# kmurf1999/RustSolver

Measured on NVIDIA B200. Metric: cfr_iterations_per_sec, higher is better.
Workload: dtype f32

## Files before the change

### include/b200cfr.h

```cpp
#ifndef B200CFR_H
#define B200CFR_H

#include <stddef.h>
#include <stdint.h>

#ifdef __cplusplus
extern "C" {
#endif

#define RS_OK 0
#define RS_ERR_INVALID -1
#define RS_ERR_CUDA -2
#define RS_ERR_NCCL -3
#define RS_ERR_CAPACITY -4
#define RS_ERR_UNSUPPORTED -5

#define RS_NODE_ACTION 0
#define RS_NODE_TERMINAL 1
#define RS_NODE_PUBLIC_CHANCE 2
#define RS_NODE_PRIVATE_CHANCE 3
#define RS_TERM_ALLIN 0
#define RS_TERM_SHOWDOWN 1
#define RS_TERM_UNCONTESTED 2
#define RS_ROUND_FLOP 0
#define RS_ROUND_TURN 1
#define RS_ROUND_RIVER 2

typedef struct rs_tree {
    uint32_t n_nodes;
    const uint8_t* type;
    const int32_t* parent;
    const uint32_t* child_offset;
    const uint32_t* children;
    const uint8_t* player;
    const uint32_t* an_index;
    const uint8_t* round_idx;
    const uint32_t* value;
    const uint8_t* ttype;
    const uint8_t* last_to_act;
} rs_tree;

typedef struct rs_ranges {
    uint32_t n_hands[2];
    const uint8_t* hands[2];
} rs_ranges;

#define RS_ABS_NONE 0
#define RS_ABS_ISOMORPHIC 1
#define RS_ABS_CLUSTER_ARR 2
#define RS_ABS_BUCKET_TABLE 3
typedef struct rs_round_abstraction {
    uint32_t kind;
    const uint32_t* cluster_arr;
    uint64_t cluster_arr_len;
    const uint32_t* bucket_table[2];
} rs_round_abstraction;
typedef struct rs_abstraction {
    uint32_t n_rounds;
    rs_round_abstraction rounds[3];
} rs_abstraction;

#define RS_NCCL_ID_BYTES 128
typedef struct rs_config {
    uint64_t board_mask;
    int32_t device;
    int32_t rank;
    int32_t world_size;
    uint8_t nccl_id[RS_NCCL_ID_BYTES];
    uint32_t flags;
    uint32_t threads_per_block;
    uint64_t discount_interval;
    uint64_t discount_cap;
} rs_config;
#define RS_FLAG_NO_GRAPH 1u
#define RS_FLAG_NO_CHAIN_SPLIT 2u
#define RS_FLAG_STREET_KERNEL 4u
#define RS_FLAG_SHARD_ISOLATED 8u
#define RS_FLAG_ALL (RS_FLAG_NO_GRAPH | RS_FLAG_NO_CHAIN_SPLIT | RS_FLAG_STREET_KERNEL | RS_FLAG_SHARD_ISOLATED)

typedef struct rs_engine rs_engine;

typedef struct rs_stats {
    uint64_t iterations;
    uint64_t updates_per_iteration;
    uint64_t updates_per_iteration_global;
    double device_ms;
    uint64_t kernel_launches;
    uint64_t table_bytes;
    uint32_t n_rounds;
    uint32_t n_boards[3];
    uint32_t n_boards_local[3];
    uint32_t n_hands[2];
    uint64_t n_combos;
} rs_stats;

const char* rs_last_error(void);
int rs_version(void);
int rs_device_count(void);
int rs_nccl_unique_id(uint8_t* out);

int rs_gpu_index_hands(uint32_t n_board_cards, const uint8_t* cards, size_t n, uint64_t* out, float* kernel_ms);

#define RS_DIST_EMD_1D 0u
#define RS_DIST_L2 1u
int rs_kmeans_assign(const float* points, size_t n, uint32_t dim, const float* centers, uint32_t k, uint32_t dist_kind,
                     uint32_t* cluster, float* min_dist, double* inertia, float* kernel_ms);
int rs_histogram_distances(const float* p, const float* q, size_t n, uint32_t dim, uint32_t dist_kind, float* out);
int rs_kmeans_fit_regular(const float* points, size_t n, uint32_t dim, float* centers, uint32_t k, uint32_t dist_kind,
                          uint32_t rounds, uint32_t* cluster, float* inertia);
int rs_generate_histograms(uint32_t round, uint64_t first_index, size_t count, uint32_t samples, uint32_t bins, uint64_t seed,
                           float* out, uint8_t* cards_out, float* kernel_ms);
int rs_kmeans_fit_growbatch(const float* points, size_t n, uint32_t dim, float* centers, uint32_t k, uint32_t dist_kind,
                            uint32_t initial_batch_size, uint64_t seed, uint32_t* batch_index_out, uint32_t* cluster_out,
                            float* stats_out);
int rs_kmeans_update_min_dists(const float* points, size_t n, uint32_t dim, const float* new_center, uint32_t dist_kind,
                               float* min_dists);
int rs_kmeans_init_pp(const float* points, size_t n, uint32_t dim, uint32_t k, uint32_t dist_kind, uint64_t seed, uint32_t* chosen_out,
                      float* centers_out);
int rs_kmeans_init_random(const float* points, size_t n, uint32_t dim, uint32_t k, uint32_t n_restarts, uint32_t dist_kind, uint64_t seed,
                          uint32_t* chosen_out, float* centers_out);

#define RS_EXCHANGE_HANDLE_BYTES 64
int rs_exchange_export(rs_engine* e, uint8_t* out );
int rs_exchange_import(rs_engine* e, const uint8_t* handles , uint32_t n_ranks);
int rs_exchange_disable(rs_engine* e);


int rs_create(const rs_tree* tree, const rs_ranges* ranges, const rs_abstraction* abs,
              const rs_config* cfg, rs_engine** out);
int rs_create_batch(const rs_tree* tree, const rs_ranges* ranges, const rs_abstraction* abs,
                    const rs_config* cfg, const uint64_t* board_masks, uint32_t n_subgames,
                    rs_engine** out);
void rs_destroy(rs_engine* e);

int rs_iterate(rs_engine* e, uint64_t n_iters);
int rs_iterate_sampled(rs_engine* e, const uint8_t* dealt, uint32_t n_paths);
int rs_sample_runouts(uint64_t seed, uint64_t board_mask, uint32_t n_cards, uint32_t n_paths, int distinct_first, uint8_t* dealt_out);
int rs_discount(rs_engine* e, float d);
int rs_set_wait_timeout_ms(rs_engine* e, uint64_t ms);
int rs_abort(rs_engine* e);
int rs_set_prune_threshold(rs_engine* e, float threshold);
#define RS_OPP_FULL 0u
#define RS_OPP_SAMPLE 1u
#define RS_OPP_SAMPLE_TIMES_SIGMA 2u
int rs_set_opponent_sampling(rs_engine* e, uint32_t mode, uint64_t seed);
#define RS_RULE_VANILLA 0u
#define RS_RULE_DCFR 1u
#define RS_RULE_LCFR 2u
#define RS_RULE_CFR_PLUS 3u
typedef struct rs_update_rule {
    uint32_t kind;
    float alpha, beta, gamma;
} rs_update_rule;
int rs_set_update_rule(rs_engine* e, const rs_update_rule* rule);
int rs_get_update_rule(rs_engine* e, rs_update_rule* out, uint64_t* t_out);
int rs_reset(rs_engine* e);

int rs_read_infoset(rs_engine* e, uint32_t an_index, uint32_t board_id, float* regrets,
                    float* strategy_sum, size_t cap_floats, uint32_t* n_rows_out,
                    uint32_t* n_actions_out);
int rs_write_infoset(rs_engine* e, uint32_t an_index, uint32_t board_id, const float* regrets,
                     const float* strategy_sum, size_t n_floats);
int rs_average_strategy(rs_engine* e, uint32_t an_index, uint32_t board_id, float* out,
                        size_t cap_floats, uint32_t* n_rows_out, uint32_t* n_actions_out);
int rs_current_strategy(rs_engine* e, uint32_t an_index, uint32_t board_id, float* out,
                        size_t cap_floats, uint32_t* n_rows_out, uint32_t* n_actions_out);
int rs_dump_average_strategy(rs_engine* e, const char* path, uint64_t* n_floats_out);

int rs_board_id(rs_engine* e, uint32_t round_idx, const uint8_t* dealt, uint32_t n_dealt,
                uint32_t* board_id_out);
int rs_card_table(rs_engine* e, uint32_t round_idx, uint32_t player, uint32_t board_id,
                  uint16_t* rows_out, size_t cap, uint32_t* n_rows_out);

int rs_best_response(rs_engine* e, double out[2]);
int rs_average_value(rs_engine* e, double out[2]);
int rs_root_values(rs_engine* e, uint32_t player, float* out, size_t cap);

int rs_stats_get(rs_engine* e, rs_stats* out);

int rs_set_range_weights(rs_engine* e, uint32_t player, const float* weights, size_t n);

#define RS_KERNEL_TRAVERSAL 0
#define RS_KERNEL_STREET 1
#define RS_KERNEL_ALLREDUCE 3
typedef struct rs_kernel_time {
    uint32_t kind;
    uint32_t phase;
    uint32_t traverser;
    uint32_t grid;
    float ms;
    uint64_t table_bytes;
    uint64_t vector_bytes;
} rs_kernel_time;
int rs_profile_iteration(rs_engine* e, rs_kernel_time* out, size_t cap, uint32_t* n_out);

int rs_debug_task_timing(rs_engine* e, unsigned long long* out32, int reset);

typedef struct rs_plan rs_plan;
int rs_plan_create(const rs_tree* tree, const rs_ranges* ranges, const rs_abstraction* abs,
                   const rs_config* cfg, const uint64_t* board_masks, uint32_t n_subgames,
                   rs_plan** out);
void rs_plan_destroy(rs_plan* p);
int rs_plan_stats(const rs_plan* p, rs_stats* out);
int rs_plan_board_id(const rs_plan* p, uint32_t round_idx, const uint8_t* dealt, uint32_t n_dealt,
                     uint32_t* board_id_out);
int rs_plan_card_table(const rs_plan* p, uint32_t round_idx, uint32_t player, uint32_t board_id,
                       uint16_t* rows_out, size_t cap, uint32_t* n_rows_out);
int rs_plan_infoset_offset(const rs_plan* p, uint32_t an_index, uint32_t board_id,
                           uint64_t* offset_out, uint32_t* n_rows_out, uint32_t* n_actions_out);
int rs_plan_showdown_order(const rs_plan* p, uint32_t player, uint32_t board_id,
                           uint16_t* order_out, uint32_t* class_out, size_t cap,
                           uint32_t* n_live_out);

int rs_plan_local_tables(const rs_plan* p, uint32_t round_idx, uint32_t player, uint32_t board_id, uint32_t* hrec_words_out,
                         uint16_t* cl_pos_out, uint16_t* slot_of_pos_out, uint32_t dims_out[2]);
int rs_plan_check_execution_order(const rs_plan* p, uint32_t traverser, int force_board_major, uint32_t* n_tickets_out,
                                  uint32_t* n_moved_out);
int rs_plan_street_info(const rs_plan* p, uint32_t traverser, uint32_t out[8]);
int rs_plan_street_program(const rs_plan* p, uint32_t traverser, uint32_t board_id, uint32_t* words_out, size_t cap,
                           uint32_t* n_words_out, uint32_t* hinfo_out, size_t hinfo_cap, uint32_t dims_out[4]);

#ifdef __cplusplus
}
#endif
#endif
```

### rustsolver_b200/_lib.py

```python
from __future__ import annotations

import ctypes as C
import os
from pathlib import Path

_HERE = Path(__file__).resolve().parent
LIB_PATH = Path(os.environ.get("RS_ENGINE_LIB", str(_HERE / "libb200cfr.so")))

u8p = C.POINTER(C.c_uint8)
u16p = C.POINTER(C.c_uint16)
u32p = C.POINTER(C.c_uint32)
u64p = C.POINTER(C.c_uint64)
i32p = C.POINTER(C.c_int32)
f32p = C.POINTER(C.c_float)
f64p = C.POINTER(C.c_double)

RS_NCCL_ID_BYTES = 128
RS_EXCHANGE_HANDLE_BYTES = 64


class rs_tree(C.Structure):
    _fields_ = [("n_nodes", C.c_uint32), ("type", u8p), ("parent", i32p), ("child_offset", u32p),
                ("children", u32p), ("player", u8p), ("an_index", u32p), ("round_idx", u8p),
                ("value", u32p), ("ttype", u8p), ("last_to_act", u8p)]


class rs_ranges(C.Structure):
    _fields_ = [("n_hands", C.c_uint32 * 2), ("hands", u8p * 2)]


class rs_round_abstraction(C.Structure):
    _fields_ = [("kind", C.c_uint32), ("cluster_arr", u32p), ("cluster_arr_len", C.c_uint64),
                ("bucket_table", u32p * 2)]


class rs_abstraction(C.Structure):
    _fields_ = [("n_rounds", C.c_uint32), ("rounds", rs_round_abstraction * 3)]


class rs_config(C.Structure):
    _fields_ = [("board_mask", C.c_uint64), ("device", C.c_int32), ("rank", C.c_int32),
                ("world_size", C.c_int32), ("nccl_id", C.c_uint8 * RS_NCCL_ID_BYTES),
                ("flags", C.c_uint32), ("threads_per_block", C.c_uint32),
                ("discount_interval", C.c_uint64), ("discount_cap", C.c_uint64)]


class rs_stats(C.Structure):
    _fields_ = [("iterations", C.c_uint64), ("updates_per_iteration", C.c_uint64),
                ("updates_per_iteration_global", C.c_uint64), ("device_ms", C.c_double),
                ("kernel_launches", C.c_uint64), ("table_bytes", C.c_uint64), ("n_rounds", C.c_uint32),
                ("n_boards", C.c_uint32 * 3), ("n_boards_local", C.c_uint32 * 3),
                ("n_hands", C.c_uint32 * 2), ("n_combos", C.c_uint64)]


class rs_update_rule(C.Structure):
    _fields_ = [("kind", C.c_uint32), ("alpha", C.c_float), ("beta", C.c_float), ("gamma", C.c_float)]


class rs_kernel_time(C.Structure):
    _fields_ = [("kind", C.c_uint32), ("phase", C.c_uint32), ("traverser", C.c_uint32), ("grid", C.c_uint32),
                ("ms", C.c_float), ("table_bytes", C.c_uint64), ("vector_bytes", C.c_uint64)]


VP = C.c_void_p
ENGINE_API = {
    "rs_last_error": (C.c_char_p, []),
    "rs_version": (C.c_int, []),
    "rs_device_count": (C.c_int, []),
    "rs_nccl_unique_id": (C.c_int, [u8p]),
    "rs_kmeans_assign": (C.c_int, [f32p, C.c_size_t, C.c_uint32, f32p, C.c_uint32, C.c_uint32, u32p, f32p, f64p, f32p]),
    "rs_kmeans_fit_regular": (C.c_int, [f32p, C.c_size_t, C.c_uint32, f32p, C.c_uint32, C.c_uint32, C.c_uint32, u32p, f32p]),
    "rs_histogram_distances": (C.c_int, [f32p, f32p, C.c_size_t, C.c_uint32, C.c_uint32, f32p]),
    "rs_kmeans_update_min_dists": (C.c_int, [f32p, C.c_size_t, C.c_uint32, f32p, C.c_uint32, f32p]),
    "rs_kmeans_init_pp": (C.c_int, [f32p, C.c_size_t, C.c_uint32, C.c_uint32, C.c_uint32, C.c_uint64, u32p, f32p]),
    "rs_generate_histograms": (C.c_int, [C.c_uint32, C.c_uint64, C.c_size_t, C.c_uint32, C.c_uint32, C.c_uint64, f32p, u8p, f32p]),
    "rs_kmeans_fit_growbatch": (C.c_int, [f32p, C.c_size_t, C.c_uint32, f32p, C.c_uint32, C.c_uint32, C.c_uint32, C.c_uint64, u32p, u32p, f32p]),
    "rs_kmeans_init_random": (C.c_int, [f32p, C.c_size_t, C.c_uint32, C.c_uint32, C.c_uint32, C.c_uint32, C.c_uint64, u32p, f32p]),
    "rs_gpu_index_hands": (C.c_int, [C.c_uint32, u8p, C.c_size_t, u64p, f32p]),
    "rs_exchange_export": (C.c_int, [VP, u8p]),
    "rs_exchange_import": (C.c_int, [VP, u8p, C.c_uint32]),
    "rs_exchange_disable": (C.c_int, [VP]),
    "rs_create": (C.c_int, [C.POINTER(rs_tree), C.POINTER(rs_ranges), C.POINTER(rs_abstraction),
                            C.POINTER(rs_config), C.POINTER(VP)]),
    "rs_create_batch": (C.c_int, [C.POINTER(rs_tree), C.POINTER(rs_ranges), C.POINTER(rs_abstraction),
                                  C.POINTER(rs_config), u64p, C.c_uint32, C.POINTER(VP)]),
    "rs_destroy": (None, [VP]),
    "rs_iterate": (C.c_int, [VP, C.c_uint64]),
    "rs_iterate_sampled": (C.c_int, [VP, u8p, C.c_uint32]),
    "rs_discount": (C.c_int, [VP, C.c_float]),
    "rs_set_prune_threshold": (C.c_int, [VP, C.c_float]),
    "rs_set_opponent_sampling": (C.c_int, [VP, C.c_uint32, C.c_uint64]),
    "rs_set_wait_timeout_ms": (C.c_int, [VP, C.c_uint64]),
    "rs_abort": (C.c_int, [VP]),
    "rs_sample_runouts": (C.c_int, [C.c_uint64, C.c_uint64, C.c_uint32, C.c_uint32, C.c_int, u8p]),
    "rs_set_update_rule": (C.c_int, [VP, C.POINTER(rs_update_rule)]),
    "rs_get_update_rule": (C.c_int, [VP, C.POINTER(rs_update_rule), u64p]),
    "rs_reset": (C.c_int, [VP]),
    "rs_read_infoset": (C.c_int, [VP, C.c_uint32, C.c_uint32, f32p, f32p, C.c_size_t, u32p, u32p]),
    "rs_write_infoset": (C.c_int, [VP, C.c_uint32, C.c_uint32, f32p, f32p, C.c_size_t]),
    "rs_average_strategy": (C.c_int, [VP, C.c_uint32, C.c_uint32, f32p, C.c_size_t, u32p, u32p]),
    "rs_dump_average_strategy": (C.c_int, [VP, C.c_char_p, u64p]),
    "rs_current_strategy": (C.c_int, [VP, C.c_uint32, C.c_uint32, f32p, C.c_size_t, u32p, u32p]),
    "rs_board_id": (C.c_int, [VP, C.c_uint32, u8p, C.c_uint32, u32p]),
    "rs_card_table": (C.c_int, [VP, C.c_uint32, C.c_uint32, C.c_uint32, u16p, C.c_size_t, u32p]),
    "rs_best_response": (C.c_int, [VP, f64p]),
    "rs_average_value": (C.c_int, [VP, f64p]),
    "rs_root_values": (C.c_int, [VP, C.c_uint32, f32p, C.c_size_t]),
    "rs_stats_get": (C.c_int, [VP, C.POINTER(rs_stats)]),
    "rs_set_range_weights": (C.c_int, [VP, C.c_uint32, f32p, C.c_size_t]),
    "rs_profile_iteration": (C.c_int, [VP, C.POINTER(rs_kernel_time), C.c_size_t, u32p]),
    "rs_debug_task_timing": (C.c_int, [VP, u64p, C.c_int]),
    "rs_plan_create": (C.c_int, [C.POINTER(rs_tree), C.POINTER(rs_ranges), C.POINTER(rs_abstraction),
                                 C.POINTER(rs_config), u64p, C.c_uint32, C.POINTER(VP)]),
    "rs_plan_destroy": (None, [VP]),
    "rs_plan_stats": (C.c_int, [VP, C.POINTER(rs_stats)]),
    "rs_plan_board_id": (C.c_int, [VP, C.c_uint32, u8p, C.c_uint32, u32p]),
    "rs_plan_card_table": (C.c_int, [VP, C.c_uint32, C.c_uint32, C.c_uint32, u16p, C.c_size_t, u32p]),
    "rs_plan_infoset_offset": (C.c_int, [VP, C.c_uint32, C.c_uint32, u64p, u32p, u32p]),
    "rs_plan_showdown_order": (C.c_int, [VP, C.c_uint32, C.c_uint32, u16p, u32p, C.c_size_t, u32p]),
    "rs_plan_local_tables": (C.c_int, [VP, C.c_uint32, C.c_uint32, C.c_uint32, u32p, u16p, u16p, u32p]),
    "rs_plan_check_execution_order": (C.c_int, [VP, C.c_uint32, C.c_int, u32p, u32p]),
    "rs_plan_street_info": (C.c_int, [VP, C.c_uint32, u32p]),
    "rs_plan_street_program": (C.c_int, [VP, C.c_uint32, C.c_uint32, u32p, C.c_size_t, u32p, u32p, C.c_size_t, u32p]),
}
HOST_API = {
    "rsh_options_default_flop": (VP, []),
    "rsh_options_new": (VP, [C.c_uint64, C.c_uint32, C.c_uint32, C.c_uint32]),
    "rsh_options_free": (None, [VP]),
    "rsh_options_set_sizes": (C.c_int, [VP, C.c_uint32, u32p, f64p, u32p, f64p]),
    "rsh_options_set_range": (C.c_int, [VP, C.c_uint32, C.c_char_p]),
    "rsh_options_set_range_hands": (C.c_int, [VP, C.c_uint32, u8p, C.c_uint32]),
    "rsh_options_board_mask": (C.c_uint64, [VP]),
    "rsh_options_range": (C.c_int, [VP, C.c_uint32, u8p, C.c_size_t]),
    "rsh_build_game_tree": (C.c_int, [VP, C.POINTER(VP)]),
    "rsh_tree_free": (None, [VP]),
    "rsh_tree_n_nodes": (C.c_uint32, [VP]),
    "rsh_tree_n_actions": (C.c_uint32, [VP]),
    "rsh_tree_n_edges": (C.c_uint32, [VP]),
    "rsh_tree_view": (C.c_int, [VP, C.POINTER(rs_tree)]),
    "rsh_tree_round": (u8p, [VP]),
    "rsh_tree_action_kind": (u8p, [VP]),
    "rsh_tree_action_amount": (f64p, [VP]),
    "rsh_evaluate": (C.c_uint32, [u8p, C.c_uint32]),
    "rsh_get_card_mask": (C.c_int, [C.c_char_p, u64p]),
    "rsh_range_from_string": (C.c_int, [C.c_char_p, C.c_uint64, u8p, C.c_size_t]),
    "rsh_indexer_new": (VP, [C.c_uint32, u8p]),
    "rsh_indexer_free": (None, [VP]),
    "rsh_indexer_size": (C.c_uint64, [VP, C.c_uint32]),
    "rsh_indexer_index": (C.c_uint64, [VP, u8p]),
    "rsh_indexer_index_many": (None, [VP, u8p, C.c_size_t, u64p]),
    "rsh_indexer_get_hand": (C.c_int, [VP, C.c_uint32, C.c_uint64, u8p]),
}

_lib = None


def load():
    global _lib
    if _lib is not None:
        return _lib
    if not LIB_PATH.exists():
        raise ImportError(
            f"{LIB_PATH} is missing: build it with `python -m rustsolver_b200.build` "
            "(there is no CPU/Python fallback for the engine)")
    if "RS_NCCL_LIB" not in os.environ:
        try:
            import importlib.util
            spec = importlib.util.find_spec("nvidia.nccl")
            if spec and spec.submodule_search_locations:
                cand = Path(list(spec.submodule_search_locations)[0]) / "lib" / "libnccl.so.2"
                if cand.exists():
                    os.environ["RS_NCCL_LIB"] = str(cand)
        except Exception:
            pass
    lib = C.CDLL(str(LIB_PATH))
    for table in (ENGINE_API, HOST_API):
        for name, (res, args) in table.items():
            fn = getattr(lib, name)
            fn.restype = res
            fn.argtypes = args
    _lib = lib
    return lib


class EngineError(RuntimeError):
    def __init__(self, code: int, msg: str):
        super().__init__(f"b200cfr error {code}: {msg}")
        self.code = code


def check(rc: int):
    if rc != 0:
        raise EngineError(rc, load().rs_last_error().decode())
```

### rustsolver_b200/csrc/engine.cu

```cuda
#include <cuda_runtime.h>
#include <dlfcn.h>

#include <cmath>
#include <cstdio>
#include <cstdlib>
#include <cstring>
#include <map>
#include <memory>
#include <string>
#include <vector>

#include "../../include/b200cfr.h"
#include <cmath>

#include "abstraction_kernels.h"
#include "histogram_kernel.h"
#include "indexer_kernel.h"
#include "kernels.cuh"
#include "plan.h"
#include "street_kernel.cuh"

namespace rs {

thread_local std::string g_last_error;

static int set_err(int code, const std::string& msg) {
    g_last_error = msg;
    return code;
}

namespace nccl {
typedef struct {
    char internal[128];
} UniqueId;
typedef void* Comm;
typedef int (*GetUniqueId_t)(UniqueId*);
typedef int (*CommInitRank_t)(Comm*, int, UniqueId, int);
typedef int (*AllReduce_t)(const void*, void*, size_t, int, int, Comm, cudaStream_t);
typedef int (*CommDestroy_t)(Comm);
typedef const char* (*GetErrorString_t)(int);
struct Api {
    void* lib = nullptr;
    GetUniqueId_t GetUniqueId = nullptr;
    CommInitRank_t CommInitRank = nullptr;
    AllReduce_t AllReduce = nullptr;
    CommDestroy_t CommDestroy = nullptr;
    GetErrorString_t GetErrorString = nullptr;
};
static Api g_api;
constexpr int kFloat32 = 7;
constexpr int kSum = 0;

static bool load(std::string* err) {
    if (g_api.lib) return true;
    const char* env = getenv("RS_NCCL_LIB");
    const char* names[] = {env, "libnccl.so.2", "libnccl.so"};
    void* lib = nullptr;
    for (const char* n : names) {
        if (!n || !*n) continue;
        lib = dlopen(n, RTLD_NOW | RTLD_GLOBAL);
        if (lib) break;
    }
    if (!lib) {
        *err = "cannot dlopen libnccl.so.2 (set RS_NCCL_LIB to its path)";
        return false;
    }
    g_api.lib = lib;
    g_api.GetUniqueId = (GetUniqueId_t)dlsym(lib, "ncclGetUniqueId");
    g_api.CommInitRank = (CommInitRank_t)dlsym(lib, "ncclCommInitRank");
    g_api.AllReduce = (AllReduce_t)dlsym(lib, "ncclAllReduce");
    g_api.CommDestroy = (CommDestroy_t)dlsym(lib, "ncclCommDestroy");
    g_api.GetErrorString = (GetErrorString_t)dlsym(lib, "ncclGetErrorString");
    if (!g_api.GetUniqueId || !g_api.CommInitRank || !g_api.AllReduce || !g_api.CommDestroy) {
        *err = "libnccl is missing expected symbols";
        g_api = Api();
        return false;
    }
    return true;
}
}

#define CU(call)                                                                                   \
    do {                                                                                           \
        cudaError_t e__ = (call);                                                                  \
        if (e__ != cudaSuccess)                                                                    \
            return set_err(RS_ERR_CUDA, std::string(#call) + ": " + cudaGetErrorString(e__));      \
    } while (0)

static bool device_batch_index(const HandIndexer& ix, const uint8_t* cards, size_t n, uint64_t* out, std::string* err) {
    return gpu_index_hands(ix, ix.rounds() - 1, cards, n, out, nullptr, err);
}

template <class T>
struct DevBuf {
    T* p = nullptr;
    size_t n = 0;
    ~DevBuf() {
        if (p) cudaFree(p);
    }
    cudaError_t alloc(size_t count) {
        n = count;
        if (count == 0) count = 1;
        return cudaMalloc(&p, count * sizeof(T));
    }
    cudaError_t upload(const T* src, size_t count) {
        cudaError_t e = alloc(count);
        if (e != cudaSuccess || count == 0) return e;
        return cudaMemcpy(p, src, count * sizeof(T), cudaMemcpyHostToDevice);
    }
    cudaError_t upload(const std::vector<T>& v) { return upload(v.data(), v.size()); }
    cudaError_t zero() { return cudaMemset(p, 0, (n ? n : 1) * sizeof(T)); }
};

struct RoundDev {
    DevBuf<uint16_t> row_of_pos[2], row_start[2], row_pos[2], cl_pos[2], parent_pos[2], child_pos[2], slot_of_pos[2];
    DevBuf<HandRec> hrec[2];
    DevBuf<uint32_t> n_rows[2], n_rows_pad[2], n_live[2];
    DevBuf<uint64_t> board_off[2];
    DevBuf<float> regrets[2], ssum[2];
    DevBuf<float> chance_scale;
    DevBuf<int32_t> parent_board;
    DevBuf<float> rbuf, cbuf, gathered;
    DevBuf<float> sbuf[2];
    uint32_t n_leaves = 0, n_boards = 0;
};

struct TaskSet {
    DevBuf<NodeTask> tasks;
    DevBuf<TaskSrc> srcs;
    DevBuf<uint32_t> tix;
    DevBuf<uint32_t> order;
    uint32_t n_tickets = 0, phase_cut = 0, n_tasks = 0;
    uint32_t street_lo = 0, street_hi = 0;
    uint32_t street_inst = 0;
    struct Run {
        uint32_t t0, t1;
        int threads;
    };
    std::vector<Run> runs;
    uint32_t xch_lo = 0, xch_hi = 0;
    struct Section {
        uint32_t first;
        uint32_t round_k;
        bool up;
    };
    std::vector<Section> sections;
};

struct StreetDev {
    DevBuf<SwSeg> segs;
    DevBuf<SwDown> downs;
    DevBuf<SwUp> ups;
    DevBuf<SwTerm> terms;
    DevBuf<uint32_t> prog, prog_off, l_steps, c_steps, hinfo;
    uint32_t n_segs = 0;
};

struct Engine {
    Plan plan;
    int device = 0;
    int threads = 512;
    cudaStream_t stream = nullptr;
    cudaEvent_t ev0 = nullptr, ev1 = nullptr;
    cudaGraph_t graph = nullptr;
    cudaGraphExec_t graph_exec = nullptr;
    bool use_graph = true;
    nccl::Comm comm = nullptr;
    bool isolated = false;

    RoundDev rd[3];
    DevBuf<float> scratch;
    DevBuf<float> root_weights[2];
    TaskSet full[2];
    std::map<int, std::unique_ptr<TaskSet[]>> sampled_sets;
    DevBuf<int32_t> sample_board[3];
    int sample_cap = 0;
    DevBuf<uint32_t> flags;
    DevBuf<TaskCtl> ctl;
    DevBuf<unsigned long long> timing;
    DevBuf<unsigned char> xch;
    size_t xch_flag_bytes = 0, xch_vectors = 0;
    void* xch_peer_base[RS_MAX_PEERS] = {nullptr};
    bool fused_exchange = false;
    float prune_threshold = -INFINITY;
    int xs_mode = 0;
    uint64_t xs_seed = 0, xs_count = 0;
    uint32_t* abort_host = nullptr;
    uint32_t* abort_dev = nullptr;
    uint64_t wait_timeout_ms = 30000;
    bool aborted = false;
    int check_abort(const char* what);
    int maybe_discount();
    rs_update_rule rule = {RS_RULE_VANILLA, 1.5f, 0.f, 2.f};
    uint64_t rule_t = 0;
    bool rule_on() const { return rule.kind != RS_RULE_VANILLA; }
    int advance_rule();
    uint64_t last_discount_period = 0;
    bool street_on = false;
    StreetDev street[2];
    DevBuf<float> st_scratch;
    size_t st_stride = 0, st_smem = 0;
    int st_XP = 0, st_rows = 0, st_vy_rows = 0, st_vm_rows = 0, st_slots = 0, st_threads = 0, st_blocks_per_sm = 1, st_qs = 1, st_qm = 1;
    int slots = 1;
    size_t smem_bytes = 0;
    size_t smem_small = 0;
    int blocks_per_sm = 1, n_sms = 148;
    int round_threads[3] = {0, 0, 0};
    int bps_small = 0;
    bool wide_for(int thr, uint64_t tickets) const {
        return thr > 288 || bps_small == 0 || getenv("RS_WIDE_ONLY") || (tickets <= uint64_t(n_sms) * blocks_per_sm && !getenv("RS_SMALL_ONLY"));
    }
    std::vector<rs_kernel_time>* prof = nullptr;
    std::vector<std::pair<cudaEvent_t, cudaEvent_t>> prof_events;

    uint64_t iterations = 0;
    double device_ms = 0;
    uint64_t launches = 0;
    uint64_t launches_per_iter = 0;
    uint64_t table_bytes = 0;
    uint64_t updates_global = 0;
    uint64_t discount_interval = 0, discount_cap = 0;

    void close_peers() {
        for (int r = 0; r < RS_MAX_PEERS; ++r) {
            if (xch_peer_base[r] && r != plan.rank) cudaIpcCloseMemHandle(xch_peer_base[r]);
            xch_peer_base[r] = nullptr;
        }
    }

    ~Engine() {
        close_peers();
        if (graph_exec) cudaGraphExecDestroy(graph_exec);
        if (graph) cudaGraphDestroy(graph);
        if (comm && nccl::g_api.CommDestroy) nccl::g_api.CommDestroy(comm);
        if (abort_host) cudaFreeHost(abort_host);
        if (root_stage) cudaFreeHost(root_stage);
        if (ev0) cudaEventDestroy(ev0);
        if (ev1) cudaEventDestroy(ev1);
        if (stream) cudaStreamDestroy(stream);
    }

    int init(const rs_config* cfg);
    void fill_args(TaskArgs* a, int trav, const TaskSet& set) const;
    int materialize(int trav, const uint32_t counts[3], TaskSet* out);
    int enqueue_sampled(int n_paths, int n_paths_global, uint64_t* count);
    int enqueue_traversal(int trav, int mode, uint64_t* count, const TaskSet* set = nullptr, int n_paths = -1, int n_paths_global = 0);
    int init_street();
    int enqueue_street(int trav, int mode, const TaskSet& set, int n_paths);
    int enqueue_iteration(uint64_t* count);
    int iterate(uint64_t n);
    int root_sum(int player, double* out);
    int root_values(int player, std::vector<float>* out);
    int root_values_into(int player, float* dst);
    DevBuf<float> root_out;
    float* root_stage = nullptr;
    size_t root_stage_n = 0;
    int prof_begin();
    int prof_end(uint32_t kind, uint32_t k, int trav, uint32_t grid, uint64_t table_bytes, uint64_t vector_bytes);
};

template <class T>
static std::vector<T> slice(const std::vector<T>& v, size_t lo, size_t hi, size_t stride) {
    if (v.empty()) return {};
    return std::vector<T>(v.begin() + lo * stride, v.begin() + hi * stride);
}

int Engine::init(const rs_config* cfg) {
    int ndev = 0;
    cudaError_t e = cudaGetDeviceCount(&ndev);
    if (e != cudaSuccess || ndev == 0)
        return set_err(RS_ERR_CUDA, std::string("no CUDA device available (the engine has no CPU fallback): ") +
                                        (e != cudaSuccess ? cudaGetErrorString(e) : "device count is 0"));
    device = cfg->device;
    if (device < 0 || device >= ndev) return set_err(RS_ERR_INVALID, "device ordinal out of range");
    CU(cudaSetDevice(device));
    cudaDeviceProp prop;
    CU(cudaGetDeviceProperties(&prop, device));
    if (prop.major < 10) return set_err(RS_ERR_UNSUPPORTED, "kernels are built for sm_100a only; found an older device");
    if (cfg->threads_per_block)
        return set_err(RS_ERR_INVALID, "threads_per_block is derived from the range size (4 hands per thread) and cannot be set");
    if (cfg->flags & ~uint32_t(RS_FLAG_ALL)) return set_err(RS_ERR_INVALID, "unknown bits in rs_config.flags");
    use_graph = !(cfg->flags & RS_FLAG_NO_GRAPH);
    isolated = (cfg->flags & RS_FLAG_SHARD_ISOLATED) != 0;
    discount_interval = cfg->discount_interval;
    discount_cap = cfg->discount_cap;
    CU(cudaStreamCreateWithFlags(&stream, cudaStreamNonBlocking));
    CU(cudaEventCreate(&ev0));
    CU(cudaEventCreate(&ev1));

    const Plan& P = plan;
    for (int q = 0; q < 2; ++q) {
        std::vector<float> ones(P.H[q], 1.0f);
        CU(root_weights[q].upload(ones));
    }
    const int HP[2] = {int((P.H[0] + 3) & ~3u), int((P.H[1] + 3) & ~3u)};
    const size_t maxHP = size_t(std::max(HP[0], HP[1]));
    const bool street_wanted = P.street[0].eligible && P.street[1].eligible;
    threads = int(((maxHP / 4) + 31) / 32 * 32);
    if (threads > MAX_TASK_THREADS) return set_err(RS_ERR_UNSUPPORTED, "range larger than 1326 hands");
    for (uint32_t k = 0; k < P.n_rounds; ++k) {
        round_threads[k] = threads;
        if (!P.board_mask[k].empty() && !getenv("RS_UNIFORM_BLOCK")) {
            const int left = 52 - __builtin_popcountll(P.board_mask[k][0]);
            const size_t live_max = std::min<size_t>(maxHP, size_t(left) * size_t(left - 1) / 2);
            round_threads[k] = std::min(threads, int((((live_max + 3) / 4) + 31) / 32 * 32));
        }
    }
    n_sms = prop.multiProcessorCount;
    if (street_wanted) {
        int rc = init_street();
        if (rc != RS_OK) return rc;
    }
    for (uint32_t k = 0; k < P.n_rounds; ++k) {
        RoundDev& R = rd[k];
        const uint32_t lo = P.local_lo[k], hi = P.local_hi[k], nb = hi - lo;
        R.n_boards = nb;
        R.n_leaves = (k + 1 < P.n_rounds) ? uint32_t(P.segs[k + 1].size()) : 0;
        for (int q = 0; q < 2; ++q) {
            const RoundPlayerTables& T = P.tabs[k][q];
            const LocalTables& L = P.loc[k][q];
            const size_t hp = L.Hpad;
            CU(R.row_of_pos[q].upload(slice(L.row_of_pos, lo, hi, hp)));
            CU(R.row_start[q].upload(slice(L.row_start, lo, hi, hp + 4)));
            CU(R.row_pos[q].upload(slice(L.row_pos, lo, hi, hp)));
            CU(R.cl_pos[q].upload(slice(L.cl_pos, lo, hi, 2 * hp)));
            CU(R.slot_of_pos[q].upload(slice(L.slot_of_pos, lo, hi, hp)));
            {
                std::vector<HandRec> aos = slice(L.hrec, lo, hi, hp);
                std::vector<HandRec> soa(aos.size());
                const uint32_t* src = reinterpret_cast<const uint32_t*>(aos.data());
                uint32_t* dst = reinterpret_cast<uint32_t*>(soa.data());
                for (size_t b = 0; b < size_t(nb); ++b)
                    for (size_t i = 0; i < hp; ++i)
                        for (int wd = 0; wd < 4; ++wd) dst[(b * 4 + wd) * hp + i] = src[(b * hp + i) * 4 + wd];
                CU(R.hrec[q].upload(soa));
            }
            if (k > 0) {
                CU(R.parent_pos[q].upload(slice(L.parent_pos, lo, hi, hp)));
                CU(R.child_pos[q].upload(slice(L.child_pos, lo, hi, size_t(P.loc[k - 1][q].Hpad))));
            }
            CU(R.n_rows[q].upload(slice(T.n_rows, lo, hi, 1)));
            CU(R.n_rows_pad[q].upload(slice(L.n_rows_pad, lo, hi, 1)));
            CU(R.n_live[q].upload(slice(L.n_live, lo, hi, 1)));
            CU(R.board_off[q].upload(slice(T.board_off, lo, hi, 1)));
            const size_t cells = size_t(T.board_off[P.n_boards[k]]);
            CU(R.regrets[q].alloc(cells));
            CU(R.ssum[q].alloc(cells));
            CU(R.regrets[q].zero());
            CU(R.ssum[q].zero());
            table_bytes += 2 * cells * sizeof(float);
        }
        CU(R.chance_scale.upload(slice(P.chance_scale[k], lo, hi, 1)));
        std::vector<int32_t> pb(nb, -1);
        if (k > 0)
            for (uint32_t b = 0; b < nb; ++b) pb[b] = P.board_parent[k][lo + b] - int32_t(P.local_lo[k - 1]);
        CU(R.parent_board.upload(pb));
        const bool fused_round = street_on && k + 1 == P.n_rounds;
        const size_t n_r = fused_round ? 0 : std::max(P.tl[0].n_rbuf[k], P.tl[1].n_rbuf[k]);
        const size_t n_c = (fused_round && k > 0) ? 0 : std::max(P.tl[0].n_cbuf[k], P.tl[1].n_cbuf[k]);
        CU(R.rbuf.alloc(n_r * nb * maxHP));
        CU(R.cbuf.alloc(n_c * nb * maxHP));
        CU(R.gathered.alloc(size_t(R.n_leaves) * nb * maxHP));
        for (int p = 0; p < 2; ++p) {
            CU(R.sbuf[p].alloc(size_t(P.tl[p].n_sbuf[k]) * nb * maxHP));
            CU(R.sbuf[p].zero());
        }
        CU(R.rbuf.zero());
        CU(R.cbuf.zero());
        CU(R.gathered.zero());
    }
    uint32_t max_tickets = 0;
    for (int p = 0; p < 2; ++p) {
        uint32_t counts[3] = {0, 0, 0};
        for (uint32_t k = 0; k < P.n_rounds; ++k) counts[k] = rd[k].n_boards;
        int rc = materialize(p, counts, &full[p]);
        if (rc != RS_OK) return rc;
        max_tickets = std::max(max_tickets, full[p].n_tickets);
        slots = std::max(slots, int(std::max(P.tl[p].max_terminal, 1 + P.tl[p].max_children)));
    }
    CU(timing.alloc(96));
    CU(timing.zero());
    CU(flags.alloc(max_tickets));
    CU(flags.zero());
    {
        TaskCtl c0{};
        c0.ticket = 0;
        c0.exited = 0;
        c0.xch_seq = 1;
        c0.epoch = 1;
        c0.rule[0] = c0.rule[1] = c0.rule[2] = 1.f;
        c0.rule[3] = -INFINITY;
        CU(ctl.upload(&c0, 1));
        CU(cudaHostAlloc(reinterpret_cast<void**>(&abort_host), sizeof(uint32_t), cudaHostAllocMapped));
        *abort_host = 0;
        CU(cudaHostGetDevicePointer(reinterpret_cast<void**>(&abort_dev), abort_host, 0));
    }
    size_t smem_need = std::max(task_kernel_smem_bytes(true, slots, HP[0], HP[1]), task_kernel_smem_bytes(true, slots, HP[1], HP[0]));
    int max_optin = 0;
    CU(cudaDeviceGetAttribute(&max_optin, cudaDevAttrMaxSharedMemoryPerBlockOptin, device));
    if (smem_need > size_t(max_optin))
        return set_err(RS_ERR_UNSUPPORTED, "node too wide for one CTA's shared memory: need " +
                                               std::to_string(smem_need) + " B, device allows " + std::to_string(max_optin));
    smem_bytes = smem_need;
    CU(configure_task_kernels(smem_need, threads, true, &blocks_per_sm));
    if (blocks_per_sm < 1) return set_err(RS_ERR_UNSUPPORTED, "task kernel does not fit on an SM");
    for (uint32_t k = 0; k < P.n_rounds; ++k)
        if (round_threads[k] <= 288 && bps_small == 0) {
            smem_small = std::max(task_kernel_smem_bytes(false, slots, HP[0], HP[1]), task_kernel_smem_bytes(false, slots, HP[1], HP[0]));
            CU(configure_task_kernels(smem_small, 288, false, &bps_small));
            if (bps_small < 1) return set_err(RS_ERR_UNSUPPORTED, "task kernel does not fit on an SM");
        }
    n_sms = prop.multiProcessorCount;
    CU(scratch.alloc(size_t(1326) * MAX_ACTIONS));

    updates_global = P.updates_per_iter_local;
    if (P.world > 1 && !isolated) {
        std::string err;
        if (!nccl::load(&err)) return set_err(RS_ERR_NCCL, err);
        nccl::UniqueId id;
        static_assert(sizeof(id) == RS_NCCL_ID_BYTES, "nccl id size");
        memcpy(&id, cfg->nccl_id, sizeof(id));
        int rc = nccl::g_api.CommInitRank(&comm, P.world, id, P.rank);
        if (rc != 0)
            return set_err(RS_ERR_NCCL, std::string("ncclCommInitRank: ") +
                                            (nccl::g_api.GetErrorString ? nccl::g_api.GetErrorString(rc) : "error"));
        DevBuf<float> tmp;
        CU(tmp.alloc(4));
        uint64_t u = P.updates_per_iter_local;
        if (P.rank > 0)
            for (uint32_t k = 0; k < P.shard_round; ++k)
                for (int q = 0; q < 2; ++q) u -= P.tabs[k][q].board_off[P.n_boards[k]];
        float parts[4] = {float(u & 0xFFFFF), float((u >> 20) & 0xFFFFF), float((u >> 40) & 0xFFFFF), 0.f};
        CU(cudaMemcpy(tmp.p, parts, sizeof(parts), cudaMemcpyHostToDevice));
        rc = nccl::g_api.AllReduce(tmp.p, tmp.p, 4, nccl::kFloat32, nccl::kSum, comm, stream);
        if (rc != 0) return set_err(RS_ERR_NCCL, "ncclAllReduce failed");
        CU(cudaStreamSynchronize(stream));
        CU(cudaMemcpy(parts, tmp.p, sizeof(parts), cudaMemcpyDeviceToHost));
        updates_global = uint64_t(parts[0]) + (uint64_t(parts[1]) << 20) + (uint64_t(parts[2]) << 40);
    }
    if (P.world > 1 && P.shard_round >= 1 && !isolated) {
        const RoundDev& Par = rd[P.shard_round - 1];
        xch_vectors = size_t(Par.n_leaves) * Par.n_boards * size_t(P.world);
        xch_flag_bytes = (2 * xch_vectors * sizeof(uint32_t) + 255) & ~size_t(255);
        CU(xch.alloc(xch_flag_bytes + 2 * xch_vectors * maxHP * sizeof(float)));
        CU(xch.zero());
    }
    CU(cudaDeviceSynchronize());
    return RS_OK;
}


int Engine::init_street() {
    const Plan& P = plan;
    uint32_t max_rows = 1, max_slots = 1, max_q_sd = 1, max_q_mo = 1;
    for (int p = 0; p < 2; ++p) {
        const StreetPlan& S = P.street[p];
        StreetDev& D = street[p];
        CU(D.segs.upload(S.segs));
        CU(D.downs.upload(S.downs));
        CU(D.ups.upload(S.ups));
        CU(D.terms.upload(S.terms));
        CU(D.prog.upload(S.prog));
        CU(D.prog_off.upload(S.prog_off));
        CU(D.l_steps.upload(S.l_steps));
        CU(D.c_steps.upload(S.c_steps));
        CU(D.hinfo.upload(S.hinfo));
        D.n_segs = uint32_t(S.segs.size());
        max_rows = std::max(max_rows, S.max_rows);
        max_slots = std::max(max_slots, S.max_slots);
        max_q_sd = std::max(max_q_sd, S.max_q_sd);
        max_q_mo = std::max(max_q_mo, S.max_q_mo);
    }
    const int HP[2] = {int((P.H[0] + 3) & ~3u), int((P.H[1] + 3) & ~3u)};
    const int HPmax = std::max(HP[0], HP[1]);
    st_XP = (HPmax + 31) & ~31;
    st_rows = int(max_rows);
    st_vy_rows = 4 * int(max_q_sd);
    st_vm_rows = 4 * int(max_q_sd + max_q_mo);
    st_slots = int(max_slots);
    st_stride = size_t(st_rows) * st_XP + size_t(st_vy_rows + st_vm_rows + st_slots) * HPmax;
    st_threads = threads;
    if (const char* e = getenv("RS_STREET_THREADS")) st_threads = std::max(64, std::min(352, atoi(e) / 32 * 32));
    size_t budget = 72 * 1024;
    if (const char* e = getenv("RS_STREET_SMEM_KB")) budget = size_t(std::max(16, atoi(e))) * 1024;
    st_qs = st_qm = 1;
    const int max_q = st_threads / 32;
    while (st_qs < int(max_q_sd) && st_qs < max_q && street_smem_bytes(st_qs + 1, st_qm, HPmax, HPmax) <= budget) ++st_qs;
    while (st_qm < int(max_q_mo) && st_qm < max_q && street_smem_bytes(st_qs, st_qm + 1, HPmax, HPmax) <= budget) ++st_qm;
    st_smem = street_smem_bytes(st_qs, st_qm, HPmax, HPmax);
    int max_optin = 0;
    CU(cudaDeviceGetAttribute(&max_optin, cudaDevAttrMaxSharedMemoryPerBlockOptin, device));
    if (st_smem > size_t(max_optin)) return RS_OK;
    CU(configure_street_kernels(st_smem, st_threads, &st_blocks_per_sm));
    if (st_blocks_per_sm < 1) return RS_OK;
    if (const char* e = getenv("RS_STREET_BLOCKS")) st_blocks_per_sm = std::max(1, std::min(st_blocks_per_sm, atoi(e)));
    CU(st_scratch.alloc(st_stride * size_t(n_sms) * st_blocks_per_sm));
    CU(st_scratch.zero());
    street_on = true;
    return RS_OK;
}

int Engine::enqueue_street(int trav, int mode, const TaskSet& set, int n_paths) {
    const Plan& P = plan;
    const uint32_t k = P.n_rounds - 1;
    const RoundDev& R = rd[k];
    const StreetDev& D = street[trav];
    StreetArgs a;
    memset(&a, 0, sizeof(a));
    for (int q = 0; q < 2; ++q) {
        DevRoundPlayer& d = a.rp[q];
        d.row_of_pos = R.row_of_pos[q].p;
        d.row_start = R.row_start[q].p;
        d.row_pos = R.row_pos[q].p;
        d.cl_pos = R.cl_pos[q].p;
        d.parent_pos = R.parent_pos[q].p;
        d.child_pos = R.child_pos[q].p;
        d.slot_of_pos = R.slot_of_pos[q].p;
        d.hrec = R.hrec[q].p;
        d.n_rows = R.n_rows[q].p;
        d.n_rows_pad = R.n_rows_pad[q].p;
        d.n_live = R.n_live[q].p;
        d.board_off = R.board_off[q].p;
        d.regrets = R.regrets[q].p;
        d.ssum = R.ssum[q].p;
        d.identity = 1;
    }
    a.chance_scale = R.chance_scale.p;
    a.parent_board = R.parent_board.p;
    a.parent_rbuf = k > 0 ? rd[k - 1].rbuf.p : nullptr;
    a.parent_n_boards = k > 0 ? int(rd[k - 1].n_boards) : 0;
    a.n_boards = int(R.n_boards);
    a.root_weights = root_weights[1 - trav].p;
    a.out_buf = k > 0 ? R.sbuf[trav].p : R.cbuf.p;
    a.out_scatter = k > 0 ? 1 : 0;
    a.n_segs = int(D.n_segs);
    a.segs = D.segs.p;
    a.downs = D.downs.p;
    a.ups = D.ups.p;
    a.terms = D.terms.p;
    a.prog = D.prog.p;
    a.prog_off = D.prog_off.p;
    a.l_steps = D.l_steps.p;
    a.c_steps = D.c_steps.p;
    a.hinfo = D.hinfo.p;
    a.scratch = st_scratch.p;
    a.scratch_stride = st_stride;
    a.XP = st_XP;
    a.max_rows = st_rows;
    a.vy_rows = st_vy_rows;
    a.vm_rows = st_vm_rows;
    a.max_slots = st_slots;
    a.qs = st_qs;
    a.qm = st_qm;
    a.trav = trav;
    a.HpP = int((P.H[trav] + 3) & ~3u);
    a.HoP = int((P.H[1 - trav] + 3) & ~3u);
    a.n_units = set.street_inst * D.n_segs;
    a.sample_board = (n_paths >= 0 && k > 0) ? sample_board[k].p : nullptr;
    a.prune_threshold = prune_threshold;
    const int grid = int(std::min<uint64_t>(a.n_units, uint64_t(n_sms) * st_blocks_per_sm));
    CU(launch_street_kernel(a, mode, grid, st_threads, st_smem, stream));
    return RS_OK;
}

int Engine::materialize(int trav, const uint32_t counts[3], TaskSet* out) {
    MaterializedTasks mt;
    materialize_tasks(plan, trav, counts, &mt);
    std::vector<NodeTask>& t = mt.tasks;
    std::vector<TaskSrc>& sr = mt.srcs;
    const uint32_t first = mt.n_tickets;
    out->phase_cut = mt.phase_cut;
    out->n_tickets = first;
    out->n_tasks = uint32_t(t.size());
    out->street_lo = out->street_hi = 0;
    out->street_inst = counts[plan.n_rounds - 1];
    if (street_on) {
        bool seen = false, closed = false;
        for (const NodeTask& x : t) {
            const bool fin = uint32_t(x.round_k) + 1 == plan.n_rounds;
            if (fin && closed) return set_err(RS_ERR_INVALID, "internal: final-round tasks are not contiguous");
            if (fin && !seen) {
                seen = true;
                out->street_lo = x.first;
            }
            if (fin) out->street_hi = x.first + x.count;
            if (!fin && seen) closed = true;
        }
    }
    out->runs.clear();
    out->sections.clear();
    out->xch_lo = out->xch_hi = 0;
    for (const NodeTask& x : t) {
        if (x.count == 0) continue;
        if (x.kind == TK_GATHER && plan.world > 1 && plan.shard_round >= 1 && uint32_t(x.round_k) + 1 == plan.shard_round) {
            if (out->xch_hi == out->xch_lo) out->xch_lo = x.first;
            out->xch_hi = x.first + x.count;
        }
        const int thr = round_threads[x.round_k];
        if (out->runs.empty() || out->runs.back().threads != thr) out->runs.push_back({x.first, x.first + x.count, thr});
        else out->runs.back().t1 = x.first + x.count;
        const bool up = x.kind == TK_UP_TRAV, down = x.kind == TK_DOWN;
        if (up || down) {
            bool seen = false;
            for (const TaskSet::Section& sc : out->sections) seen |= (sc.round_k == x.round_k && sc.up == up);
            if (!seen) out->sections.push_back({x.first, uint32_t(x.round_k), up});
        }
    }
    std::vector<uint32_t> tix(first);
    for (size_t j = 0; j < t.size(); ++j)
        for (uint32_t i = 0; i < t[j].count; ++i) tix[t[j].first + i] = uint32_t(j);
    CU(out->tasks.upload(t));
    CU(out->srcs.upload(sr));
    CU(out->tix.upload(tix));
    if (!getenv("RS_TASK_MAJOR")) {
        std::vector<uint32_t> ord;
        std::string oerr;
        if (!build_execution_order(plan, trav, mt, counts, getenv("RS_BOARD_MAJOR") != nullptr, &ord, &oerr)) return set_err(RS_ERR_INVALID, oerr);
        if (!ord.empty()) CU(out->order.upload(ord));
    }
    return RS_OK;
}

void Engine::fill_args(TaskArgs* a, int trav, const TaskSet& set) const {
    const Plan& P = plan;
    memset(a, 0, sizeof(*a));
    for (int q = 0; q < 2; ++q) {
        a->H[q] = int(P.H[q]);
        a->Hpad[q] = int((P.H[q] + 3) & ~3u);
        a->root_weights[q] = root_weights[q].p;
    }
    for (uint32_t k = 0; k < P.n_rounds; ++k) {
        const RoundDev& R = rd[k];
        RoundArgs& ra = a->rounds[k];
        for (int q = 0; q < 2; ++q) {
            DevRoundPlayer& d = ra.rp[q];
            d.row_of_pos = R.row_of_pos[q].p;
            d.row_start = R.row_start[q].p;
            d.row_pos = R.row_pos[q].p;
            d.cl_pos = R.cl_pos[q].p;
            d.parent_pos = R.parent_pos[q].p;
            d.child_pos = R.child_pos[q].p;
            d.slot_of_pos = R.slot_of_pos[q].p;
            d.hrec = R.hrec[q].p;
            d.n_rows = R.n_rows[q].p;
            d.n_rows_pad = R.n_rows_pad[q].p;
            d.n_live = R.n_live[q].p;
            d.board_off = R.board_off[q].p;
            d.regrets = R.regrets[q].p;
            d.ssum = R.ssum[q].p;
            d.identity = P.loc[k][q].identity ? 1 : 0;
        }
        ra.chance_scale = R.chance_scale.p;
        ra.parent_board = R.parent_board.p;
        ra.rbuf = R.rbuf.p;
        ra.cbuf = R.cbuf.p;
        ra.sbuf = R.sbuf[trav].p;
        ra.gathered = R.gathered.p;
        ra.n_boards = int(R.n_boards);
        ra.board_base = int(P.local_lo[k]);
        if (k + 1 < P.n_rounds) {
            const bool sharded_next = (P.world > 1 && k + 1 == P.shard_round);
            ra.per_parent = sharded_next ? 0 : int(P.deal_count[k + 1]);
            ra.n_boards_next = int(rd[k + 1].n_boards);
        }
    }
    a->tasks = set.tasks.p;
    a->srcs = set.srcs.p;
    a->task_of_ticket = set.tix.p;
    a->order = set.order.n ? set.order.p : nullptr;
    a->n_tasks = set.n_tasks;
    a->flags = flags.p;
    a->ctl = ctl.p;
    a->trav = trav;
    a->HpP = a->Hpad[trav];
    a->HoP = a->Hpad[1 - trav];
    a->Hx = std::max(a->HpP, a->HoP);
    if (fused_exchange) {
        a->xch_world = P.world;
        a->xch_rank = P.rank;
        a->xch_round = int(P.shard_round);
        a->xch_leaves = int(rd[P.shard_round - 1].n_leaves);
        for (int r = 0; r < P.world; ++r) {
            a->xflag_peer[r] = reinterpret_cast<uint32_t*>(xch_peer_base[r]);
            a->xch_peer[r] = reinterpret_cast<float*>(static_cast<unsigned char*>(xch_peer_base[r]) + xch_flag_bytes);
        }
    }
    a->slots = slots;
    a->prune_threshold = prune_threshold;
    a->host_abort = abort_dev;
    a->wait_timeout_ns = wait_timeout_ms * 1000000ull;
    a->timing = timing.p;
}

int Engine::prof_begin() {
    if (!prof) return RS_OK;
    cudaEvent_t a, b;
    CU(cudaEventCreate(&a));
    CU(cudaEventCreate(&b));
    prof_events.emplace_back(a, b);
    CU(cudaEventRecord(a, stream));
    return RS_OK;
}

int Engine::prof_end(uint32_t kind, uint32_t phase, int trav, uint32_t grid, uint64_t tb, uint64_t vb) {
    if (!prof) return RS_OK;
    CU(cudaEventRecord(prof_events.back().second, stream));
    rs_kernel_time t;
    memset(&t, 0, sizeof(t));
    t.kind = kind;
    t.phase = phase;
    t.traverser = uint32_t(trav);
    t.grid = grid;
    t.table_bytes = tb;
    t.vector_bytes = vb;
    prof->push_back(t);
    return RS_OK;
}

int Engine::enqueue_traversal(int trav, int mode, uint64_t* count, const TaskSet* set, int n_paths, int n_paths_global) {
    const Plan& P = plan;
    const TaskList& tl = P.tl[trav];
    if (!set) set = &full[trav];
    TaskArgs a;
    fill_args(&a, trav, *set);
    if (n_paths >= 0) {
        a.n_paths = n_paths;
        for (uint32_t k = 1; k < P.n_rounds; ++k) {
            a.sample_board[k] = sample_board[k].p;
            a.gather_scale[k - 1] = float(P.deal_count[k]) / float(k == 1 ? n_paths_global : 1);
        }
    }
    if (mode == KM_CFR && xs_mode) {
        uint64_t z = xs_seed + 0x9E3779B97F4A7C15ull * (++xs_count);
        z = (z ^ (z >> 30)) * 0xBF58476D1CE4E5B9ull;
        z = (z ^ (z >> 27)) * 0x94D049BB133111EBull;
        a.xs_key = z ^ (z >> 31);
        a.xs_mode = xs_mode;
        mode = KM_CFR_XS;
    }
    if (rule_on() && (mode == KM_CFR || mode == KM_CFR_XS)) mode = mode == KM_CFR ? KM_CFR_DR : KM_CFR_XS_DR;
    int rc;
    struct Step {
        int kind;
        uint32_t t0, t1, phase;
    };
    std::vector<Step> steps;
    const bool use_street = street_on && set->street_hi > set->street_lo;
    uint32_t at = 0;
    if (use_street) {
        if (set->street_lo > 0) steps.push_back({0, 0, set->street_lo, 0});
        steps.push_back({1, 0, 0, 0});
        at = set->street_hi;
    }
    const bool split = !fused_exchange && !isolated && set->phase_cut < set->n_tickets;
    const uint32_t cut = split ? std::max(set->phase_cut, at) : set->n_tickets;
    if (cut > at) steps.push_back({0, at, cut, use_street ? 1u : 0u});
    if (split) {
        steps.push_back({2, 0, 0, 0});
        steps.push_back({0, cut, set->n_tickets, 2});
    }
    uint64_t vec = 0;
    for (uint32_t k = 0; k < P.n_rounds; ++k)
        vec += (uint64_t(tl.n_rbuf[k]) * P.H[1 - trav] + uint64_t(tl.n_cbuf[k]) * P.H[trav]) * rd[k].n_boards * 8;
    for (const Step& sp : steps) {
        if ((rc = prof_begin()) != RS_OK) return rc;
        if (sp.kind == 0) {
            struct Piece {
                uint32_t t0, t1;
                int threads;
            };
            std::vector<Piece> pieces;
            for (const TaskSet::Run& r : set->runs) {
                const uint32_t lo = std::max(sp.t0, r.t0), hi = std::min(sp.t1, r.t1);
                if (lo < hi) pieces.push_back({lo, hi, r.threads});
            }
            size_t longest = 0;
            for (size_t i = 1; i < pieces.size(); ++i)
                if (pieces[i].t1 - pieces[i].t0 > pieces[longest].t1 - pieces[longest].t0) longest = i;
            for (size_t i = 0; i < pieces.size(); ++i) {
                if (i > 0 && (rc = prof_begin()) != RS_OK) return rc;
                a.t0 = pieces[i].t0;
                a.t1 = pieces[i].t1;
                a.xch_bump = (fused_exchange && set->xch_lo < set->xch_hi && a.t0 <= set->xch_lo && set->xch_lo < a.t1) ? 1 : 0;
                const int thr = pieces[i].threads;
                const bool wide = wide_for(thr, a.t1 - a.t0);
                const int grid = int(std::min<uint64_t>(uint64_t(a.t1 - a.t0), uint64_t(n_sms) * (wide ? blocks_per_sm : bps_small)));
                CU(launch_task_kernel(a, mode, grid, thr, wide, wide ? smem_bytes : smem_small, stream));
                uint64_t bytes = 0;
                for (const TaskSet::Section& sc : set->sections)
                    if (sc.first >= a.t0 && sc.first < a.t1) {
                        const uint64_t own = P.tabs[sc.round_k][trav].board_off[P.n_boards[sc.round_k]];
                        const uint64_t opp = P.tabs[sc.round_k][1 - trav].board_off[P.n_boards[sc.round_k]];
                        bytes += sc.up ? own * 16 : opp * 4;
                    }
                if ((rc = prof_end(RS_KERNEL_TRAVERSAL, sp.phase + (i == longest ? 0u : 8u), trav, uint32_t(grid), bytes, i == longest ? vec : 0)) != RS_OK)
                    return rc;
                if (i + 1 < pieces.size()) ++*count;
            }
        } else if (sp.kind == 1) {
            if ((rc = enqueue_street(trav, mode, *set, n_paths)) != RS_OK) return rc;
            const uint32_t k = P.n_rounds - 1;
            const uint64_t own = P.tabs[k][trav].board_off[P.n_boards[k]], opp = P.tabs[k][1 - trav].board_off[P.n_boards[k]];
            const uint32_t grid = uint32_t(std::min<uint64_t>(uint64_t(set->street_inst) * street[trav].n_segs, uint64_t(n_sms) * st_blocks_per_sm));
            if ((rc = prof_end(RS_KERNEL_STREET, 0, trav, grid, own * 16 + opp * 4, 0)) != RS_OK) return rc;
        } else {
            RoundDev& Par = rd[P.shard_round - 1];
            const size_t n = size_t(Par.n_leaves) * Par.n_boards * ((P.H[trav] + 3) & ~3u);
            int nrc = nccl::g_api.AllReduce(Par.gathered.p, Par.gathered.p, n, nccl::kFloat32, nccl::kSum, comm, stream);
            if (nrc != 0) return set_err(RS_ERR_NCCL, "ncclAllReduce failed");
            if ((rc = prof_end(RS_KERNEL_ALLREDUCE, 0, trav, 0, 0, n * 4)) != RS_OK) return rc;
        }
        ++*count;
    }
    return RS_OK;
}

int Engine::enqueue_sampled(int n_paths, int n_paths_global, uint64_t* count) {
    auto it = sampled_sets.find(n_paths);
    if (it == sampled_sets.end()) {
        std::unique_ptr<TaskSet[]> sets(new TaskSet[2]);
        for (int p = 0; p < 2; ++p) {
            uint32_t counts[3] = {rd[0].n_boards, uint32_t(n_paths), uint32_t(n_paths)};
            int rc = materialize(p, counts, &sets[p]);
            if (rc != RS_OK) return rc;
        }
        it = sampled_sets.emplace(n_paths, std::move(sets)).first;
    }
    for (int p = 0; p < 2; ++p) {
        int rc = enqueue_traversal(p, KM_CFR, count, &it->second[p], n_paths, n_paths_global);
        if (rc != RS_OK) return rc;
    }
    return RS_OK;
}

int Engine::enqueue_iteration(uint64_t* count) {
    for (int p = 0; p < 2; ++p) {
        int rc = enqueue_traversal(p, KM_CFR, count);
        if (rc != RS_OK) return rc;
    }
    return RS_OK;
}

int Engine::iterate(uint64_t n) {
    CU(cudaSetDevice(device));
    if (n == 0) return RS_OK;
    if (aborted) return set_err(RS_ERR_CUDA, "an earlier traversal was aborted: the tables are partly updated, create a new engine");
    const bool use_graph = this->use_graph && !xs_mode;
    if (use_graph && !graph_exec) {
        uint64_t cnt = 0;
        CU(cudaStreamBeginCapture(stream, cudaStreamCaptureModeThreadLocal));
        int rc = enqueue_iteration(&cnt);
        cudaError_t e = cudaStreamEndCapture(stream, &graph);
        if (rc != RS_OK) return rc;
        if (e != cudaSuccess) return set_err(RS_ERR_CUDA, std::string("graph capture: ") + cudaGetErrorString(e));
        CU(cudaGraphInstantiate(&graph_exec, graph, 0));
        launches_per_iter = cnt;
    }
    CU(cudaEventRecord(ev0, stream));
    for (uint64_t i = 0; i < n; ++i) {
        {
            int rc = advance_rule();
            if (rc != RS_OK) return rc;
        }
        if (use_graph) {
            CU(cudaGraphLaunch(graph_exec, stream));
            launches += launches_per_iter;
        } else {
            uint64_t cnt = 0;
            int rc = enqueue_iteration(&cnt);
            if (rc != RS_OK) return rc;
            launches += cnt;
            launches_per_iter = cnt;
        }
        ++iterations;
        {
            int rc = maybe_discount();
            if (rc != RS_OK) return rc;
        }
    }
    CU(cudaEventRecord(ev1, stream));
    CU(cudaStreamSynchronize(stream));
    float ms = 0.f;
    CU(cudaEventElapsedTime(&ms, ev0, ev1));
    device_ms += ms;
    return check_abort("rs_iterate");
}

static void update_rule_factors(const rs_update_rule& r, uint64_t t, float f[4]) {
    f[0] = f[1] = f[2] = 1.f;
    f[3] = r.kind == RS_RULE_CFR_PLUS ? 0.f : -INFINITY;
    if (t <= 1) return;
    const double s = double(t - 1);
    if (r.kind == RS_RULE_DCFR || r.kind == RS_RULE_LCFR) {
        const bool lin = r.kind == RS_RULE_LCFR;
        const double a = lin ? 1.0 : double(r.alpha), b = lin ? 1.0 : double(r.beta), g = lin ? 1.0 : double(r.gamma);
        f[0] = float(1.0 / (1.0 + std::pow(s, -a)));
        f[1] = float(1.0 / (1.0 + std::pow(s, -b)));
        f[2] = float(std::pow(s / double(t), g));
    } else if (r.kind == RS_RULE_CFR_PLUS) {
        f[2] = float(s / double(t));
    }
}

int Engine::advance_rule() {
    if (!rule_on()) return RS_OK;
    float f[4];
    update_rule_factors(rule, ++rule_t, f);
    CU(launch_set_rule(ctl.p, f, stream));
    ++launches;
    return RS_OK;
}

int Engine::maybe_discount() {
    if (!discount_interval) return RS_OK;
    const uint64_t period = iterations / discount_interval;
    if (period == last_discount_period) return RS_OK;
    last_discount_period = period;
    if (discount_cap && iterations > discount_cap) return RS_OK;
    const float pf = float(period);
    const float d = pf / (pf + 1.0f);
    for (uint32_t k = 0; k < plan.n_rounds; ++k)
        for (int q = 0; q < 2; ++q) {
            CU(launch_scale(rd[k].regrets[q].p, rd[k].regrets[q].n, d, stream));
            CU(launch_scale(rd[k].ssum[q].p, rd[k].ssum[q].n, d, stream));
            launches += 2;
        }
    return RS_OK;
}

int Engine::check_abort(const char* what) {
    if (!fused_exchange && !(abort_host && *abort_host)) return RS_OK;
    TaskCtl c;
    CU(cudaMemcpy(&c, ctl.p, sizeof(c), cudaMemcpyDeviceToHost));
    if (!c.abort) return RS_OK;
    aborted = true;
    return set_err(RS_ERR_CUDA, std::string(what) + ": the traversal kernel gave up waiting (" +
                                    ((abort_host && *abort_host) ? "rs_abort was called" : "a wait exceeded the bound of " + std::to_string(wait_timeout_ms) +
                                                                                               " ms: a peer rank did not launch the same traversal") +
                                    "); the tables are partly updated, create a new engine");
}
// ... 625 lines not shown
    return RS_OK;
}

int rs_average_strategy(rs_engine* e, uint32_t an_index, uint32_t board_id, float* out, size_t cap_floats,
                        uint32_t* n_rows_out, uint32_t* n_actions_out) {
    return strategy_impl(e, an_index, board_id, out, cap_floats, n_rows_out, n_actions_out, true);
}
int rs_current_strategy(rs_engine* e, uint32_t an_index, uint32_t board_id, float* out, size_t cap_floats,
                        uint32_t* n_rows_out, uint32_t* n_actions_out) {
    return strategy_impl(e, an_index, board_id, out, cap_floats, n_rows_out, n_actions_out, false);
}

int rs_dump_average_strategy(rs_engine* e, const char* path, uint64_t* n_floats_out) {
    if (!e || !path) return set_err(RS_ERR_INVALID, "null argument");
    Engine& E = e->e;
    const Plan& P = E.plan;
    FILE* f = fopen(path, "wb");
    if (!f) return set_err(RS_ERR_INVALID, std::string("cannot open ") + path);
    uint64_t total = 0;
    std::vector<float> buf;
    int rc = RS_OK;
    for (uint32_t an = 0; an < P.an_to_pnode.size() && rc == RS_OK; ++an) {
        if (P.an_to_pnode[an] < 0) continue;
        const uint32_t k = P.nodes[P.an_to_pnode[an]].round_k;
        for (uint32_t b = P.local_lo[k]; b < P.local_hi[k]; ++b) {
            uint32_t nr = 0, na = 0;
            if ((rc = strategy_impl(e, an, b, nullptr, 0, &nr, &na, true)) != RS_OK) break;
            buf.resize(size_t(nr) * na);
            if (buf.empty()) continue;
            if ((rc = strategy_impl(e, an, b, buf.data(), buf.size(), &nr, &na, true)) != RS_OK) break;
            if (fwrite(buf.data(), sizeof(float), buf.size(), f) != buf.size()) {
                rc = set_err(RS_ERR_INVALID, std::string("short write to ") + path);
                break;
            }
            total += buf.size();
        }
    }
    fclose(f);
    if (rc == RS_OK && n_floats_out) *n_floats_out = total;
    return rc;
}

static int board_id_impl(const Plan& P, uint32_t round_idx, const uint8_t* dealt, uint32_t n_dealt, uint32_t* out) {
    if (round_idx >= P.n_rounds) return set_err(RS_ERR_INVALID, "round_idx out of range");
    if (n_dealt != round_idx) return set_err(RS_ERR_INVALID, "need exactly round_idx dealt cards");
    if (P.n_sub != 1) return set_err(RS_ERR_UNSUPPORTED, "board lookup by dealt cards needs a single root board; batch boards are their own ids");
    uint32_t id = 0;
    uint64_t mask = P.board_mask[0][0];
    for (uint32_t k = 1; k <= round_idx; ++k) {
        const int c = dealt[k - 1];
        if (c >= 52 || (mask & (1ull << c))) return set_err(RS_ERR_INVALID, "dealt card already on the board");
        const uint32_t idx = uint32_t(__builtin_popcountll(~mask & ((1ull << c) - 1)));
        id = id * P.deal_count[k] + idx;
        mask |= 1ull << c;
    }
    *out = id;
    return RS_OK;
}

int rs_plan_board_id(const rs_plan* p, uint32_t round_idx, const uint8_t* dealt, uint32_t n_dealt, uint32_t* board_id_out) {
    if (!p || !board_id_out) return set_err(RS_ERR_INVALID, "null argument");
    return board_id_impl(p->p, round_idx, dealt, n_dealt, board_id_out);
}
int rs_board_id(rs_engine* e, uint32_t round_idx, const uint8_t* dealt, uint32_t n_dealt, uint32_t* board_id_out) {
    if (!e || !board_id_out) return set_err(RS_ERR_INVALID, "null argument");
    return board_id_impl(e->e.plan, round_idx, dealt, n_dealt, board_id_out);
}

static int card_table_impl(const Plan& P, uint32_t round_idx, uint32_t player, uint32_t board_id, uint16_t* rows_out,
                           size_t cap, uint32_t* n_rows_out) {
    if (round_idx >= P.n_rounds || player > 1) return set_err(RS_ERR_INVALID, "round/player out of range");
    if (board_id >= P.n_boards[round_idx]) return set_err(RS_ERR_INVALID, "board_id out of range");
    if (board_id < P.local_lo[round_idx] || board_id >= P.local_hi[round_idx])
        return set_err(RS_ERR_INVALID, "board is owned by another rank");
    const RoundPlayerTables& T = P.tabs[round_idx][player];
    const uint32_t H = P.H[player];
    if (n_rows_out) *n_rows_out = T.n_rows[board_id];
    if (rows_out) {
        if (cap < H) return set_err(RS_ERR_CAPACITY, "output buffer too small");
        memcpy(rows_out, &T.row_of_hand[size_t(board_id) * H], H * sizeof(uint16_t));
    }
    return RS_OK;
}
int rs_plan_card_table(const rs_plan* p, uint32_t round_idx, uint32_t player, uint32_t board_id, uint16_t* rows_out,
                       size_t cap, uint32_t* n_rows_out) {
    if (!p) return set_err(RS_ERR_INVALID, "null plan");
    return card_table_impl(p->p, round_idx, player, board_id, rows_out, cap, n_rows_out);
}
int rs_card_table(rs_engine* e, uint32_t round_idx, uint32_t player, uint32_t board_id, uint16_t* rows_out, size_t cap,
                  uint32_t* n_rows_out) {
    if (!e) return set_err(RS_ERR_INVALID, "null engine");
    return card_table_impl(e->e.plan, round_idx, player, board_id, rows_out, cap, n_rows_out);
}

int rs_plan_showdown_order(const rs_plan* p, uint32_t player, uint32_t board_id, uint16_t* order_out, uint32_t* class_out,
                           size_t cap, uint32_t* n_live_out) {
    if (!p || player > 1) return set_err(RS_ERR_INVALID, "bad argument");
    const Plan& P = p->p;
    const uint32_t k = P.n_rounds - 1;
    const ShowdownTables& S = P.sd[player];
    if (S.n_live.empty()) return set_err(RS_ERR_INVALID, "tree has no showdown terminals");
    if (board_id >= P.n_boards[k]) return set_err(RS_ERR_INVALID, "board_id out of range");
    const uint32_t H = P.H[player];
    const uint32_t nl = S.n_live[board_id];
    if (n_live_out) *n_live_out = nl;
    if (cap < nl) return set_err(RS_ERR_CAPACITY, "output buffer too small");
    for (uint32_t i = 0; i < nl; ++i) {
        if (order_out) order_out[i] = S.sorted[size_t(board_id) * H + i];
        if (class_out) class_out[i] = S.cls[size_t(board_id) * H + i];
    }
    return RS_OK;
}

int rs_plan_local_tables(const rs_plan* p, uint32_t round_idx, uint32_t player, uint32_t board_id, uint32_t* hrec_words_out, uint16_t* cl_pos_out,
                         uint16_t* slot_of_pos_out, uint32_t dims_out[2]) {
    if (!p || player > 1 || !dims_out) return set_err(RS_ERR_INVALID, "bad argument");
    const Plan& P = p->p;
    if (round_idx >= P.n_rounds || board_id >= P.n_boards[round_idx]) return set_err(RS_ERR_INVALID, "round or board out of range");
    if (board_id < P.local_lo[round_idx] || board_id >= P.local_hi[round_idx]) return set_err(RS_ERR_INVALID, "board belongs to another rank");
    const LocalTables& L = P.loc[round_idx][player];
    dims_out[0] = L.Hpad;
    dims_out[1] = L.n_live[board_id];
    if (hrec_words_out) memcpy(hrec_words_out, &L.hrec[size_t(board_id) * L.Hpad], size_t(L.Hpad) * sizeof(HandRec));
    if (cl_pos_out) memcpy(cl_pos_out, &L.cl_pos[size_t(board_id) * 2 * L.Hpad], size_t(2) * L.Hpad * sizeof(uint16_t));
    if (slot_of_pos_out) memcpy(slot_of_pos_out, &L.slot_of_pos[size_t(board_id) * L.Hpad], size_t(L.Hpad) * sizeof(uint16_t));
    return RS_OK;
}

int rs_plan_check_execution_order(const rs_plan* p, uint32_t traverser, int force_board_major, uint32_t* n_tickets_out, uint32_t* n_moved_out) {
    if (!p || traverser > 1) return set_err(RS_ERR_INVALID, "bad argument");
    const Plan& P = p->p;
    uint32_t counts[3] = {0, 0, 0};
    for (uint32_t k = 0; k < P.n_rounds; ++k) counts[k] = P.boards_local(k);
    MaterializedTasks mt;
    materialize_tasks(P, int(traverser), counts, &mt);
    std::vector<uint32_t> ord;
    std::string err;
    if (!build_execution_order(P, int(traverser), mt, counts, force_board_major > 0, &ord, &err)) return set_err(RS_ERR_INVALID, err);
    if (force_board_major < 0) {
        ord.resize(mt.n_tickets);
        for (uint32_t i = 0; i < mt.n_tickets; ++i) ord[i] = mt.n_tickets - 1 - i;
    }
    err = check_execution_order(P, int(traverser), mt, counts, ord);
    if (!err.empty()) return set_err(RS_ERR_INVALID, "execution order: " + err);
    if (n_tickets_out) *n_tickets_out = mt.n_tickets;
    if (n_moved_out) {
        uint32_t moved = 0;
        for (uint32_t i = 0; i < ord.size(); ++i) moved += ord[i] != i;
        *n_moved_out = moved;
    }
    return RS_OK;
}

int rs_plan_street_info(const rs_plan* p, uint32_t traverser, uint32_t out[8]) {
    if (!p || !out || traverser > 1) return set_err(RS_ERR_INVALID, "bad argument");
    const StreetPlan& S = p->p.street[traverser];
    out[0] = S.eligible ? 1u : 0u;
    out[1] = uint32_t(S.segs.size());
    out[2] = S.max_rows;
    out[3] = S.max_slots;
    out[4] = S.max_q_sd;
    out[5] = S.max_q_mo;
    out[6] = uint32_t(S.downs.size());
    out[7] = uint32_t(S.ups.size());
    if (!S.eligible) g_last_error = S.why;
    return RS_OK;
}

int rs_plan_street_program(const rs_plan* p, uint32_t traverser, uint32_t board_id, uint32_t* words_out, size_t cap,
                           uint32_t* n_words_out, uint32_t* hinfo_out, size_t hinfo_cap, uint32_t dims_out[4]) {
    if (!p || !n_words_out || !dims_out || traverser > 1) return set_err(RS_ERR_INVALID, "bad argument");
    const Plan& P = p->p;
    const StreetPlan& S = P.street[traverser];
    if (!S.eligible) return set_err(RS_ERR_INVALID, "the final round does not run on the street kernel: " + S.why);
    const uint32_t k = P.n_rounds - 1;
    if (board_id < P.local_lo[k] || board_id >= P.local_hi[k]) return set_err(RS_ERR_INVALID, "board is owned by another rank");
    const uint32_t lb = board_id - P.local_lo[k];
    const uint32_t n = S.prog_off[lb + 1] - S.prog_off[lb];
    const uint32_t HpP = P.loc[k][traverser].Hpad;
    *n_words_out = n;
    dims_out[0] = S.l_steps[lb];
    dims_out[1] = S.c_steps[lb];
    dims_out[2] = HpP;
    dims_out[3] = P.loc[k][1 - traverser].Hpad;
    if (words_out) {
        if (cap < n) return set_err(RS_ERR_CAPACITY, "output buffer too small");
        memcpy(words_out, S.prog.data() + S.prog_off[lb], size_t(n) * sizeof(uint32_t));
    }
    if (hinfo_out) {
        if (hinfo_cap < 2 * size_t(HpP)) return set_err(RS_ERR_CAPACITY, "hinfo buffer too small");
        memcpy(hinfo_out, S.hinfo.data() + size_t(lb) * HpP * 2, size_t(HpP) * 2 * sizeof(uint32_t));
    }
    return RS_OK;
}

static int score_impl(rs_engine* e, int mode, double out[2]) {
    if (!e || !out) return set_err(RS_ERR_INVALID, "null argument");
    Engine& E = e->e;
    if (E.aborted) return set_err(RS_ERR_CUDA, "an earlier traversal was aborted: create a new engine");
    CU(cudaSetDevice(E.device));
    for (int p = 0; p < 2; ++p) {
        uint64_t cnt = 0;
        int rc = E.enqueue_traversal(p, mode, &cnt);
        if (rc != RS_OK) return rc;
        CU(cudaStreamSynchronize(E.stream));
        if ((rc = E.check_abort(mode == KM_BR ? "rs_best_response" : "rs_average_value")) != RS_OK) return rc;
        double s = 0;
        rc = E.root_sum(p, &s);
        if (rc != RS_OK) return rc;
        out[p] = s;
    }
    return RS_OK;
}

int rs_best_response(rs_engine* e, double out[2]) { return score_impl(e, KM_BR, out); }
int rs_average_value(rs_engine* e, double out[2]) { return score_impl(e, KM_EVAL, out); }

int rs_root_values(rs_engine* e, uint32_t player, float* out, size_t cap) {
    if (!e || !out || player > 1) return set_err(RS_ERR_INVALID, "bad argument");
    Engine& E = e->e;
    const size_t n = size_t(E.rd[0].n_boards) * E.plan.H[player];
    if (cap < n) return set_err(RS_ERR_CAPACITY, "output buffer too small");
    CU(cudaSetDevice(E.device));
    return E.root_values_into(int(player), out);
}

int rs_set_range_weights(rs_engine* e, uint32_t player, const float* weights, size_t n) {
    if (!e || !weights || player > 1) return set_err(RS_ERR_INVALID, "bad argument");
    Engine& E = e->e;
    if (n != E.plan.H[player]) return set_err(RS_ERR_INVALID, "weights length must equal the range size");
    CU(cudaSetDevice(E.device));
    CU(cudaMemcpyAsync(E.root_weights[player].p, weights, n * sizeof(float), cudaMemcpyHostToDevice, E.stream));
    return RS_OK;
}

int rs_profile_iteration(rs_engine* e, rs_kernel_time* out, size_t cap, uint32_t* n_out) {
    if (!e || !n_out) return set_err(RS_ERR_INVALID, "null argument");
    Engine& E = e->e;
    CU(cudaSetDevice(E.device));
    std::vector<rs_kernel_time> rec;
    int rc = E.advance_rule();
    if (rc != RS_OK) return rc;
    E.prof = &rec;
    uint64_t cnt = 0;
    rc = E.enqueue_iteration(&cnt);
    E.prof = nullptr;
    cudaError_t se = cudaStreamSynchronize(E.stream);
    for (size_t i = 0; i < E.prof_events.size(); ++i) {
        if (rc == RS_OK && se == cudaSuccess && i < rec.size())
            cudaEventElapsedTime(&rec[i].ms, E.prof_events[i].first, E.prof_events[i].second);
        cudaEventDestroy(E.prof_events[i].first);
        cudaEventDestroy(E.prof_events[i].second);
    }
    E.prof_events.clear();
    if (rc != RS_OK) return rc;
    if (se != cudaSuccess) return set_err(RS_ERR_CUDA, cudaGetErrorString(se));
    E.iterations += 1;
    E.launches += cnt;
    *n_out = uint32_t(rec.size());
    if (out) {
        if (cap < rec.size()) return set_err(RS_ERR_CAPACITY, "output buffer too small");
        memcpy(out, rec.data(), rec.size() * sizeof(rs_kernel_time));
    }
    return RS_OK;
}

int rs_debug_task_timing(rs_engine* e, unsigned long long* out32, int reset) {
    if (!e || !out32) return set_err(RS_ERR_INVALID, "null argument");
    Engine& E = e->e;
    CU(cudaSetDevice(E.device));
    CU(cudaStreamSynchronize(E.stream));
    CU(cudaMemcpy(out32, E.timing.p, 96 * sizeof(unsigned long long), cudaMemcpyDeviceToHost));
    if (reset) {
        std::vector<unsigned long long> init(96, 0);
        for (int i = 0; i < 32; ++i) init[32 + 2 * i] = ~0ull;
        CU(cudaMemcpy(E.timing.p, init.data(), 96 * sizeof(unsigned long long), cudaMemcpyHostToDevice));
    }
    return RS_OK;
}

static void fill_stats(const Plan& P, rs_stats* s) {
    memset(s, 0, sizeof(*s));
    s->updates_per_iteration = P.updates_per_iter_local;
    s->updates_per_iteration_global = P.updates_per_iter_global;
    s->n_rounds = P.n_rounds;
    for (uint32_t k = 0; k < P.n_rounds; ++k) {
        s->n_boards[k] = P.n_boards[k];
        s->n_boards_local[k] = P.local_hi[k] - P.local_lo[k];
    }
    s->n_hands[0] = P.H[0];
    s->n_hands[1] = P.H[1];
    s->n_combos = P.n_combos.empty() ? 0 : P.n_combos[0];
}

int rs_plan_stats(const rs_plan* p, rs_stats* out) {
    if (!p || !out) return set_err(RS_ERR_INVALID, "null argument");
    fill_stats(p->p, out);
    return RS_OK;
}

int rs_stats_get(rs_engine* e, rs_stats* out) {
    if (!e || !out) return set_err(RS_ERR_INVALID, "null argument");
    fill_stats(e->e.plan, out);
    out->iterations = e->e.iterations;
    out->device_ms = e->e.device_ms;
    out->kernel_launches = e->e.launches;
    out->table_bytes = e->e.table_bytes;
    out->updates_per_iteration_global = e->e.updates_global;
    return RS_OK;
}

}
```

### rustsolver_b200/csrc/kernels.cu

```cuda
#include "kernels.cuh"

#ifndef RS_MIN_BLOCKS_288
#define RS_MIN_BLOCKS_288 3
#endif
#ifndef RS_MIN_BLOCKS_352
#define RS_MIN_BLOCKS_352 2
#endif

#ifndef RS_POLL_SLEEP_NS
#define RS_POLL_SLEEP_NS 64
#endif

namespace rs {

namespace {

__device__ __forceinline__ uint32_t ld_acquire_u32(const uint32_t* p) {
    uint32_t v;
    asm volatile("ld.acquire.gpu.global.u32 %0, [%1];" : "=r"(v) : "l"(p) : "memory");
    return v;
}
__device__ __forceinline__ uint32_t ld_acquire_sys_u32(const uint32_t* p) {
    uint32_t v;
    asm volatile("ld.acquire.sys.global.u32 %0, [%1];" : "=r"(v) : "l"(p) : "memory");
    return v;
}
__device__ __forceinline__ void st_release_sys_u32(uint32_t* p, uint32_t v) {
    asm volatile("st.release.sys.global.u32 [%0], %1;" ::"l"(p), "r"(v) : "memory");
}
__device__ __forceinline__ void st_release_u32(uint32_t* p, uint32_t v) {
    asm volatile("st.release.gpu.global.u32 [%0], %1;" ::"l"(p), "r"(v) : "memory");
}
__device__ __forceinline__ void prefetch_l2_bulk(const void* p, uint32_t bytes) {
    if (bytes) asm volatile("cp.async.bulk.prefetch.L2.global [%0], %1;" ::"l"(p), "r"(bytes) : "memory");
}
__device__ __forceinline__ float4 ldcg4(const float* p) { return __ldcg(reinterpret_cast<const float4*>(p)); }
__device__ __forceinline__ void stcg4(float* p, float4 v) { __stcg(reinterpret_cast<float4*>(p), v); }
__device__ __forceinline__ float4 f4zero() { return make_float4(0.f, 0.f, 0.f, 0.f); }
__device__ __forceinline__ float4 f4add(float4 a, float4 b) { return make_float4(a.x + b.x, a.y + b.y, a.z + b.z, a.w + b.w); }
__device__ __forceinline__ float f4get(const float4& v, int i) { return i == 0 ? v.x : (i == 1 ? v.y : (i == 2 ? v.z : v.w)); }
__device__ __forceinline__ void f4set(float4& v, int i, float x) {
    if (i == 0) v.x = x;
    else if (i == 1) v.y = x;
    else if (i == 2) v.z = x;
    else v.w = x;
}
__device__ __forceinline__ void unpack4(uint2 u, uint32_t (&o)[4]) {
    o[0] = u.x & 0xffffu;
    o[1] = u.x >> 16;
    o[2] = u.y & 0xffffu;
    o[3] = u.y >> 16;
}

__device__ __forceinline__ void csync(int n_compute) { asm volatile("bar.sync 2, %0;" ::"r"(n_compute) : "memory"); }
__device__ __forceinline__ void hsync(int n_all) { asm volatile("bar.sync 1, %0;" ::"r"(n_all) : "memory"); }

__device__ __forceinline__ void mbar_init(uint64_t* bar, uint32_t count) {
    asm volatile("mbarrier.init.shared::cta.b64 [%0], %1;" ::"r"(uint32_t(__cvta_generic_to_shared(bar))), "r"(count) : "memory");
}
__device__ __forceinline__ void mbar_arrive(uint64_t* bar) {
    asm volatile("mbarrier.arrive.release.cta.shared::cta.b64 _, [%0];" ::"r"(uint32_t(__cvta_generic_to_shared(bar))) : "memory");
}
__device__ __forceinline__ bool mbar_test(uint64_t* bar, uint32_t parity) {
    uint32_t ok;
    asm volatile(
        "{\n\t.reg .pred p;\n\tmbarrier.test_wait.parity.acquire.cta.shared::cta.b64 p, [%1], %2;\n\tselp.u32 %0, 1, 0, p;\n\t}"
        : "=r"(ok)
        : "r"(uint32_t(__cvta_generic_to_shared(bar))), "r"(parity)
        : "memory");
    return ok != 0;
}

__device__ __forceinline__ bool wait_gives_up(const TaskArgs& A, unsigned long long t_start, uint32_t& spins) {
    if ((++spins & 255u) != 0) return false;
    if (*reinterpret_cast<const volatile unsigned int*>(&A.ctl->abort)) return true;
    bool trip = false;
    if ((spins & 4095u) == 0 && A.host_abort && *A.host_abort) trip = true;
    if (A.wait_timeout_ns) {
        unsigned long long now;
        asm volatile("mov.u64 %0, %globaltimer;" : "=l"(now));
        if (now - t_start > A.wait_timeout_ns) trip = true;
    }
    if (trip) atomicExch(&A.ctl->abort, 1u);
    return trip;
}
__device__ __forceinline__ unsigned long long global_ns() {
    unsigned long long now;
    asm volatile("mov.u64 %0, %globaltimer;" : "=l"(now));
    return now;
}

struct Ctx {
    int nc;
    int tid, lane, warp, nwarps;
    int pos4;
    int p, o, Hp, Ho, HpP, HoP, Hx;
};

extern __shared__ __align__(16) float smem_raw[];
#define SM_RS (smem_raw)
#define SM_P (smem_raw + HC)
#define SM_GB (smem_raw + 2 * HC + 4)
#define SM_WSA (smem_raw + 4 * HC + 12)
#define SM_WSB (smem_raw + 4 * HC + 44)
#define SM_B (smem_raw + 4 * HC + 76)
#define SM_WSC (smem_raw + 4 * HC + 140)
#define SM_WSD (smem_raw + 4 * HC + 172)
#define SM_BF (smem_raw + 4 * HC + 204)
#define SM_REC (reinterpret_cast<uint32_t*>(smem_raw + 4 * HC + 268))
#define SM_CL (reinterpret_cast<uint32_t*>(smem_raw + 8 * HC + 268))
#define SM_X (smem_raw + 9 * HC + 268)
constexpr int smem_fixed_floats(int HC) { return 9 * HC + 268; }

template <int HC>
__device__ __forceinline__ void stage_lists_raw(int tid, int HoP, const uint16_t* __restrict__ cl_pos_b) {
    if (8 * tid < 2 * HoP)
        asm volatile("cp.async.cg.shared.global [%0], [%1], 16;" ::"r"(uint32_t(__cvta_generic_to_shared(SM_CL + 4 * tid))), "l"(cl_pos_b + 8 * tid)
                     : "memory");
    asm volatile("cp.async.commit_group;" ::: "memory");
}

template <int HC, bool FOLD>
__device__ __forceinline__ float scan_reach(const Ctx& c, const float* r, const float* rf = nullptr, float* total_f = nullptr) {
    csync(c.nc);
    const int hend = HC >= 4 * MAX_TASK_THREADS ? c.HoP : min(c.HoP, 4 * c.nc);
    float4 x = f4zero();
    float lc = 0.f;
    if (c.pos4 < c.HoP) {
        x = *reinterpret_cast<const float4*>(r + c.pos4);
        if (FOLD) {
            const float4 xf = *reinterpret_cast<const float4*>(rf + c.pos4);
            lc = (xf.x + xf.y) + (xf.z + xf.w);
        }
    }
    float y[8], yf[8];
    uint32_t w[4];
    {
        asm volatile("cp.async.wait_group 0;" ::: "memory");
        uint4 u = make_uint4(0x07ff07ffu, 0x07ff07ffu, 0x07ff07ffu, 0x07ff07ffu);
        if (8 * c.tid < 2 * c.HoP) u = *reinterpret_cast<const uint4*>(SM_CL + 4 * c.tid);
        w[0] = u.x;
        w[1] = u.y;
        w[2] = u.z;
        w[3] = u.w;
#pragma unroll
        for (int i = 0; i < 4; ++i) {
            const uint32_t a = w[i] & CL_POS_MASK, b = (w[i] >> 16) & CL_POS_MASK;
            y[2 * i] = a != CL_POS_NONE ? r[a] : 0.f;
            y[2 * i + 1] = b != CL_POS_NONE ? r[b] : 0.f;
            if (FOLD) {
                yf[2 * i] = a != CL_POS_NONE ? rf[a] : 0.f;
                yf[2 * i + 1] = b != CL_POS_NONE ? rf[b] : 0.f;
            }
// ... 330 lines not shown
                        float m, sd;
                        if (ck == CK_FOLD) {
                            m = hand_mass(SM_B, r, total, rec[i]);
                            f4set(acc, i, f4get(acc, i) + cf * m);
                        } else {
                            hand_terms<HC>(c, r, total, rec[i], m, sd);
                            f4set(acc, i, f4get(acc, i) + cf * sd);
                        }
                    }
                }
            }
        }
    }
    if (c.pos4 < c.HpP) stcg4(Rk.cbuf + (size_t(nt.out) * Rk.n_boards + b) * c.HpP + c.pos4, acc);
}

template <int HC, int MODE, int NA, bool XS>
__device__ __forceinline__ void task_down(const TaskArgs& A, const Ctx& c, const NodeTask& nt, const RoundArgs& Rk, int k, int b) {
    const DevRoundPlayer& O = Rk.rp[c.o];
    const uint32_t nrp = O.n_rows_pad[b];
    const float* __restrict__ slab = (MODE == KM_CFR ? O.regrets : O.ssum) + O.board_off[b] + size_t(nrp) * nt.cum_a;
    if (nt.out >= 0) {
        stage_lists_raw<HC>(c.tid, c.HoP, O.cl_pos + size_t(b) * 2 * c.HoP);
        stage_recs<HC>(c, reinterpret_cast<const uint32_t*>(Rk.rp[c.p].hrec) + size_t(b) * 4 * c.HpP);
    }
    const float4 r4 = load_reach4(A, c, nt, Rk, k, b);
    uint32_t rows[4] = {0xffffu, 0xffffu, 0xffffu, 0xffffu};
    if (!O.identity && c.pos4 < c.HoP) unpack4(__ldg(reinterpret_cast<const uint2*>(O.row_of_pos + size_t(b) * c.HoP + c.pos4)), rows);
    float g[4 * NA];
    load_rows<NA>(slab, O.identity != 0, c.pos4, nrp, rows, g);
    float4 v[NA];
    uint32_t xs_slot[4] = {0, 0, 0, 0};
    if (XS && c.pos4 < c.HoP) unpack4(__ldg(reinterpret_cast<const uint2*>(O.slot_of_pos + size_t(b) * c.HoP + c.pos4)), xs_slot);
#pragma unroll
    for (int i = 0; i < 4; ++i) {
        float sg[NA];
        sigma_row<NA>(g, i, sg);
        if (XS) xs_pick<NA>(A, xs_uniform(A.xs_key, nt.an_index, uint32_t(Rk.board_base + b), xs_slot[i]), sg);
        const float r = f4get(r4, i);
#pragma unroll
        for (int a = 0; a < NA; ++a) f4set(v[a], i, r * sg[a]);
    }
    int slot = 0;
#pragma unroll
    for (int a = 0; a < NA; ++a) {
        const int ck = nt.child[a].kind;
        if (c.pos4 < c.HoP) {
            if (ck == CK_FOLD || ck == CK_SHOWDOWN) *reinterpret_cast<float4*>(SM_X + slot * c.Hx + c.pos4) = v[a];
            else if (nt.child[a].buf >= 0) stcg4(Rk.rbuf + (size_t(nt.child[a].buf) * Rk.n_boards + b) * c.HoP + c.pos4, v[a]);
        }
        if (ck == CK_FOLD || ck == CK_SHOWDOWN) ++slot;
    }
    if (nt.out < 0) return;
    down_terminals<HC>(c, nt, Rk, b, NA);
}

template <int HC, int MODE, bool XS>
__device__ __forceinline__ void task_down_generic(const TaskArgs& A, const Ctx& c, const NodeTask& nt, const RoundArgs& Rk, int k, int b) {
    const DevRoundPlayer& O = Rk.rp[c.o];
    const uint32_t nrp = O.n_rows_pad[b];
    const float* __restrict__ slab = (MODE == KM_CFR ? O.regrets : O.ssum) + O.board_off[b] + size_t(nrp) * nt.cum_a;
    const float4 r4 = load_reach4(A, c, nt, Rk, k, b);
    const int n_act = nt.n_act;
    const uint32_t nl_o = O.n_live[b];
    uint32_t rows[4] = {0xffffu, 0xffffu, 0xffffu, 0xffffu};
    if (c.pos4 < c.HoP) unpack4(__ldg(reinterpret_cast<const uint2*>(O.row_of_pos + size_t(b) * c.HoP + c.pos4)), rows);
    if (c.pos4 < c.HoP) {
        for (int i = 0; i < 4; ++i) {
            const bool live = uint32_t(c.pos4 + i) < nl_o && rows[i] != 0xffffu;
            const float r = live ? f4get(r4, i) : 0.f;
            float norm = 0.f;
            if (live)
                for (int a = 0; a < n_act; ++a) norm += fmaxf(slab[size_t(rows[i]) * n_act + a], 0.f);
            int pick = -1;
            if (XS && live) {
                const float u = xs_uniform(A.xs_key, nt.an_index, uint32_t(Rk.board_base + b), O.slot_of_pos[size_t(b) * c.HoP + c.pos4 + i]);
                pick = n_act - 1;
                float cum = 0.f;
                for (int a = 0; a + 1 < n_act; ++a) {
                    cum += norm > 0.f ? fmaxf(slab[size_t(rows[i]) * n_act + a], 0.f) / norm : 1.0f / float(n_act);
                    if (u < cum) {
                        pick = a;
                        break;
                    }
                }
            }
            int slot = 0;
            for (int a = 0; a < n_act; ++a) {
                float v = 0.f;
                if (live) v = norm > 0.f ? r * fmaxf(slab[size_t(rows[i]) * n_act + a], 0.f) / norm : r / float(n_act);
                if (XS && live) v = (a == pick) ? (A.xs_mode == 2 ? v : r) : 0.f;
                const int ck = nt.child[a].kind;
                if (ck == CK_FOLD || ck == CK_SHOWDOWN) SM_X[(slot++) * c.Hx + c.pos4 + i] = v;
                else if (nt.child[a].buf >= 0) __stcg(Rk.rbuf + (size_t(nt.child[a].buf) * Rk.n_boards + b) * c.HoP + c.pos4 + i, v);
            }
        }
    }
    if (nt.out < 0) return;
    stage_lists_raw<HC>(c.tid, c.HoP, O.cl_pos + size_t(b) * 2 * c.HoP);
    stage_recs<HC>(c, reinterpret_cast<const uint32_t*>(Rk.rp[c.p].hrec) + size_t(b) * 4 * c.HpP);
    down_terminals<HC>(c, nt, Rk, b, n_act);
}

template <int HC>
__device__ __forceinline__ void trav_terms(const TaskArgs& A, const Ctx& c, const NodeTask& nt, const RoundArgs& Rk, int k, int b,
                                           bool need_sd, float4& mass, float4& sd) {
    const DevRoundPlayer& Pp = Rk.rp[c.p];
    stage_lists_raw<HC>(c.tid, c.HoP, Rk.rp[c.o].cl_pos + size_t(b) * 2 * c.HoP);
    stage_recs<HC>(c, reinterpret_cast<const uint32_t*>(Pp.hrec) + size_t(b) * 4 * c.HpP);
    const float4 r4 = load_reach4(A, c, nt, Rk, k, b);
    if (c.pos4 < c.HoP) *reinterpret_cast<float4*>(SM_RS + c.pos4) = r4;
    const float total = scan_reach<HC, false>(c, SM_RS);
    mass = f4zero();
    sd = f4zero();
    const uint32_t nl_p = Pp.n_live[b];
    staged_recs_wait();
    if (c.pos4 < c.HpP) {
        uint4 rec[4];
        staged_recs4<HC>(c, rec);
#pragma unroll
        for (int i = 0; i < 4; ++i) {
            if (uint32_t(c.pos4 + i) < nl_p) {
                float m, s = 0.f;
                if (need_sd) hand_terms<HC>(c, SM_RS, total, rec[i], m, s);
                else m = hand_mass(SM_B, SM_RS, total, rec[i]);
                f4set(mass, i, m);
                f4set(sd, i, s);
            }
        }
    }
}

template <int HC>
__device__ __forceinline__ void trav_terms_or_load(const TaskArgs& A, const Ctx& c, const NodeTask& nt, const RoundArgs& Rk, int k, int b,
                                                   bool need_sd, float4& mass, float4& sd) {
    if (!nt.pre_terms) {
        trav_terms<HC>(A, c, nt, Rk, k, b, need_sd, mass, sd);
        return;
    }
    mass = f4zero();
    sd = f4zero();
    if (c.pos4 < c.HpP) {
        const float* m = Rk.cbuf + (size_t(nt.aux) * Rk.n_boards + b) * c.HpP + c.pos4;
        mass = ldcg4(m);
        if (need_sd) sd = ldcg4(m + size_t(Rk.n_boards) * c.HpP);
    }
}

__device__ __forceinline__ float4 rule_factors(const TaskArgs& A) { return ldcg4(A.ctl->rule); }
__device__ __forceinline__ float rule_regret(const float4& f, float r, float d) { return fmaxf((r > 0.f ? f.x : f.y) * r + d, f.w); }

template <int HC, int MODE, int NA, bool DR>
__device__ __forceinline__ void task_trav(const TaskArgs& A, const Ctx& c, const NodeTask& nt, const RoundArgs& Rk, int k, int b) {
    const DevRoundPlayer& Pp = Rk.rp[c.p];
    const float scale = Rk.chance_scale[b];
    float4 dr;
    if (DR) dr = rule_factors(A);
    float4 v[NA];
    bool need_sd = false;
#pragma unroll
    for (int a = 0; a < NA; ++a) {
        v[a] = f4zero();
        need_sd |= (nt.child[a].kind == CK_SHOWDOWN);
    }
    float4 mass, sd;
    trav_terms_or_load<HC>(A, c, nt, Rk, k, b, need_sd, mass, sd);
#pragma unroll
    for (int a = 0; a < NA; ++a)
        if (nt.child[a].kind == CK_VALUE) v[a] = child_value4(A, c, Rk, nt.child[a], b);
#pragma unroll
    for (int a = 0; a < NA; ++a) {
        const int ck = nt.child[a].kind;
        const float cf = nt.child[a].coef * scale;
        if (ck == CK_FOLD) v[a] = make_float4(cf * mass.x, cf * mass.y, cf * mass.z, cf * mass.w);
        else if (ck == CK_SHOWDOWN) v[a] = make_float4(cf * sd.x, cf * sd.y, cf * sd.z, cf * sd.w);
    }
    const uint32_t nrp = Pp.n_rows_pad[b];
    const uint32_t nl_p = Pp.n_live[b];
    float* out = (nt.root_scatter ? Rk.sbuf : Rk.cbuf) + (size_t(nt.out) * Rk.n_boards + b) * c.HpP;
    float* tabR = Pp.regrets + Pp.board_off[b] + size_t(nrp) * nt.cum_a;
    float* tabS = Pp.ssum + Pp.board_off[b] + size_t(nrp) * nt.cum_a;
    if (Pp.identity) {
        if (uint32_t(c.pos4) >= nrp) {
            if (c.pos4 < c.HpP && !nt.root_scatter) stcg4(out + c.pos4, f4zero());
            return;
        }
        const uint32_t none[4] = {0, 0, 0, 0};
        float g[4 * NA], ss[4 * NA];
        if (MODE == KM_CFR) load_rows<NA>(tabR, true, c.pos4, nrp, none, g);
        if (MODE != KM_BR) load_rows<NA>(tabS, true, c.pos4, nrp, none, ss);
        float4 vn4 = f4zero();
#pragma unroll
        for (int i = 0; i < 4; ++i) {
            float sg[NA];
            float vn;
            if (MODE == KM_BR) {
                vn = -3.0e38f;
#pragma unroll
                for (int a = 0; a < NA; ++a) vn = fmaxf(vn, f4get(v[a], i));
            } else {
                if (MODE == KM_CFR) sigma_row<NA>(g, i, sg);
                else sigma_row<NA>(ss, i, sg);
                vn = 0.f;
#pragma unroll
                for (int a = 0; a < NA; ++a) vn += sg[a] * f4get(v[a], i);
            }
            const bool live = uint32_t(c.pos4 + i) < nl_p;
            f4set(vn4, i, live ? vn : 0.f);
            if (MODE == KM_CFR) {
                const float w = f4get(mass, i) * scale;
#pragma unroll
                for (int a = 0; a < NA; ++a) {
                    if (DR) {
                        const float r = g[i * NA + a];
                        if (live) {
                            g[i * NA + a] = rule_regret(dr, r, r > A.prune_threshold ? f4get(v[a], i) - vn : 0.f);
                            ss[i * NA + a] = dr.z * ss[i * NA + a] + sg[a] * w;
                        }
                    } else {
                        g[i * NA + a] += (live && g[i * NA + a] > A.prune_threshold) ? f4get(v[a], i) - vn : 0.f;
                        ss[i * NA + a] += live ? sg[a] * w : 0.f;
                    }
                }
            }
        }
        if (MODE == KM_CFR) {
#pragma unroll
            for (int q = 0; q < NA; ++q) {
                *reinterpret_cast<float4*>(tabR + size_t(c.pos4) * NA + 4 * q) = make_float4(g[4 * q], g[4 * q + 1], g[4 * q + 2], g[4 * q + 3]);
                *reinterpret_cast<float4*>(tabS + size_t(c.pos4) * NA + 4 * q) = make_float4(ss[4 * q], ss[4 * q + 1], ss[4 * q + 2], ss[4 * q + 3]);
            }
        }
        store_value4(c, nt, Rk, b, out, vn4);
        return;
    }
    float* M = SM_X;
    if (c.pos4 < c.HpP) {
        *reinterpret_cast<float4*>(M + c.pos4) = mass;
#pragma unroll
        for (int a = 0; a < NA; ++a) *reinterpret_cast<float4*>(SM_X + (1 + a) * c.Hx + c.pos4) = v[a];
        if (!nt.root_scatter) stcg4(out + c.pos4, f4zero());
    }
    csync(c.nc);
    const uint32_t n_rows = Pp.n_rows[b];
    const uint16_t* __restrict__ rstart = Pp.row_start + size_t(b) * (c.HpP + 4);
    const uint16_t* __restrict__ rpos = Pp.row_pos + size_t(b) * c.HpP;
    const float* V1 = SM_X + c.Hx;
    for (uint32_t row = c.tid; row < n_rows; row += c.nc) {
        float rg[NA], sr[NA], sg[NA], d[NA];
        float norm = 0.f;
#pragma unroll
        for (int a = 0; a < NA; ++a) {
            rg[a] = MODE == KM_CFR ? tabR[size_t(row) * NA + a] : 0.f;
            sr[a] = MODE != KM_BR ? tabS[size_t(row) * NA + a] : 0.f;
            sg[a] = fmaxf(MODE == KM_CFR ? rg[a] : sr[a], 0.f);
            norm += sg[a];
            d[a] = 0.f;
        }
        const float inv = norm > 0.f ? 1.0f / norm : 0.f;
#pragma unroll
        for (int a = 0; a < NA; ++a) sg[a] = norm > 0.f ? sg[a] * inv : 1.0f / float(NA);
        float msum = 0.f;
        const int hs = rstart[row], he = rstart[row + 1];
        for (int q = hs; q < he; ++q) {
            const int h = rpos[q];
            float va[NA];
            float vn = (MODE == KM_BR) ? -3.0e38f : 0.f;
#pragma unroll
            for (int a = 0; a < NA; ++a) {
                va[a] = V1[a * c.Hx + h];
                if (MODE == KM_BR) vn = fmaxf(vn, va[a]);
                else vn += sg[a] * va[a];
            }
            if (MODE == KM_CFR) {
#pragma unroll
                for (int a = 0; a < NA; ++a) d[a] += va[a] - vn;
                msum += M[h];
            }
            store_value1(c, nt, Rk, b, out, h, vn);
        }
        if (MODE == KM_CFR) {
            const float w = msum * scale;
#pragma unroll
            for (int a = 0; a < NA; ++a) {
                if (DR) {
                    tabR[size_t(row) * NA + a] = rule_regret(dr, rg[a], rg[a] > A.prune_threshold ? d[a] : 0.f);
                    tabS[size_t(row) * NA + a] = dr.z * sr[a] + sg[a] * w;
                } else {
                    tabR[size_t(row) * NA + a] = rg[a] + (rg[a] > A.prune_threshold ? d[a] : 0.f);
                    tabS[size_t(row) * NA + a] = sr[a] + sg[a] * w;
                }
            }
        }
    }
}

template <int HC, int MODE, bool DR>
__device__ __forceinline__ void task_trav_generic(const TaskArgs& A, const Ctx& c, const NodeTask& nt, const RoundArgs& Rk, int k, int b) {
    const DevRoundPlayer& Pp = Rk.rp[c.p];
    const float scale = Rk.chance_scale[b];
    float4 dr;
    if (DR) dr = rule_factors(A);
    const int n_act = nt.n_act;
    bool need_sd = false;
    for (int a = 0; a < n_act; ++a) {
        const int ck = nt.child[a].kind;
        if (ck == CK_VALUE && c.pos4 < c.HpP) *reinterpret_cast<float4*>(SM_X + (1 + a) * c.Hx + c.pos4) = child_value4(A, c, Rk, nt.child[a], b);
        need_sd |= (ck == CK_SHOWDOWN);
    }
    float4 mass, sd;
    trav_terms_or_load<HC>(A, c, nt, Rk, k, b, need_sd, mass, sd);
    float* out = (nt.root_scatter ? Rk.sbuf : Rk.cbuf) + (size_t(nt.out) * Rk.n_boards + b) * c.HpP;
    if (c.pos4 < c.HpP) {
        *reinterpret_cast<float4*>(SM_X + c.pos4) = mass;
        for (int a = 0; a < n_act; ++a) {
            const int ck = nt.child[a].kind;
            const float cf = nt.child[a].coef * scale;
            if (ck == CK_FOLD) *reinterpret_cast<float4*>(SM_X + (1 + a) * c.Hx + c.pos4) = make_float4(cf * mass.x, cf * mass.y, cf * mass.z, cf * mass.w);
            else if (ck == CK_SHOWDOWN) *reinterpret_cast<float4*>(SM_X + (1 + a) * c.Hx + c.pos4) = make_float4(cf * sd.x, cf * sd.y, cf * sd.z, cf * sd.w);
        }
        if (!nt.root_scatter) stcg4(out + c.pos4, f4zero());
    }
    csync(c.nc);
    const uint32_t nrp = Pp.n_rows_pad[b];
    const uint32_t n_rows = Pp.n_rows[b];
    float* tabR = Pp.regrets + Pp.board_off[b] + size_t(nrp) * nt.cum_a;
    float* tabS = Pp.ssum + Pp.board_off[b] + size_t(nrp) * nt.cum_a;
    const uint16_t* __restrict__ rstart = Pp.row_start + size_t(b) * (c.HpP + 4);
    const uint16_t* __restrict__ rpos = Pp.row_pos + size_t(b) * c.HpP;
    const float* M = SM_X;
    const float* V1 = SM_X + c.Hx;
    for (uint32_t row = c.tid; row < n_rows; row += c.nc) {
        const float* tsrc = (MODE == KM_EVAL ? tabS : tabR) + size_t(row) * n_act;
        float norm = 0.f;
        if (MODE != KM_BR)
            for (int a = 0; a < n_act; ++a) norm += fmaxf(tsrc[a], 0.f);
        const float inv = norm > 0.f ? 1.0f / norm : 0.f;
        const float uni = 1.0f / float(n_act);
        float msum = 0.f, vsum = 0.f;
        const int hs = rstart[row], he = rstart[row + 1];
        for (int q = hs; q < he; ++q) {
            const int h = rpos[q];
            float vn = (MODE == KM_BR) ? -3.0e38f : 0.f;
            for (int a = 0; a < n_act; ++a) {
                const float va = V1[a * c.Hx + h];
                if (MODE == KM_BR) vn = fmaxf(vn, va);
                else vn += (norm > 0.f ? fmaxf(tsrc[a], 0.f) * inv : uni) * va;
            }
            vsum += vn;
            msum += M[h];
            store_value1(c, nt, Rk, b, out, h, vn);
        }
        if (MODE == KM_CFR) {
            const float w = msum * scale;
            for (int a = 0; a < n_act; ++a) {
                float da = -vsum;
                for (int q = hs; q < he; ++q) da += V1[a * c.Hx + rpos[q]];
                const float old = tabR[size_t(row) * n_act + a];
                const float sga = norm > 0.f ? fmaxf(old, 0.f) * inv : uni;
                if (DR) {
                    tabS[size_t(row) * n_act + a] = dr.z * tabS[size_t(row) * n_act + a] + sga * w;
                    tabR[size_t(row) * n_act + a] = rule_regret(dr, old, old > A.prune_threshold ? da : 0.f);
                } else {
                    tabS[size_t(row) * n_act + a] += sga * w;
                    tabR[size_t(row) * n_act + a] = old + (old > A.prune_threshold ? da : 0.f);
                }
            }
        }
    }
}

__device__ __forceinline__ int board_of(const TaskArgs& A, int k, int inst) {
    return (k > 0 && A.sample_board[k] != nullptr) ? A.sample_board[k][inst] : inst;
}
__device__ __forceinline__ int parent_instance(const TaskArgs& A, const RoundArgs& Rk, int k, int inst, int b) {
    if (A.sample_board[k] == nullptr) return Rk.parent_board[b];
    return k - 1 == 0 ? Rk.parent_board[b] : inst;
}

template <int MODE>
__device__ __forceinline__ void prefetch_task_tables(const TaskArgs& A, uint32_t tk, uint32_t j) {
    const NodeTask* g = A.tasks + j;
    const int kind = g->kind;
    if (kind != TK_DOWN && kind != TK_UP_TRAV) return;
    const RoundArgs& Rk = A.rounds[g->round_k];
    const int b = board_of(A, g->round_k, int(tk - g->first));
    const int q = kind == TK_DOWN ? 1 - A.trav : A.trav;
    const DevRoundPlayer& D = Rk.rp[q];
    const uint32_t nrp = D.n_rows_pad[b];
// ... 220 lines not shown
                    default: task_trav_generic<HC, MODE, DR>(A, c, nt, Rk, k, b); break;
                }
                break;
            }
            case TK_UP_OPP: {
                if (c.pos4 < c.HpP) {
                    float4 v = nt.aux >= 0 ? ldcg4(Rk.cbuf + (size_t(nt.aux) * Rk.n_boards + b) * c.HpP + c.pos4) : f4zero();
                    for (int a = 0; a < nt.n_act; ++a)
                        if (nt.child[a].kind == CK_VALUE) v = f4add(v, child_value4(A, c, Rk, nt.child[a], b));
                    store_value4(c, nt, Rk, b, (nt.root_scatter ? Rk.sbuf : Rk.cbuf) + (size_t(nt.out) * Rk.n_boards + b) * c.HpP, v);
                }
                break;
            }
            case TK_GATHER: {
                if (c.pos4 < c.HpP) {
                    const RoundArgs& Rn = A.rounds[k + 1];
                    const float* base = Rn.sbuf + size_t(nt.aux) * Rn.n_boards * c.HpP + c.pos4;
                    float4 acc = f4zero();
                    if (A.sample_board[k + 1] != nullptr) {
                        const int32_t* sb = A.sample_board[k + 1];
                        const int s0 = k == 0 ? 0 : inst, ns = k == 0 ? A.n_paths : 1;
                        for (int i = 0; i < ns; ++i) acc = f4add(acc, ldcg4(base + size_t(sb[s0 + i]) * c.HpP));
                        const float w = A.gather_scale[k];
                        acc = make_float4(acc.x * w, acc.y * w, acc.z * w, acc.w * w);
                    } else {
                        const int cb0 = Rk.per_parent > 0 ? b * Rk.per_parent : 0;
                        const int ncb = Rk.per_parent > 0 ? Rk.per_parent : Rk.n_boards_next;
                        const float* src = base + size_t(cb0) * c.HpP;
                        for (int i0 = 0; i0 < ncb; i0 += 8) {
                            float4 val[8];
#pragma unroll
                            for (int u = 0; u < 8; ++u) val[u] = (i0 + u < ncb) ? ldcg4(src + size_t(i0 + u) * c.HpP) : f4zero();
#pragma unroll
                            for (int u = 0; u < 8; ++u) acc = f4add(acc, val[u]);
                        }
                    }
                    stcg4(Rk.gathered + (size_t(nt.out) * Rk.n_boards + b) * c.HpP + c.pos4, acc);
                }
                if (A.xch_world > 1 && k + 1 == A.xch_round) {
                    const uint32_t ep = s_slot[buf].xseq;
                    const size_t vec = ((size_t(ep & 1u) * A.xch_leaves + nt.out) * Rk.n_boards + b) * A.xch_world;
                    if (c.pos4 < c.HpP) {
                        const float4 part = ldcg4(Rk.gathered + (size_t(nt.out) * Rk.n_boards + b) * c.HpP + c.pos4);
                        for (int peer = 0; peer < A.xch_world; ++peer)
                            *reinterpret_cast<float4*>(A.xch_peer[peer] + (vec + A.xch_rank) * c.HpP + c.pos4) = part;
                    }
                    __threadfence_system();
                    csync(c.nc);
                    if (tid < A.xch_world) {
                        st_release_sys_u32(A.xflag_peer[tid] + vec + A.xch_rank, ep);
                        const uint32_t* mine = A.xflag_peer[A.xch_rank] + vec + tid;
                        const unsigned long long t_wait = global_ns();
                        uint32_t spins = 0;
                        while (ld_acquire_sys_u32(mine) != ep) {
                            __nanosleep(100);
                            spins += 31;
                            if (wait_gives_up(A, t_wait, spins)) break;
                        }
                    }
                    csync(c.nc);
                    if (c.pos4 < c.HpP) {
                        const float* src = A.xch_peer[A.xch_rank] + vec * c.HpP + c.pos4;
                        float4 acc = f4zero();
                        for (int r = 0; r < A.xch_world; ++r) acc = f4add(acc, ldcg4(src + size_t(r) * c.HpP));
                        stcg4(Rk.gathered + (size_t(nt.out) * Rk.n_boards + b) * c.HpP + c.pos4, acc);
                    }
                }
                break;
            }
            case TK_TRAV_TERMS: {
                bool need_sd = false;
                for (int a = 0; a < nt.n_act; ++a) need_sd |= (nt.child[a].kind == CK_SHOWDOWN);
                float4 mass, sd;
                trav_terms<HC>(A, c, nt, Rk, k, b, need_sd, mass, sd);
                if (c.pos4 < c.HpP) {
                    float* m = Rk.cbuf + (size_t(nt.out) * Rk.n_boards + b) * c.HpP + c.pos4;
                    stcg4(m, mass);
                    stcg4(m + size_t(Rk.n_boards) * c.HpP, sd);
                }
                break;
            }
            case TK_ROOT_SHOWDOWN: {
                float4 mass, sd;
                trav_terms<HC>(A, c, nt, Rk, k, b, true, mass, sd);
                const float cf = nt.child[0].coef * Rk.chance_scale[b];
                if (c.pos4 < c.HpP)
                    store_value4(c, nt, Rk, b, (nt.root_scatter ? Rk.sbuf : Rk.cbuf) + (size_t(nt.out) * Rk.n_boards + b) * c.HpP,
                                 make_float4(cf * sd.x, cf * sd.y, cf * sd.z, cf * sd.w));
                break;
            }
            case TK_CHANCE_DOWN: {
                const float4 r4 = load_reach4(A, c, nt, Rk, k, b);
                if (c.pos4 < c.HoP) stcg4(Rk.rbuf + (size_t(nt.aux) * Rk.n_boards + b) * c.HoP + c.pos4, r4);
                break;
            }
            case TK_CHANCE_UP: {
                if (c.pos4 < c.HpP)
                    store_value4(c, nt, Rk, b, (nt.root_scatter ? Rk.sbuf : Rk.cbuf) + (size_t(nt.out) * Rk.n_boards + b) * c.HpP,
                                 ldcg4(Rk.gathered + (size_t(nt.aux) * Rk.n_boards + b) * c.HpP + c.pos4));
                break;
            }
            default: break;
        }
#ifdef RS_TASK_TIMING
        if (tid == 0 && A.timing) {
            atomicAdd(A.timing + kind * 4 + 0, 1ull);
            atomicAdd(A.timing + kind * 4 + 2, (unsigned long long)(clock64() - tm1));
            unsigned long long gt1;
            asm volatile("mov.u64 %0, %globaltimer;" : "=l"(gt1));
            atomicMax(A.timing + 32 + (kind * 3 + k) * 2 + 1, gt1);
        }
#endif
        __syncwarp();
        if (c.lane == 0) mbar_arrive(&s_done);
        buf ^= 1;
    }
}

__global__ void scale_kernel(float* __restrict__ data, size_t n, float d) {
    const size_t n4 = n / 4;
    float4* v4 = reinterpret_cast<float4*>(data);
    const size_t stride = size_t(gridDim.x) * blockDim.x;
    for (size_t i = size_t(blockIdx.x) * blockDim.x + threadIdx.x; i < n4; i += stride) {
        float4 v = v4[i];
        v.x *= d;
        v.y *= d;
        v.z *= d;
        v.w *= d;
        v4[i] = v;
    }
    if (blockIdx.x == 0 && threadIdx.x < n - n4 * 4) data[n4 * 4 + threadIdx.x] *= d;
}

__global__ void set_rule_kernel(TaskCtl* ctl, float4 f) { *reinterpret_cast<float4*>(ctl->rule) = f; }

__global__ void normalize_kernel(const float* __restrict__ in, float* __restrict__ out, uint32_t n_rows, uint32_t A) {
    const uint32_t row = blockIdx.x * blockDim.x + threadIdx.x;
    if (row >= n_rows) return;
    float norm = 0.f;
    for (uint32_t a = 0; a < A; ++a) norm += fmaxf(in[size_t(row) * A + a], 0.f);
    for (uint32_t a = 0; a < A; ++a)
        out[size_t(row) * A + a] = norm > 0.f ? fmaxf(in[size_t(row) * A + a], 0.f) / norm : 1.0f / float(A);
}

__global__ void unpermute_kernel(const float* __restrict__ in, const uint16_t* __restrict__ slot_of_pos, const uint32_t* __restrict__ n_live,
                                 float* __restrict__ out, uint32_t hp, uint32_t H) {
    const uint32_t b = blockIdx.y;
    const uint32_t pos = blockIdx.x * blockDim.x + threadIdx.x;
    if (pos < n_live[b]) out[size_t(b) * H + slot_of_pos[size_t(b) * hp + pos]] = in[size_t(b) * hp + pos];
}

}

size_t task_kernel_smem_bytes(bool wide, int slots, int Hp_pad, int Ho_pad) {
    const int hx = Hp_pad > Ho_pad ? Hp_pad : Ho_pad;
    const int hc = 4 * (wide ? 352 : 288);
    size_t floats = size_t(smem_fixed_floats(hc)) + size_t(slots) * hx;
    return floats * sizeof(float);
}

template <int MAXT, int MINB>
static cudaError_t configure_for(size_t smem, int threads, int* blocks_per_sm) {
    cudaError_t e;
    e = cudaFuncSetAttribute(task_kernel<KM_CFR, MAXT, MINB, false>, cudaFuncAttributeMaxDynamicSharedMemorySize, int(smem));
    if (e != cudaSuccess) return e;
    e = cudaFuncSetAttribute(task_kernel<KM_CFR, MAXT, MINB, true>, cudaFuncAttributeMaxDynamicSharedMemorySize, int(smem));
    if (e != cudaSuccess) return e;
    e = cudaFuncSetAttribute(task_kernel<KM_CFR_DR, MAXT, MINB, false>, cudaFuncAttributeMaxDynamicSharedMemorySize, int(smem));
    if (e != cudaSuccess) return e;
    e = cudaFuncSetAttribute(task_kernel<KM_CFR_DR, MAXT, MINB, true>, cudaFuncAttributeMaxDynamicSharedMemorySize, int(smem));
    if (e != cudaSuccess) return e;
    e = cudaFuncSetAttribute(task_kernel<KM_BR, MAXT, MINB, false>, cudaFuncAttributeMaxDynamicSharedMemorySize, int(smem));
    if (e != cudaSuccess) return e;
    e = cudaFuncSetAttribute(task_kernel<KM_EVAL, MAXT, MINB, false>, cudaFuncAttributeMaxDynamicSharedMemorySize, int(smem));
    if (e != cudaSuccess) return e;
    int n = 0, m = 0, x = 0;
    e = cudaOccupancyMaxActiveBlocksPerMultiprocessor(&n, task_kernel<KM_CFR, MAXT, MINB, false>, threads + 32, smem);
    if (e != cudaSuccess) return e;
    e = cudaOccupancyMaxActiveBlocksPerMultiprocessor(&m, task_kernel<KM_BR, MAXT, MINB, false>, threads + 32, smem);
    if (e != cudaSuccess) return e;
    e = cudaOccupancyMaxActiveBlocksPerMultiprocessor(&x, task_kernel<KM_CFR, MAXT, MINB, true>, threads + 32, smem);
    if (e != cudaSuccess) return e;
    n = n < x ? n : x;
    *blocks_per_sm = n < m ? n : m;
    return cudaSuccess;
}

cudaError_t configure_task_kernels(size_t smem, int threads, bool wide, int* blocks_per_sm) {
    if (threads <= 288 && !wide) return configure_for<288, RS_MIN_BLOCKS_288>(smem, threads, blocks_per_sm);
    return configure_for<352, RS_MIN_BLOCKS_352>(smem, threads, blocks_per_sm);
}

template <int MAXT, int MINB>
static void launch_for(const TaskArgs& a, int mode, int grid, int threads, size_t smem, cudaStream_t st) {
    switch (mode) {
        case KM_CFR: task_kernel<KM_CFR, MAXT, MINB, false><<<grid, threads + 32, smem, st>>>(a); break;
        case KM_CFR_XS: task_kernel<KM_CFR, MAXT, MINB, true><<<grid, threads + 32, smem, st>>>(a); break;
        case KM_CFR_DR: task_kernel<KM_CFR_DR, MAXT, MINB, false><<<grid, threads + 32, smem, st>>>(a); break;
        case KM_CFR_XS_DR: task_kernel<KM_CFR_DR, MAXT, MINB, true><<<grid, threads + 32, smem, st>>>(a); break;
        case KM_BR: task_kernel<KM_BR, MAXT, MINB, false><<<grid, threads + 32, smem, st>>>(a); break;
        default: task_kernel<KM_EVAL, MAXT, MINB, false><<<grid, threads + 32, smem, st>>>(a); break;
    }
}

cudaError_t launch_task_kernel(const TaskArgs& a, int mode, int grid, int threads, bool wide, size_t smem, cudaStream_t st) {
    if (grid <= 0 || a.t1 <= a.t0) return cudaSuccess;
    if (threads <= 288 && !wide) launch_for<288, RS_MIN_BLOCKS_288>(a, mode, grid, threads, smem, st);
    else launch_for<352, RS_MIN_BLOCKS_352>(a, mode, grid, threads, smem, st);
    return cudaGetLastError();
}

cudaError_t launch_scale(float* data, size_t n, float d, cudaStream_t st) {
    if (n == 0) return cudaSuccess;
    const int threads = 256;
    size_t blocks = (n / 4 + threads - 1) / threads;
    if (blocks < 1) blocks = 1;
    if (blocks > 148 * 16) blocks = 148 * 16;
    scale_kernel<<<unsigned(blocks), threads, 0, st>>>(data, n, d);
    return cudaGetLastError();
}

cudaError_t launch_set_rule(TaskCtl* ctl, const float f[4], cudaStream_t st) {
    set_rule_kernel<<<1, 1, 0, st>>>(ctl, make_float4(f[0], f[1], f[2], f[3]));
    return cudaGetLastError();
}

cudaError_t launch_unpermute(const float* in, const uint16_t* slot_of_pos, const uint32_t* n_live, float* out, uint32_t n_boards, uint32_t hp,
                             uint32_t H, cudaStream_t st) {
    if (n_boards == 0) return cudaSuccess;
    unpermute_kernel<<<dim3((hp + 255) / 256, n_boards), 256, 0, st>>>(in, slot_of_pos, n_live, out, hp, H);
    return cudaGetLastError();
}

cudaError_t launch_normalize(const float* in, float* out, uint32_t n_rows, uint32_t A, cudaStream_t st) {
    if (n_rows == 0) return cudaSuccess;
    normalize_kernel<<<(n_rows + 255) / 256, 256, 0, st>>>(in, out, n_rows, A);
    return cudaGetLastError();
}

}
```

### rustsolver_b200/csrc/kernels.cuh

```cuda
#pragma once
#include <cuda_runtime.h>
#include <stdint.h>

#include "plan.h"
#include "tasks.h"

namespace rs {

constexpr int MAX_ACTIONS = MAX_TASK_CHILDREN;
constexpr int RS_MAX_PEERS = 8;
constexpr int FAST_ACTIONS = 4;
constexpr int MAX_TASK_THREADS = 352;

enum KernelMode { KM_CFR = 0, KM_BR = 1, KM_EVAL = 2, KM_CFR_XS = 3, KM_CFR_DR = 4, KM_CFR_XS_DR = 5 };

__host__ __device__ inline float xs_uniform(unsigned long long key, uint32_t an_index, uint32_t board, uint32_t slot) {
    unsigned long long z = key ^ ((unsigned long long)an_index << 44) ^ ((unsigned long long)board << 20) ^ (unsigned long long)slot;
    z = (z ^ (z >> 30)) * 0xBF58476D1CE4E5B9ull;
    z = (z ^ (z >> 27)) * 0x94D049BB133111EBull;
    z ^= z >> 31;
    return float(uint32_t(z >> 40)) * (1.0f / 16777216.0f);
}

struct DevRoundPlayer {
    const uint16_t* row_of_pos;
    const uint16_t* row_start;
    const uint16_t* row_pos;
    const uint16_t* cl_pos;
    const uint16_t* parent_pos;
    const uint16_t* child_pos;
    const uint16_t* slot_of_pos;
    const HandRec* hrec;
    const uint32_t* n_rows;
    const uint32_t* n_rows_pad;
    const uint32_t* n_live;
    const uint64_t* board_off;
    float* regrets;
    float* ssum;
    int identity;
    int pad;
};

struct RoundArgs {
    DevRoundPlayer rp[2];
    const float* chance_scale;
    const int32_t* parent_board;
    float* rbuf;
    float* cbuf;
    float* sbuf;
    float* gathered;
    int n_boards;
    int per_parent;
    int n_boards_next;
    int board_base;
};

struct TaskArgs {
    RoundArgs rounds[3];
    const NodeTask* tasks;
    const TaskSrc* srcs;
    const uint32_t* task_of_ticket;
    const uint32_t* order;
    uint32_t n_tasks;
    uint32_t* flags;
    TaskCtl* ctl;
    const float* root_weights[2];
    int H[2], Hpad[2];
    int trav;
    int HpP, HoP, Hx;
    uint32_t t0, t1;
    const int32_t* sample_board[3];
    int n_paths;
    float gather_scale[3];
    int slots;
    float prune_threshold;
    float* xch_peer[RS_MAX_PEERS];
    uint32_t* xflag_peer[RS_MAX_PEERS];
    int xch_world, xch_rank;
    int xch_round;
    int xch_leaves;
    unsigned long long xs_key;
    int xs_mode;
    int xch_bump;
    const volatile uint32_t* host_abort;
    unsigned long long wait_timeout_ns;
    unsigned long long* timing;
};

size_t task_kernel_smem_bytes(bool wide, int slots, int Hp_pad, int Ho_pad);
cudaError_t configure_task_kernels(size_t smem, int threads, bool wide, int* blocks_per_sm);
cudaError_t launch_task_kernel(const TaskArgs& a, int mode, int grid, int threads, bool wide, size_t smem, cudaStream_t st);

cudaError_t launch_scale(float* data, size_t n, float d, cudaStream_t st);
cudaError_t launch_set_rule(TaskCtl* ctl, const float f[4], cudaStream_t st);
cudaError_t launch_normalize(const float* in, float* out, uint32_t n_rows, uint32_t A, cudaStream_t st);
cudaError_t launch_unpermute(const float* in, const uint16_t* slot_of_pos, const uint32_t* n_live, float* out, uint32_t n_boards, uint32_t hp,
                             uint32_t H, cudaStream_t st);

}
```

### rustsolver_b200/csrc/plan.cpp

```cpp
#include "plan.h"

#include <algorithm>
#include <cstring>
#include <functional>
#include <numeric>
#include <unordered_map>

#include <cstdlib>

#include "hand_indexer.h"
#include "poker.h"

namespace rs {

namespace {

struct Builder {
    const rs_tree* t;
    Plan* P;
    std::string err;
    uint32_t max_round = 0;

    bool fail(const std::string& m) {
        if (err.empty()) err = m;
// ... 1276 lines not shown
                for (uint32_t i = 0; i < L.n_live[b]; ++i) {
                    for (int w = 0; w < 2; ++w) {
                        const int c = P->hand_cards[q][2 * sop[i] + w];
                        cl[fill[c]++] = uint16_t(i);
                        if (final_round) seg_str[q][c].push_back(P->sd[q].strength[size_t(b) * H + sop[i]]);
                    }
                }
                uint32_t n_lists = 0;
                for (int c = 0; c < 52; ++c) {
                    seg_ord[q][c] = -1;
                    if (seg_start[q][c + 1] > seg_start[q][c]) {
                        seg_ord[q][c] = int(n_lists++);
                        cl[seg_start[q][c]] |= uint16_t(CL_FIRST);
                    }
                }
                {
                    uint32_t started = 0;
                    const uint32_t n_entries = 2 * L.Hpad;
                    for (uint32_t e = 0; e < n_entries; e += 8) {
                        const uint32_t ord = e == 0 ? n_lists : started;
                        cl[e] |= uint16_t((ord & 7u) << 11);
                        cl[e + 1] |= uint16_t(((ord >> 3) & 7u) << 11);
                        for (uint32_t x = e; x < e + 8 && x < n_entries; ++x)
                            if (cl[x] & CL_FIRST) ++started;
                    }
                }
                if (k > 0) {
                    const LocalTables& Lp = P->loc[k - 1][q];
                    const uint32_t pb = uint32_t(P->board_parent[k][b]);
                    uint16_t* pp = &L.parent_pos[size_t(b) * L.Hpad];
                    uint16_t* cp = &L.child_pos[size_t(b) * Lp.Hpad];
                    for (uint32_t i = 0; i < L.n_live[b]; ++i) {
                        const uint16_t ppos = Lp.pos_of_slot[size_t(pb) * H + sop[i]];
                        pp[i] = ppos;
                        cp[ppos] = uint16_t(i);
                    }
                }
            }
            for (int q = 0; q < 2; ++q) {
                const int o = 1 - q;
                LocalTables& L = P->loc[k][q];
                const LocalTables& Lo = P->loc[k][o];
                const uint32_t H = P->H[q], Ho = P->H[o];
                const uint16_t* sop = &L.slot_of_pos[size_t(b) * L.Hpad];
                std::vector<uint32_t> ostr;
                if (final_round) {
                    ostr.resize(Lo.n_live[b]);
                    for (uint32_t i = 0; i < Lo.n_live[b]; ++i)
                        ostr[i] = P->sd[o].strength[size_t(b) * Ho + Lo.slot_of_pos[size_t(b) * Lo.Hpad + i]];
                }
                for (uint32_t i = 0; i < L.n_live[b]; ++i) {
                    const uint32_t h = sop[i];
                    const int c0 = P->hand_cards[q][2 * h], c1 = P->hand_cards[q][2 * h + 1];
                    uint32_t lo = 0, hi = 0, ab[2][2] = {{0, 0}, {0, 0}}, kk[2] = {HREC_K_NONE, HREC_K_NONE}, same4 = HREC_SAME_NONE;
                    const int cc[2] = {c0, c1};
                    const uint16_t sm = P->same[q][h];
                    if (sm != 0xFFFF) {
                        const uint16_t op = Lo.pos_of_slot[size_t(b) * Ho + sm];
                        if (op < Lo.n_live[b]) same4 = uint32_t(op) * 4u;
                    }
                    const uint32_t st = final_round ? P->sd[q].strength[size_t(b) * H + h] : 0;
                    if (final_round) {
                        lo = uint32_t(std::lower_bound(ostr.begin(), ostr.end(), st) - ostr.begin());
                        hi = uint32_t(std::upper_bound(ostr.begin(), ostr.end(), st) - ostr.begin());
                    }
                    for (int w = 0; w < 2; ++w) {
                        const int c = cc[w];
                        if (seg_ord[o][c] < 0) continue;
                        kk[w] = uint32_t(seg_ord[o][c]) * 4u;
                        const uint32_t s0 = seg_start[o][c];
                        uint32_t dlo = 0, dhi = 0;
                        if (final_round) {
                            const auto& l = seg_str[o][c];
                            dlo = uint32_t(std::lower_bound(l.begin(), l.end(), st) - l.begin());
                            dhi = uint32_t(std::upper_bound(l.begin(), l.end(), st) - l.begin());
                        }
                        ab[w][0] = (s0 + dlo) * 4u;
                        ab[w][1] = (s0 + dhi) * 4u;
                    }
                    HandRec r;
                    r.w0 = (lo * 4u) | ((hi * 4u) << 16);
                    r.w1 = ab[0][0] | (ab[0][1] << 16);
                    r.w2 = ab[1][0] | (ab[1][1] << 16);
                    r.w3 = kk[0] | (kk[1] << 9) | (same4 << 18);
                    L.hrec[size_t(b) * L.Hpad + i] = r;
                }
            }
        }
    }

    if (any_showdown) {
        const uint32_t k = P->n_rounds - 1;
        const uint32_t nB = P->n_boards[k];
        bool same = P->H[0] == P->H[1];
        for (int q = 0; q < 2; ++q) {
            LocalTables& L = P->loc[k][q];
            L.pcards.assign(size_t(nB) * L.Hpad, 0);
            for (uint32_t b = P->local_lo[k]; b < P->local_hi[k]; ++b) {
                const uint16_t* sop = &L.slot_of_pos[size_t(b) * L.Hpad];
                for (uint32_t i = 0; i < L.n_live[b]; ++i) {
                    L.pcards[size_t(b) * L.Hpad + i] = uint16_t(P->hand_cards[q][2 * sop[i]] | (P->hand_cards[q][2 * sop[i] + 1] << 8));
                    if ((L.hrec[size_t(b) * L.Hpad + i].w3 >> 18) != i * 4u) same = false;
                }
                if (L.n_live[b] != P->loc[k][1 - q].n_live[b]) same = false;
            }
        }
        P->same_order = same;
    }

    for (int p = 0; p < 2; ++p) {
        TaskGen g{P, p};
        if (!g.run()) return fail(g.err);
        P->tl[p] = std::move(g.tl);
        P->street[p] = std::move(g.sp);
    }

    for (uint32_t k = 0; k < P->n_rounds; ++k)
        for (int q = 0; q < 2; ++q) {
            const RoundPlayerTables& T = P->tabs[k][q];
            for (uint32_t b = P->local_lo[k]; b < P->local_hi[k]; ++b)
                P->updates_per_iter_local += uint64_t(T.n_rows[b]) * T.sum_a;
        }
    P->updates_per_iter_global = P->updates_per_iter_local;
    return true;
}

void materialize_tasks(const Plan& P, int trav, const uint32_t counts[3], MaterializedTasks* out) {
    const TaskList& tl = P.tl[trav];
    std::vector<NodeTask>& t = out->tasks;
    std::vector<TaskSrc>& sr = out->srcs;
    t = tl.tasks;
    sr = tl.srcs;
    uint32_t first = 0;
    out->phase_cut = 0;
    bool cut_set = false;
    for (size_t j = 0; j < t.size(); ++j) {
        if (!cut_set && tl.tasks[j].first >= tl.phase_cut) {
            out->phase_cut = first;
            cut_set = true;
        }
        t[j].first = first;
        t[j].count = counts[t[j].round_k];
        first += t[j].count;
    }
    if (!cut_set) out->phase_cut = first;
    out->n_tickets = first;
    for (NodeTask& x : t)
        for (int i = 0; i < x.n_dep; ++i)
            if (x.dep[i] >= 0) x.dep[i] = int32_t(t[x.dep[i]].first);
    for (TaskSrc& x : sr)
        if (x.dep >= 0) x.dep = int32_t(t[x.dep].first);
}

bool build_execution_order(const Plan& P, int trav, const MaterializedTasks& m, const uint32_t counts[3], bool force, std::vector<uint32_t>* ord,
                           std::string* err) {
    ord->clear();
    const std::vector<NodeTask>& t = m.tasks;
    const uint32_t kf = P.n_rounds - 1;
    if (P.n_rounds < 2 || counts[kf] != P.boards_local(kf)) return true;
    const TaskList& tlp = P.tl[trav];
    const uint64_t vec_bytes = (uint64_t(tlp.n_rbuf[kf]) + tlp.n_cbuf[kf]) * counts[kf] * std::max(P.H[0], P.H[1]) * 4;
    uint32_t lo = UINT32_MAX, hi = 0;
    std::vector<uint32_t> fin;
    for (size_t j = 0; j < t.size(); ++j)
        if (t[j].round_k == kf && t[j].count) {
            fin.push_back(uint32_t(j));
            lo = std::min(lo, t[j].first);
            hi = std::max(hi, t[j].first + t[j].count);
        }
    uint64_t covered = 0;
    for (uint32_t j : fin) covered += t[j].count;
    const bool contiguous = !fin.empty() && covered == uint64_t(hi - lo);
    if (!contiguous || !(vec_bytes > (96ull << 20) || force)) return true;
    ord->resize(m.n_tickets);
    for (uint32_t i = 0; i < m.n_tickets; ++i) (*ord)[i] = i;
    const int32_t* par = P.board_parent[kf].data() + P.local_lo[kf];
    uint32_t pos = lo;
    for (uint32_t b0 = 0; b0 < counts[kf];) {
        uint32_t b1 = b0 + 1;
        while (b1 < counts[kf] && par[b1] == par[b0]) ++b1;
        for (uint32_t j : fin)
            for (uint32_t b = b0; b < b1; ++b) (*ord)[pos++] = t[j].first + b;
        b0 = b1;
    }
    if (pos != hi) {
        if (err) *err = "internal: execution order does not cover the final round";
        return false;
    }
    return true;
}

std::string check_execution_order(const Plan& P, int trav, const MaterializedTasks& m, const uint32_t counts[3], const std::vector<uint32_t>& ord) {
    (void)trav;
    const uint32_t n = m.n_tickets;
    std::vector<uint32_t> pos(n);
    if (ord.empty()) {
        for (uint32_t i = 0; i < n; ++i) pos[i] = i;
    } else {
        if (ord.size() != n) return "order has the wrong length";
        std::vector<uint8_t> seen(n, 0);
        for (uint32_t tk = 0; tk < n; ++tk) {
            if (ord[tk] >= n || seen[ord[tk]]) return "order is not a permutation (ticket " + std::to_string(tk) + ")";
            seen[ord[tk]] = 1;
            pos[ord[tk]] = tk;
        }
    }
    auto bad = [&](uint32_t producer, uint32_t slot, size_t j) -> std::string {
        if (producer >= n) return "task " + std::to_string(j) + ": producer slot " + std::to_string(producer) + " out of range";
        if (pos[producer] >= pos[slot])
            return "task " + std::to_string(j) + " slot " + std::to_string(slot) + " (ticket " + std::to_string(pos[slot]) + ") runs before its producer slot " +
                   std::to_string(producer) + " (ticket " + std::to_string(pos[producer]) + ")";
        return "";
    };
    for (size_t j = 0; j < m.tasks.size(); ++j) {
        const NodeTask& st = m.tasks[j];
        const uint32_t k = st.round_k;
        for (uint32_t inst = 0; inst < st.count; ++inst) {
            const uint32_t slot = st.first + inst, b = inst;
            if (st.kind == TK_GATHER) {
                const bool sharded_next = P.world > 1 && k + 1 == P.shard_round;
                const uint32_t per_parent = sharded_next ? 0u : P.deal_count[k + 1];
                const uint32_t gfirst = uint32_t(st.dep[0]) + (per_parent > 0 ? b * per_parent : 0u);
                const uint32_t total = per_parent > 0 ? per_parent : counts[k + 1];
                for (uint32_t c = 0; c < total; ++c) {
                    const std::string e = bad(gfirst + c, slot, j);
                    if (!e.empty()) return e;
                }
                continue;
            }
            for (int i = 0; i < st.n_dep; ++i) {
                if (st.dep[i] < 0) continue;
                uint32_t off = inst;
                if (st.dep_kind[i] == DK_PARENT_BOARD) off = uint32_t(P.board_parent[k][P.local_lo[k] + b] - int32_t(P.local_lo[k - 1]));
                const std::string e = bad(uint32_t(st.dep[i]) + off, slot, j);
                if (!e.empty()) return e;
            }
            for (uint32_t s = 0; s < st.n_src_all; ++s) {
                const int32_t d = m.srcs[st.src_all_first + s].dep;
                if (d < 0) continue;
                const std::string e = bad(uint32_t(d) + inst, slot, j);
                if (!e.empty()) return e;
            }
        }
    }
    return "";
}

}
```

### rustsolver_b200/csrc/plan.h

```cpp
#pragma once
#include <cstdint>
#include <string>
#include <vector>

#include "../../include/b200cfr.h"
#include "street.h"
#include "tasks.h"

namespace rs {

struct TaskList {
    std::vector<NodeTask> tasks;
    std::vector<TaskSrc> srcs;
    uint32_t n_tickets = 0;
    uint32_t phase_cut = 0;
    uint32_t n_rbuf[3] = {0, 0, 0};
    uint32_t n_cbuf[3] = {0, 0, 0};
    uint32_t n_sbuf[3] = {0, 0, 0};
    uint32_t max_children = 1;
    uint32_t max_terminal = 0;
    int32_t root_cbuf = -1;
};

struct PNode {
    uint8_t kind;
    uint8_t player = 0;
    uint8_t round_k = 0;
    uint8_t last_to_act = 0;
    uint32_t value = 0;
    uint32_t an_index = 0;
    int32_t src_node = -1;
    int32_t tab_j = -1;
    uint32_t cum_a = 0;
    int32_t leaf_id = -1;
    int32_t parent = -1;
    int32_t depth = 0;
    std::vector<int32_t> children;
};
enum { PK_ACTION = 0, PK_FOLD = 1, PK_SHOWDOWN = 2, PK_CHANCE = 3 };

struct Segment {
    int32_t root = -1;
    std::vector<int32_t> leaves;
};

struct RoundPlayerTables {
    uint32_t n_nodes = 0;
    std::vector<uint32_t> node_an_index;
    std::vector<uint32_t> node_n_act;
    uint32_t sum_a = 0;
    std::vector<uint16_t> row_of_hand;
    std::vector<uint16_t> row_start;
    std::vector<uint16_t> row_hands;
    std::vector<uint32_t> n_rows;
    std::vector<uint64_t> board_off;
};

struct LocalTables {
    uint32_t Hpad = 0;
    bool identity = true;
    std::vector<uint16_t> slot_of_pos;
    std::vector<uint16_t> pos_of_slot;
    std::vector<uint32_t> n_live;
    std::vector<uint16_t> row_of_pos;
    std::vector<uint16_t> row_start;
    std::vector<uint16_t> row_pos;
    std::vector<uint32_t> n_rows_pad;
    std::vector<HandRec> hrec;
    std::vector<uint16_t> cl_pos;
    std::vector<uint16_t> parent_pos;
    std::vector<uint16_t> child_pos;
    std::vector<uint16_t> pcards;
};

struct ShowdownTables {
    std::vector<uint16_t> sorted;
    std::vector<uint32_t> n_live;
    std::vector<uint32_t> cls;
    std::vector<uint32_t> strength;
};

struct Plan {
    uint32_t n_rounds = 0;
    uint32_t first_round = 0;
    uint32_t n_sub = 1;
    uint32_t H[2] = {0, 0};
    std::vector<uint8_t> hand_cards[2];
    std::vector<uint16_t> same[2];
    std::vector<uint16_t> card_hands[2];

    uint32_t n_boards[3] = {0, 0, 0};
    uint32_t deal_count[3] = {0, 0, 0};
    std::vector<uint64_t> board_mask[3];
    std::vector<int32_t> board_parent[3];
    std::vector<uint8_t> board_card[3];
    std::vector<float> chance_scale[3];
    std::vector<uint64_t> n_combos;

    int32_t rank = 0, world = 1;
    uint32_t shard_round = 0;
    uint32_t local_lo[3] = {0, 0, 0}, local_hi[3] = {0, 0, 0};

    std::vector<PNode> nodes;
    std::vector<Segment> segs[3];
    RoundPlayerTables tabs[3][2];
    ShowdownTables sd[2];
    LocalTables loc[3][2];
    std::vector<int32_t> an_to_pnode;
    TaskList tl[2];
    StreetPlan street[2];
    bool same_order = false;

    uint64_t updates_per_iter_local = 0, updates_per_iter_global = 0;
    uint32_t flags = 0;

    uint32_t boards_local(uint32_t k) const { return local_hi[k] - local_lo[k]; }
};

struct MaterializedTasks {
    std::vector<NodeTask> tasks;
    std::vector<TaskSrc> srcs;
    uint32_t n_tickets = 0, phase_cut = 0;
};
void materialize_tasks(const Plan& P, int trav, const uint32_t counts[3], MaterializedTasks* out);
bool build_execution_order(const Plan& P, int trav, const MaterializedTasks& m, const uint32_t counts[3], bool force, std::vector<uint32_t>* ord,
                           std::string* err);
std::string check_execution_order(const Plan& P, int trav, const MaterializedTasks& m, const uint32_t counts[3], const std::vector<uint32_t>& ord);

class HandIndexer;
typedef bool (*BatchIndexFn)(const HandIndexer& ix, const uint8_t* cards, size_t n, uint64_t* out, std::string* err);

bool compile_plan(const rs_tree* tree, const rs_ranges* ranges, const rs_abstraction* abs,
                  const rs_config* cfg, const uint64_t* board_masks, uint32_t n_sub, Plan* out,
                  std::string* err, BatchIndexFn batch_index = nullptr);

}
```

### rustsolver_b200/solver.py

```python
from __future__ import annotations

import ctypes as C
from dataclasses import dataclass, field
from typing import List, Optional, Sequence

import numpy as np

from . import _lib
from ._lib import (EngineError, check, f32p, f64p, i32p, rs_abstraction, rs_config, rs_ranges,
                   rs_round_abstraction, rs_stats, rs_tree, rs_update_rule, u8p, u16p, u32p, u64p)

RS_ABS_NONE, RS_ABS_ISOMORPHIC, RS_ABS_CLUSTER_ARR, RS_ABS_BUCKET_TABLE = 0, 1, 2, 3
RS_FLAG_NO_GRAPH = 1
RS_FLAG_NO_CHAIN_SPLIT = 2
RS_FLAG_STREET_KERNEL = 4
RS_FLAG_SHARD_ISOLATED = 8
RS_RULE_VANILLA, RS_RULE_DCFR, RS_RULE_LCFR, RS_RULE_CFR_PLUS = 0, 1, 2, 3
NODE_ACTION, NODE_TERMINAL, NODE_PUBLIC_CHANCE, NODE_PRIVATE_CHANCE = 0, 1, 2, 3
TERM_ALLIN, TERM_SHOWDOWN, TERM_UNCONTESTED = 0, 1, 2
ACTION_NAMES = {0: "Bet", 1: "Raise", 2: "Check", 3: "Call", 4: "Fold"}


def _ptr(a: np.ndarray, t):
    return a.ctypes.data_as(t)
# ... 290 lines not shown
        assert a.ndim == 2 and a.shape[1] == sum(self.cards_per_round)
        out = np.zeros(len(a), dtype=np.uint64)
        self._lib.rsh_indexer_index_many(self._h, _ptr(a, u8p), len(a), _ptr(out, u64p))
        return out

    def index_many_gpu(self, cards: np.ndarray, return_ms: bool = False):
        assert len(self.cards_per_round) == 2 and self.cards_per_round[0] == 2
        a = np.ascontiguousarray(cards, dtype=np.uint8)
        assert a.ndim == 2 and a.shape[1] == sum(self.cards_per_round)
        out = np.zeros(len(a), dtype=np.uint64)
        ms = C.c_float(0.0)
        check(self._lib.rs_gpu_index_hands(self.cards_per_round[1], _ptr(a, u8p), len(a), _ptr(out, u64p), C.byref(ms)))
        return (out, float(ms.value)) if return_ms else out

    def get_hand(self, round: int, index: int) -> List[int]:
        n = sum(self.cards_per_round[:round + 1])
        out = np.zeros(n, dtype=np.uint8)
        check(self._lib.rsh_indexer_get_hand(self._h, round, index, _ptr(out, u8p)))
        return [int(x) for x in out]


@dataclass
class CardAbstraction:
    kind: int = RS_ABS_NONE
    cluster_arr: Optional[np.ndarray] = None
    bucket_table: Optional[List[np.ndarray]] = None

    @staticmethod
    def ISOMORPHIC():
        return CardAbstraction(RS_ABS_ISOMORPHIC)

    @staticmethod
    def NONE():
        return CardAbstraction(RS_ABS_NONE)

    @staticmethod
    def from_file(path: str):
        return CardAbstraction(RS_ABS_CLUSTER_ARR, cluster_arr=np.fromfile(path, dtype="<u4"))


def _abstraction_struct(card_abs: Sequence[CardAbstraction], keep: list) -> rs_abstraction:
    ab = rs_abstraction()
    ab.n_rounds = len(card_abs)
    for k, ca in enumerate(card_abs):
        ra = ab.rounds[k]
        ra.kind = ca.kind
        if ca.kind == RS_ABS_CLUSTER_ARR:
            arr = np.ascontiguousarray(ca.cluster_arr, dtype=np.uint32)
            keep.append(arr)
            ra.cluster_arr = _ptr(arr, u32p)
            ra.cluster_arr_len = len(arr)
        if ca.kind == RS_ABS_BUCKET_TABLE:
            for p in range(2):
                arr = np.ascontiguousarray(ca.bucket_table[p], dtype=np.uint32)
                keep.append(arr)
                ra.bucket_table[p] = _ptr(arr, u32p)
    return ab


def nccl_unique_id() -> bytes:
    buf = (C.c_uint8 * _lib.RS_NCCL_ID_BYTES)()
    check(_lib.load().rs_nccl_unique_id(buf))
    return bytes(buf)


class _PlanOrEngine:
    _prefix = "rs_"

    def _fn(self, name):
        return getattr(self._lib, self._prefix + name)

    def board_id(self, round_idx: int, dealt: Sequence[int]) -> int:
        a = np.asarray(list(dealt) + [0], dtype=np.uint8)
        out = C.c_uint32()
        check(self._fn("board_id")(self._h, round_idx, _ptr(a, u8p), len(dealt), C.byref(out)))
        return out.value

    def card_table(self, round_idx: int, player: int, board_id: int) -> np.ndarray:
        out = np.zeros(self.n_hands[player], dtype=np.uint16)
        nr = C.c_uint32()
        check(self._fn("card_table")(self._h, round_idx, player, board_id, _ptr(out, u16p), len(out), C.byref(nr)))
        return out

    def num_rows(self, round_idx: int, player: int, board_id: int) -> int:
        nr = C.c_uint32()
        check(self._fn("card_table")(self._h, round_idx, player, board_id, None, 0, C.byref(nr)))
        return nr.value


class Plan(_PlanOrEngine):
    _prefix = "rs_plan_"

    def __init__(self, tree: GameTree, ranges: Sequence[np.ndarray], board_mask: int,
                 card_abs: Sequence[CardAbstraction] = (), board_masks: Optional[Sequence[int]] = None,
                 rank: int = 0, world_size: int = 1, flags: int = 0):
        self._lib = _lib.load()
        self._keep = []
        tv = tree.view()
        rr = rs_ranges()
        hs = [np.ascontiguousarray(r, dtype=np.uint8) for r in ranges]
        for p in range(2):
            rr.n_hands[p] = len(hs[p])
            rr.hands[p] = _ptr(hs[p], u8p)
        ab = _abstraction_struct(card_abs, self._keep)
        cfg = rs_config()
        cfg.board_mask = board_mask
        cfg.rank, cfg.world_size = rank, world_size
        cfg.flags = flags
        h = C.c_void_p()
        if board_masks is not None:
            bm = np.asarray(board_masks, dtype=np.uint64)
            check(self._lib.rs_plan_create(C.byref(tv), C.byref(rr), C.byref(ab), C.byref(cfg), _ptr(bm, u64p), len(bm), C.byref(h)))
        else:
            check(self._lib.rs_plan_create(C.byref(tv), C.byref(rr), C.byref(ab), C.byref(cfg), None, 0, C.byref(h)))
        self._h = h
        self.n_hands = [len(hs[0]), len(hs[1])]

    def __del__(self):
        if getattr(self, "_h", None):
            self._lib.rs_plan_destroy(self._h)
            self._h = None

    def stats(self) -> rs_stats:
        s = rs_stats()
        check(self._lib.rs_plan_stats(self._h, C.byref(s)))
        return s

    def infoset_offset(self, an_index: int, board_id: int):
        off, nr, na = C.c_uint64(), C.c_uint32(), C.c_uint32()
        check(self._lib.rs_plan_infoset_offset(self._h, an_index, board_id, C.byref(off), C.byref(nr), C.byref(na)))
        return off.value, nr.value, na.value

    def showdown_order(self, player: int, board_id: int):
        order = np.zeros(self.n_hands[player], dtype=np.uint16)
        cls = np.zeros(self.n_hands[player], dtype=np.uint32)
        nl = C.c_uint32()
        check(self._lib.rs_plan_showdown_order(self._h, player, board_id, _ptr(order, u16p), _ptr(cls, u32p), len(order), C.byref(nl)))
        return order[:nl.value].copy(), cls[:nl.value].copy()

    def check_execution_order(self, traverser: int, force_board_major: bool = False):
        n, moved = C.c_uint32(), C.c_uint32()
        check(self._lib.rs_plan_check_execution_order(self._h, traverser, int(force_board_major), C.byref(n), C.byref(moved)))
        return int(n.value), int(moved.value)

    def local_tables(self, round_idx: int, player: int, board_id: int):
        dims = (C.c_uint32 * 2)()
        check(self._lib.rs_plan_local_tables(self._h, round_idx, player, board_id, None, None, None, dims))
        hp, nl = int(dims[0]), int(dims[1])
        rec = np.zeros((hp, 4), dtype=np.uint32)
        cl = np.zeros(2 * hp, dtype=np.uint16)
        sop = np.zeros(hp, dtype=np.uint16)
        check(self._lib.rs_plan_local_tables(self._h, round_idx, player, board_id, _ptr(rec, u32p), _ptr(cl, u16p), _ptr(sop, u16p), dims))
        return rec, cl, sop, nl

    def street_info(self, traverser: int) -> dict:
        out = (C.c_uint32 * 8)()
        check(self._lib.rs_plan_street_info(self._h, traverser, out))
        keys = ("eligible", "segments", "max_rows", "max_slots", "max_q_sd", "max_q_mo", "down_ops", "up_ops")
        d = dict(zip(keys, [int(x) for x in out]))
        d["why"] = "" if d["eligible"] else self._lib.rs_last_error().decode()
        return d

    def street_program(self, traverser: int, board_id: int) -> dict:
        n = C.c_uint32()
        dims = (C.c_uint32 * 4)()
        check(self._lib.rs_plan_street_program(self._h, traverser, board_id, None, 0, C.byref(n), None, 0, dims))
        words = np.zeros(max(n.value, 1), dtype=np.uint32)
        hinfo = np.zeros(2 * dims[2], dtype=np.uint32)
        check(self._lib.rs_plan_street_program(self._h, traverser, board_id, _ptr(words, u32p), len(words), C.byref(n),
                                               _ptr(hinfo, u32p), len(hinfo), dims))
        ls, cs = int(dims[0]), int(dims[1])
        return {"lists": words[:ls * 208].reshape(ls, 208), "chunks": words[ls * 208:ls * 208 + cs * 128].reshape(cs, 128),
                "hinfo": hinfo.reshape(-1, 2), "HpP": int(dims[2]), "HoP": int(dims[3])}


def sample_runouts(seed: int, board_mask: int, n_cards: int, n_paths: int, distinct_first: bool = True) -> np.ndarray:
    out = np.zeros((n_paths, n_cards), dtype=np.uint8)
    check(_lib.load().rs_sample_runouts(seed, board_mask, n_cards, n_paths, int(distinct_first), _ptr(out, u8p)))
    return out


class Engine(_PlanOrEngine):

    def __init__(self, tree: GameTree, ranges: Sequence[np.ndarray], board_mask: int,
                 card_abs: Sequence[CardAbstraction] = (), board_masks: Optional[Sequence[int]] = None,
                 device: int = 0, rank: int = 0, world_size: int = 1, nccl_id: Optional[bytes] = None,
                 flags: int = 0, threads_per_block: int = 0, discount_interval: int = 0, discount_cap: int = 0):
        self._lib = _lib.load()
        self._keep = []
        self.tree = tree
        tv = tree.view()
        rr = rs_ranges()
        hs = [np.ascontiguousarray(r, dtype=np.uint8) for r in ranges]
        for p in range(2):
            rr.n_hands[p] = len(hs[p])
            rr.hands[p] = _ptr(hs[p], u8p)
        ab = _abstraction_struct(card_abs, self._keep)
        cfg = rs_config()
        cfg.board_mask = board_mask
        cfg.device, cfg.rank, cfg.world_size = device, rank, world_size
        if nccl_id is not None:
            C.memmove(cfg.nccl_id, nccl_id, _lib.RS_NCCL_ID_BYTES)
        cfg.flags = flags
        cfg.threads_per_block = threads_per_block
        cfg.discount_interval, cfg.discount_cap = discount_interval, discount_cap
        h = C.c_void_p()
        if board_masks is not None:
            bm = np.asarray(board_masks, dtype=np.uint64)
            check(self._lib.rs_create_batch(C.byref(tv), C.byref(rr), C.byref(ab), C.byref(cfg), _ptr(bm, u64p), len(bm), C.byref(h)))
        else:
            check(self._lib.rs_create(C.byref(tv), C.byref(rr), C.byref(ab), C.byref(cfg), C.byref(h)))
        self._h = h
        self.n_hands = [len(hs[0]), len(hs[1])]
        self.ranges = hs

    def close(self):
        if getattr(self, "_h", None):
            self._lib.rs_destroy(self._h)
            self._h = None

    __del__ = close

    def iterate(self, n: int = 1):
        check(self._lib.rs_iterate(self._h, n))

    def iterate_sampled(self, paths):
        a = np.ascontiguousarray(paths, dtype=np.uint8)
        if a.ndim == 1:
            a = a.reshape(1, -1)
        check(self._lib.rs_iterate_sampled(self._h, _ptr(a, u8p), a.shape[0]))

    def discount(self, d: float):
        check(self._lib.rs_discount(self._h, d))

    def reset(self):
        check(self._lib.rs_reset(self._h))

    def stats(self) -> rs_stats:
        s = rs_stats()
        check(self._lib.rs_stats_get(self._h, C.byref(s)))
        return s

    def _shape(self, an_index: int, board_id: int):
        nr, na = C.c_uint32(), C.c_uint32()
        check(self._lib.rs_read_infoset(self._h, an_index, board_id, None, None, 0, C.byref(nr), C.byref(na)))
        return nr.value, na.value

    def read_infoset(self, an_index: int, board_id: int = 0):
        nr, na = self._shape(an_index, board_id)
        r = np.zeros((nr, na), dtype=np.float32)
        s = np.zeros((nr, na), dtype=np.float32)
        check(self._lib.rs_read_infoset(self._h, an_index, board_id, _ptr(r, f32p), _ptr(s, f32p), r.size, None, None))
        return r, s

    def write_infoset(self, an_index: int, board_id: int, regrets: np.ndarray, strategy_sum: np.ndarray):
        r = np.ascontiguousarray(regrets, dtype=np.float32)
        s = np.ascontiguousarray(strategy_sum, dtype=np.float32)
        check(self._lib.rs_write_infoset(self._h, an_index, board_id, _ptr(r, f32p), _ptr(s, f32p), r.size))

    def average_strategy(self, an_index: int, board_id: int = 0) -> np.ndarray:
        nr, na = self._shape(an_index, board_id)
        out = np.zeros((nr, na), dtype=np.float32)
        check(self._lib.rs_average_strategy(self._h, an_index, board_id, _ptr(out, f32p), out.size, None, None))
        return out

    def current_strategy(self, an_index: int, board_id: int = 0) -> np.ndarray:
        nr, na = self._shape(an_index, board_id)
        out = np.zeros((nr, na), dtype=np.float32)
        check(self._lib.rs_current_strategy(self._h, an_index, board_id, _ptr(out, f32p), out.size, None, None))
        return out

    def set_range_weights(self, player: int, weights: np.ndarray):
        w = np.ascontiguousarray(weights, dtype=np.float32)
        check(self._lib.rs_set_range_weights(self._h, player, _ptr(w, f32p), w.size))

    def profile_iteration(self):
        cap = 64
        buf = (_lib.rs_kernel_time * cap)()
        n = C.c_uint32()
        check(self._lib.rs_profile_iteration(self._h, buf, cap, C.byref(n)))
        kinds = {0: "traversal", 1: "street", 3: "allreduce"}
        return [dict(kind=kinds[buf[i].kind], phase=buf[i].phase, traverser=buf[i].traverser, grid=buf[i].grid,
                     ms=buf[i].ms, table_bytes=buf[i].table_bytes, vector_bytes=buf[i].vector_bytes) for i in range(n.value)]

    def dump_average_strategy(self, path: str) -> int:
        n = C.c_uint64(0)
        check(self._lib.rs_dump_average_strategy(self._h, str(path).encode(), C.byref(n)))
        return int(n.value)

    def set_prune_threshold(self, threshold: float):
        check(self._lib.rs_set_prune_threshold(self._h, float(threshold)))

    def set_opponent_sampling(self, mode: int, seed: int = 0):
        check(self._lib.rs_set_opponent_sampling(self._h, int(mode), int(seed)))

    def set_update_rule(self, kind: int, alpha: float = 1.5, beta: float = 0.0, gamma: float = 2.0):
        r = rs_update_rule(int(kind), float(alpha), float(beta), float(gamma))
        check(self._lib.rs_set_update_rule(self._h, C.byref(r)))

    def update_rule(self):
        r, t = rs_update_rule(), C.c_uint64()
        check(self._lib.rs_get_update_rule(self._h, C.byref(r), C.byref(t)))
        return r.kind, r.alpha, r.beta, r.gamma, int(t.value)

    def set_wait_timeout_ms(self, ms: int):
        check(self._lib.rs_set_wait_timeout_ms(self._h, int(ms)))
# ... 87 lines not shown
```

Measured before the change: 21.73.

## Size 288-thread task kernel shared memory per run and set carveout for occupancy

Task runs are now computed in the plan, with per-run slot counts and hand widths, so the 288-thread build gets only the shared memory its runs actually need instead of the wide-kernel worst case. The kernel attributes now also set a preferred shared-memory carveout based on the minimum blocks per SM. In task_trav, the chance scale and table pointer computations are deferred past the terms load for smaller builds to cut register pressure. This could raise blocks per SM for small-street kernels. The trade-off is extra bookkeeping, plus an added error path when a run exceeds the configured shared memory.

```diff
diff --git a/include/b200cfr.h b/include/b200cfr.h
--- a/include/b200cfr.h
+++ b/include/b200cfr.h
@@ -92,6 +92,7 @@
     uint32_t n_boards_local[3];
     uint32_t n_hands[2];
     uint64_t n_combos;
+    uint32_t task_blocks_per_sm[2];
 } rs_stats;
 
 const char* rs_last_error(void);
@@ -217,6 +218,7 @@
 int rs_plan_check_execution_order(const rs_plan* p, uint32_t traverser, int force_board_major, uint32_t* n_tickets_out,
                                   uint32_t* n_moved_out);
 int rs_plan_street_info(const rs_plan* p, uint32_t traverser, uint32_t out[8]);
+int rs_plan_task_runs(const rs_plan* p, uint32_t traverser, uint32_t* words_out, size_t cap, uint32_t* n_runs_out);
 int rs_plan_street_program(const rs_plan* p, uint32_t traverser, uint32_t board_id, uint32_t* words_out, size_t cap,
                            uint32_t* n_words_out, uint32_t* hinfo_out, size_t hinfo_cap, uint32_t dims_out[4]);
 
diff --git a/rustsolver_b200/_lib.py b/rustsolver_b200/_lib.py
--- a/rustsolver_b200/_lib.py
+++ b/rustsolver_b200/_lib.py
@@ -50,7 +50,8 @@
                 ("updates_per_iteration_global", C.c_uint64), ("device_ms", C.c_double),
                 ("kernel_launches", C.c_uint64), ("table_bytes", C.c_uint64), ("n_rounds", C.c_uint32),
                 ("n_boards", C.c_uint32 * 3), ("n_boards_local", C.c_uint32 * 3),
-                ("n_hands", C.c_uint32 * 2), ("n_combos", C.c_uint64)]
+                ("n_hands", C.c_uint32 * 2), ("n_combos", C.c_uint64),
+                ("task_blocks_per_sm", C.c_uint32 * 2)]
 
 
 class rs_update_rule(C.Structure):
@@ -121,6 +122,7 @@
     "rs_plan_local_tables": (C.c_int, [VP, C.c_uint32, C.c_uint32, C.c_uint32, u32p, u16p, u16p, u32p]),
     "rs_plan_check_execution_order": (C.c_int, [VP, C.c_uint32, C.c_int, u32p, u32p]),
     "rs_plan_street_info": (C.c_int, [VP, C.c_uint32, u32p]),
+    "rs_plan_task_runs": (C.c_int, [VP, C.c_uint32, u32p, C.c_size_t, C.POINTER(C.c_uint32)]),
     "rs_plan_street_program": (C.c_int, [VP, C.c_uint32, C.c_uint32, u32p, C.c_size_t, u32p, u32p, C.c_size_t, u32p]),
 }
 HOST_API = {
diff --git a/rustsolver_b200/csrc/engine.cu b/rustsolver_b200/csrc/engine.cu
--- a/rustsolver_b200/csrc/engine.cu
+++ b/rustsolver_b200/csrc/engine.cu
@@ -133,11 +133,7 @@
     uint32_t n_tickets = 0, phase_cut = 0, n_tasks = 0;
     uint32_t street_lo = 0, street_hi = 0;
     uint32_t street_inst = 0;
-    struct Run {
-        uint32_t t0, t1;
-        int threads;
-    };
-    std::vector<Run> runs;
+    std::vector<TaskRun> runs;
     uint32_t xch_lo = 0, xch_hi = 0;
     struct Section {
         uint32_t first;
@@ -202,13 +198,13 @@
     size_t st_stride = 0, st_smem = 0;
     int st_XP = 0, st_rows = 0, st_vy_rows = 0, st_vm_rows = 0, st_slots = 0, st_threads = 0, st_blocks_per_sm = 1, st_qs = 1, st_qm = 1;
     int slots = 1;
-    size_t smem_bytes = 0;
-    size_t smem_small = 0;
-    int blocks_per_sm = 1, n_sms = 148;
+    int n_sms = 148;
     int round_threads[3] = {0, 0, 0};
-    int bps_small = 0;
+    size_t build_smem[2] = {0, 0};
+    int build_bps[2] = {0, 0};
     bool wide_for(int thr, uint64_t tickets) const {
-        return thr > 288 || bps_small == 0 || getenv("RS_WIDE_ONLY") || (tickets <= uint64_t(n_sms) * blocks_per_sm && !getenv("RS_SMALL_ONLY"));
+        return thr > 288 || build_bps[TB_288] == 0 || getenv("RS_WIDE_ONLY") ||
+               (tickets <= uint64_t(n_sms) * build_bps[TB_WIDE] && !getenv("RS_SMALL_ONLY"));
     }
     std::vector<rs_kernel_time>* prof = nullptr;
     std::vector<std::pair<cudaEvent_t, cudaEvent_t>> prof_events;
@@ -296,16 +292,8 @@
     const int HP[2] = {int((P.H[0] + 3) & ~3u), int((P.H[1] + 3) & ~3u)};
     const size_t maxHP = size_t(std::max(HP[0], HP[1]));
     const bool street_wanted = P.street[0].eligible && P.street[1].eligible;
-    threads = int(((maxHP / 4) + 31) / 32 * 32);
+    task_round_threads(P, getenv("RS_UNIFORM_BLOCK") != nullptr, &threads, round_threads);
     if (threads > MAX_TASK_THREADS) return set_err(RS_ERR_UNSUPPORTED, "range larger than 1326 hands");
-    for (uint32_t k = 0; k < P.n_rounds; ++k) {
-        round_threads[k] = threads;
-        if (!P.board_mask[k].empty() && !getenv("RS_UNIFORM_BLOCK")) {
-            const int left = 52 - __builtin_popcountll(P.board_mask[k][0]);
-            const size_t live_max = std::min<size_t>(maxHP, size_t(left) * size_t(left - 1) / 2);
-            round_threads[k] = std::min(threads, int((((live_max + 3) / 4) + 31) / 32 * 32));
-        }
-    }
     n_sms = prop.multiProcessorCount;
     if (street_wanted) {
         int rc = init_street();
@@ -395,21 +383,22 @@
         *abort_host = 0;
         CU(cudaHostGetDevicePointer(reinterpret_cast<void**>(&abort_dev), abort_host, 0));
     }
-    size_t smem_need = std::max(task_kernel_smem_bytes(true, slots, HP[0], HP[1]), task_kernel_smem_bytes(true, slots, HP[1], HP[0]));
+    const size_t smem_need = task_kernel_smem_bytes(TB_WIDE, slots, int(maxHP));
     int max_optin = 0;
     CU(cudaDeviceGetAttribute(&max_optin, cudaDevAttrMaxSharedMemoryPerBlockOptin, device));
     if (smem_need > size_t(max_optin))
         return set_err(RS_ERR_UNSUPPORTED, "node too wide for one CTA's shared memory: need " +
                                                std::to_string(smem_need) + " B, device allows " + std::to_string(max_optin));
-    smem_bytes = smem_need;
-    CU(configure_task_kernels(smem_need, threads, true, &blocks_per_sm));
-    if (blocks_per_sm < 1) return set_err(RS_ERR_UNSUPPORTED, "task kernel does not fit on an SM");
-    for (uint32_t k = 0; k < P.n_rounds; ++k)
-        if (round_threads[k] <= 288 && bps_small == 0) {
-            smem_small = std::max(task_kernel_smem_bytes(false, slots, HP[0], HP[1]), task_kernel_smem_bytes(false, slots, HP[1], HP[0]));
-            CU(configure_task_kernels(smem_small, 288, false, &bps_small));
-            if (bps_small < 1) return set_err(RS_ERR_UNSUPPORTED, "task kernel does not fit on an SM");
-        }
+    build_smem[TB_WIDE] = smem_need;
+    CU(configure_task_kernels(TB_WIDE, smem_need, threads, &build_bps[TB_WIDE]));
+    if (build_bps[TB_WIDE] < 1) return set_err(RS_ERR_UNSUPPORTED, "task kernel does not fit on an SM");
+    for (int p = 0; p < 2; ++p)
+        for (const TaskRun& r : full[p].runs)
+            if (r.threads <= 288) build_smem[TB_288] = std::max(build_smem[TB_288], task_kernel_smem_bytes(TB_288, r.slots, r.hx));
+    if (build_smem[TB_288]) {
+        CU(configure_task_kernels(TB_288, build_smem[TB_288], 288, &build_bps[TB_288]));
+        if (build_bps[TB_288] < 1) return set_err(RS_ERR_UNSUPPORTED, "task kernel does not fit on an SM");
+    }
     n_sms = prop.multiProcessorCount;
     CU(scratch.alloc(size_t(1326) * MAX_ACTIONS));
 
@@ -587,7 +576,7 @@
             if (!fin && seen) closed = true;
         }
     }
-    out->runs.clear();
+    task_runs(plan, trav, mt, round_threads, &out->runs);
     out->sections.clear();
     out->xch_lo = out->xch_hi = 0;
     for (const NodeTask& x : t) {
@@ -596,9 +585,6 @@
             if (out->xch_hi == out->xch_lo) out->xch_lo = x.first;
             out->xch_hi = x.first + x.count;
         }
-        const int thr = round_threads[x.round_k];
-        if (out->runs.empty() || out->runs.back().threads != thr) out->runs.push_back({x.first, x.first + x.count, thr});
-        else out->runs.back().t1 = x.first + x.count;
         const bool up = x.kind == TK_UP_TRAV, down = x.kind == TK_DOWN;
         if (up || down) {
             bool seen = false;
@@ -767,12 +753,12 @@
         if (sp.kind == 0) {
             struct Piece {
                 uint32_t t0, t1;
-                int threads;
+                const TaskRun* run;
             };
             std::vector<Piece> pieces;
-            for (const TaskSet::Run& r : set->runs) {
+            for (const TaskRun& r : set->runs) {
                 const uint32_t lo = std::max(sp.t0, r.t0), hi = std::min(sp.t1, r.t1);
-                if (lo < hi) pieces.push_back({lo, hi, r.threads});
+                if (lo < hi) pieces.push_back({lo, hi, &r});
             }
             size_t longest = 0;
             for (size_t i = 1; i < pieces.size(); ++i)
@@ -782,10 +768,19 @@
                 a.t0 = pieces[i].t0;
                 a.t1 = pieces[i].t1;
                 a.xch_bump = (fused_exchange && set->xch_lo < set->xch_hi && a.t0 <= set->xch_lo && set->xch_lo < a.t1) ? 1 : 0;
-                const int thr = pieces[i].threads;
-                const bool wide = wide_for(thr, a.t1 - a.t0);
-                const int grid = int(std::min<uint64_t>(uint64_t(a.t1 - a.t0), uint64_t(n_sms) * (wide ? blocks_per_sm : bps_small)));
-                CU(launch_task_kernel(a, mode, grid, thr, wide, wide ? smem_bytes : smem_small, stream));
+                const TaskRun& r = *pieces[i].run;
+                const int build = wide_for(r.threads, a.t1 - a.t0) ? TB_WIDE : TB_288;
+                size_t smem = build_smem[TB_WIDE];
+                a.slots = slots;
+                a.Hx = std::max(a.HpP, a.HoP);
+                if (build == TB_288) {
+                    smem = task_kernel_smem_bytes(TB_288, r.slots, r.hx);
+                    a.slots = r.slots;
+                    a.Hx = r.hx;
+                    if (smem > build_smem[TB_288]) return set_err(RS_ERR_INVALID, "internal: a run needs more shared memory than the 288-thread build was configured for");
+                }
+                const int grid = int(std::min<uint64_t>(uint64_t(a.t1 - a.t0), uint64_t(n_sms) * build_bps[build]));
+                CU(launch_task_kernel(a, mode, grid, r.threads, build, smem, stream));
                 uint64_t bytes = 0;
                 for (const TaskSet::Section& sc : set->sections)
                     if (sc.first >= a.t0 && sc.first < a.t1) {
@@ -1717,6 +1712,32 @@
     return RS_OK;
 }
 
+int rs_plan_task_runs(const rs_plan* p, uint32_t traverser, uint32_t* words_out, size_t cap, uint32_t* n_runs_out) {
+    if (!p || !n_runs_out || traverser > 1) return set_err(RS_ERR_INVALID, "bad argument");
+    const Plan& P = p->p;
+    uint32_t counts[3] = {0, 0, 0};
+    for (uint32_t k = 0; k < P.n_rounds; ++k) counts[k] = P.boards_local(k);
+    MaterializedTasks mt;
+    materialize_tasks(P, int(traverser), counts, &mt);
+    int all = 0, rt[3];
+    task_round_threads(P, getenv("RS_UNIFORM_BLOCK") != nullptr, &all, rt);
+    std::vector<TaskRun> runs;
+    task_runs(P, int(traverser), mt, rt, &runs);
+    *n_runs_out = uint32_t(runs.size());
+    if (!words_out) return RS_OK;
+    if (cap < 6 * runs.size()) return set_err(RS_ERR_INVALID, "output buffer too small");
+    int slots = 1;
+    for (int q = 0; q < 2; ++q) slots = std::max(slots, int(std::max(P.tl[q].max_terminal, 1 + P.tl[q].max_children)));
+    const int hmax = int(std::max((P.H[0] + 3) & ~3u, (P.H[1] + 3) & ~3u));
+    for (size_t i = 0; i < runs.size(); ++i) {
+        const TaskRun& r = runs[i];
+        const size_t smem = r.threads > 288 ? task_kernel_smem_bytes(TB_WIDE, slots, hmax) : task_kernel_smem_bytes(TB_288, r.slots, r.hx);
+        const uint32_t w[6] = {r.t0, r.t1, uint32_t(r.threads), uint32_t(r.slots), uint32_t(r.hx), uint32_t(smem)};
+        memcpy(words_out + 6 * i, w, sizeof(w));
+    }
+    return RS_OK;
+}
+
 int rs_plan_street_info(const rs_plan* p, uint32_t traverser, uint32_t out[8]) {
     if (!p || !out || traverser > 1) return set_err(RS_ERR_INVALID, "bad argument");
     const StreetPlan& S = p->p.street[traverser];
@@ -1872,7 +1893,8 @@
     out->kernel_launches = e->e.launches;
     out->table_bytes = e->e.table_bytes;
     out->updates_per_iteration_global = e->e.updates_global;
-    return RS_OK;
-}
-
-}
+    for (int b = 0; b < 2; ++b) out->task_blocks_per_sm[b] = uint32_t(e->e.build_bps[b]);
+    return RS_OK;
+}
+
+}
diff --git a/rustsolver_b200/csrc/kernels.cu b/rustsolver_b200/csrc/kernels.cu
--- a/rustsolver_b200/csrc/kernels.cu
+++ b/rustsolver_b200/csrc/kernels.cu
@@ -1,4 +1,5 @@
 #include "kernels.cuh"
+#include <algorithm>
 
 #ifndef RS_MIN_BLOCKS_288
 #define RS_MIN_BLOCKS_288 3
@@ -635,8 +636,9 @@
 
 template <int HC, int MODE, int NA, bool DR>
 __device__ __forceinline__ void task_trav(const TaskArgs& A, const Ctx& c, const NodeTask& nt, const RoundArgs& Rk, int k, int b) {
+    constexpr bool LATE = HC < 4 * MAX_TASK_THREADS;
     const DevRoundPlayer& Pp = Rk.rp[c.p];
-    const float scale = Rk.chance_scale[b];
+    float scale = LATE ? 0.f : Rk.chance_scale[b];
     float4 dr;
     if (DR) dr = rule_factors(A);
     float4 v[NA];
@@ -648,6 +650,7 @@
     }
     float4 mass, sd;
     trav_terms_or_load<HC>(A, c, nt, Rk, k, b, need_sd, mass, sd);
+    if (LATE) scale = Rk.chance_scale[b];
 #pragma unroll
     for (int a = 0; a < NA; ++a)
         if (nt.child[a].kind == CK_VALUE) v[a] = child_value4(A, c, Rk, nt.child[a], b);
@@ -660,18 +663,23 @@
     }
     const uint32_t nrp = Pp.n_rows_pad[b];
     const uint32_t nl_p = Pp.n_live[b];
-    float* out = (nt.root_scatter ? Rk.sbuf : Rk.cbuf) + (size_t(nt.out) * Rk.n_boards + b) * c.HpP;
-    float* tabR = Pp.regrets + Pp.board_off[b] + size_t(nrp) * nt.cum_a;
-    float* tabS = Pp.ssum + Pp.board_off[b] + size_t(nrp) * nt.cum_a;
+    auto out_vec = [&]() { return (nt.root_scatter ? Rk.sbuf : Rk.cbuf) + (size_t(nt.out) * Rk.n_boards + b) * c.HpP; };
+    float* const out0 = LATE ? nullptr : out_vec();
+    float* const tabR0 = LATE ? nullptr : Pp.regrets + Pp.board_off[b] + size_t(nrp) * nt.cum_a;
+    float* const tabS0 = LATE ? nullptr : Pp.ssum + Pp.board_off[b] + size_t(nrp) * nt.cum_a;
+    const size_t toff = LATE ? Pp.board_off[b] + size_t(nrp) * nt.cum_a : 0;
+    auto out_p = [&]() { return LATE ? out_vec() : out0; };
+    auto tabR_p = [&]() { return LATE ? Pp.regrets + toff : tabR0; };
+    auto tabS_p = [&]() { return LATE ? Pp.ssum + toff : tabS0; };
     if (Pp.identity) {
         if (uint32_t(c.pos4) >= nrp) {
-            if (c.pos4 < c.HpP && !nt.root_scatter) stcg4(out + c.pos4, f4zero());
+            if (c.pos4 < c.HpP && !nt.root_scatter) stcg4(out_p() + c.pos4, f4zero());
             return;
         }
         const uint32_t none[4] = {0, 0, 0, 0};
         float g[4 * NA], ss[4 * NA];
-        if (MODE == KM_CFR) load_rows<NA>(tabR, true, c.pos4, nrp, none, g);
-        if (MODE != KM_BR) load_rows<NA>(tabS, true, c.pos4, nrp, none, ss);
+        if (MODE == KM_CFR) load_rows<NA>(tabR_p(), true, c.pos4, nrp, none, g);
+        if (MODE != KM_BR) load_rows<NA>(tabS_p(), true, c.pos4, nrp, none, ss);
         float4 vn4 = f4zero();
 #pragma unroll
         for (int i = 0; i < 4; ++i) {
@@ -710,14 +718,17 @@
         if (MODE == KM_CFR) {
 #pragma unroll
             for (int q = 0; q < NA; ++q) {
-                *reinterpret_cast<float4*>(tabR + size_t(c.pos4) * NA + 4 * q) = make_float4(g[4 * q], g[4 * q + 1], g[4 * q + 2], g[4 * q + 3]);
-                *reinterpret_cast<float4*>(tabS + size_t(c.pos4) * NA + 4 * q) = make_float4(ss[4 * q], ss[4 * q + 1], ss[4 * q + 2], ss[4 * q + 3]);
-            }
-        }
-        store_value4(c, nt, Rk, b, out, vn4);
+                *reinterpret_cast<float4*>(tabR_p() + size_t(c.pos4) * NA + 4 * q) = make_float4(g[4 * q], g[4 * q + 1], g[4 * q + 2], g[4 * q + 3]);
+                *reinterpret_cast<float4*>(tabS_p() + size_t(c.pos4) * NA + 4 * q) = make_float4(ss[4 * q], ss[4 * q + 1], ss[4 * q + 2], ss[4 * q + 3]);
+            }
+        }
+        store_value4(c, nt, Rk, b, out_p(), vn4);
         return;
     }
     float* M = SM_X;
+    float* out = out_p();
+    float* tabR = tabR_p();
+    float* tabS = tabS_p();
     if (c.pos4 < c.HpP) {
         *reinterpret_cast<float4*>(M + c.pos4) = mass;
 #pragma unroll
@@ -1244,28 +1255,34 @@
 
 }
 
-size_t task_kernel_smem_bytes(bool wide, int slots, int Hp_pad, int Ho_pad) {
-    const int hx = Hp_pad > Ho_pad ? Hp_pad : Ho_pad;
-    const int hc = 4 * (wide ? 352 : 288);
-    size_t floats = size_t(smem_fixed_floats(hc)) + size_t(slots) * hx;
-    return floats * sizeof(float);
+static int build_threads(int build) { return build == TB_WIDE ? 352 : 288; }
+
+size_t task_kernel_smem_bytes(int build, int slots, int hx) {
+    return (size_t(smem_fixed_floats(4 * build_threads(build))) + size_t(slots) * size_t(hx)) * sizeof(float);
 }
 
 template <int MAXT, int MINB>
 static cudaError_t configure_for(size_t smem, int threads, int* blocks_per_sm) {
-    cudaError_t e;
-    e = cudaFuncSetAttribute(task_kernel<KM_CFR, MAXT, MINB, false>, cudaFuncAttributeMaxDynamicSharedMemorySize, int(smem));
+    int dev = 0, per_sm = 0, reserved = 0;
+    cudaError_t e = cudaGetDevice(&dev);
     if (e != cudaSuccess) return e;
-    e = cudaFuncSetAttribute(task_kernel<KM_CFR, MAXT, MINB, true>, cudaFuncAttributeMaxDynamicSharedMemorySize, int(smem));
-    if (e != cudaSuccess) return e;
-    e = cudaFuncSetAttribute(task_kernel<KM_CFR_DR, MAXT, MINB, false>, cudaFuncAttributeMaxDynamicSharedMemorySize, int(smem));
-    if (e != cudaSuccess) return e;
-    e = cudaFuncSetAttribute(task_kernel<KM_CFR_DR, MAXT, MINB, true>, cudaFuncAttributeMaxDynamicSharedMemorySize, int(smem));
-    if (e != cudaSuccess) return e;
-    e = cudaFuncSetAttribute(task_kernel<KM_BR, MAXT, MINB, false>, cudaFuncAttributeMaxDynamicSharedMemorySize, int(smem));
-    if (e != cudaSuccess) return e;
-    e = cudaFuncSetAttribute(task_kernel<KM_EVAL, MAXT, MINB, false>, cudaFuncAttributeMaxDynamicSharedMemorySize, int(smem));
-    if (e != cudaSuccess) return e;
+    if ((e = cudaDeviceGetAttribute(&per_sm, cudaDevAttrMaxSharedMemoryPerMultiprocessor, dev)) != cudaSuccess) return e;
+    if ((e = cudaDeviceGetAttribute(&reserved, cudaDevAttrReservedSharedMemoryPerBlock, dev)) != cudaSuccess) return e;
+    cudaFuncAttributes fa;
+    if ((e = cudaFuncGetAttributes(&fa, task_kernel<KM_CFR, MAXT, MINB, false>)) != cudaSuccess) return e;
+    const size_t need = size_t(MINB) * (smem + fa.sharedSizeBytes + size_t(reserved));
+    const int carveout = int(std::min<size_t>(100, (need * 100 + size_t(per_sm) - 1) / size_t(per_sm)));
+    auto set = [&](const void* f) -> cudaError_t {
+        cudaError_t r = cudaFuncSetAttribute(f, cudaFuncAttributeMaxDynamicSharedMemorySize, int(smem));
+        if (r != cudaSuccess) return r;
+        return cudaFuncSetAttribute(f, cudaFuncAttributePreferredSharedMemoryCarveout, carveout);
+    };
+    if ((e = set(reinterpret_cast<const void*>(task_kernel<KM_CFR, MAXT, MINB, false>))) != cudaSuccess) return e;
+    if ((e = set(reinterpret_cast<const void*>(task_kernel<KM_CFR, MAXT, MINB, true>))) != cudaSuccess) return e;
+    if ((e = set(reinterpret_cast<const void*>(task_kernel<KM_CFR_DR, MAXT, MINB, false>))) != cudaSuccess) return e;
+    if ((e = set(reinterpret_cast<const void*>(task_kernel<KM_CFR_DR, MAXT, MINB, true>))) != cudaSuccess) return e;
+    if ((e = set(reinterpret_cast<const void*>(task_kernel<KM_BR, MAXT, MINB, false>))) != cudaSuccess) return e;
+    if ((e = set(reinterpret_cast<const void*>(task_kernel<KM_EVAL, MAXT, MINB, false>))) != cudaSuccess) return e;
     int n = 0, m = 0, x = 0;
     e = cudaOccupancyMaxActiveBlocksPerMultiprocessor(&n, task_kernel<KM_CFR, MAXT, MINB, false>, threads + 32, smem);
     if (e != cudaSuccess) return e;
@@ -1278,8 +1295,8 @@
     return cudaSuccess;
 }
 
-cudaError_t configure_task_kernels(size_t smem, int threads, bool wide, int* blocks_per_sm) {
-    if (threads <= 288 && !wide) return configure_for<288, RS_MIN_BLOCKS_288>(smem, threads, blocks_per_sm);
+cudaError_t configure_task_kernels(int build, size_t smem, int threads, int* blocks_per_sm) {
+    if (build == TB_288) return configure_for<288, RS_MIN_BLOCKS_288>(smem, threads, blocks_per_sm);
     return configure_for<352, RS_MIN_BLOCKS_352>(smem, threads, blocks_per_sm);
 }
 
@@ -1295,9 +1312,10 @@
     }
 }
 
-cudaError_t launch_task_kernel(const TaskArgs& a, int mode, int grid, int threads, bool wide, size_t smem, cudaStream_t st) {
+cudaError_t launch_task_kernel(const TaskArgs& a, int mode, int grid, int threads, int build, size_t smem, cudaStream_t st) {
     if (grid <= 0 || a.t1 <= a.t0) return cudaSuccess;
-    if (threads <= 288 && !wide) launch_for<288, RS_MIN_BLOCKS_288>(a, mode, grid, threads, smem, st);
+    if (threads > build_threads(build)) return cudaErrorInvalidValue;
+    if (build == TB_288) launch_for<288, RS_MIN_BLOCKS_288>(a, mode, grid, threads, smem, st);
     else launch_for<352, RS_MIN_BLOCKS_352>(a, mode, grid, threads, smem, st);
     return cudaGetLastError();
 }
diff --git a/rustsolver_b200/csrc/kernels.cuh b/rustsolver_b200/csrc/kernels.cuh
--- a/rustsolver_b200/csrc/kernels.cuh
+++ b/rustsolver_b200/csrc/kernels.cuh
@@ -9,7 +9,6 @@
 
 constexpr int MAX_ACTIONS = MAX_TASK_CHILDREN;
 constexpr int RS_MAX_PEERS = 8;
-constexpr int FAST_ACTIONS = 4;
 constexpr int MAX_TASK_THREADS = 352;
 
 enum KernelMode { KM_CFR = 0, KM_BR = 1, KM_EVAL = 2, KM_CFR_XS = 3, KM_CFR_DR = 4, KM_CFR_XS_DR = 5 };
@@ -87,9 +86,10 @@
     unsigned long long* timing;
 };
 
-size_t task_kernel_smem_bytes(bool wide, int slots, int Hp_pad, int Ho_pad);
-cudaError_t configure_task_kernels(size_t smem, int threads, bool wide, int* blocks_per_sm);
-cudaError_t launch_task_kernel(const TaskArgs& a, int mode, int grid, int threads, bool wide, size_t smem, cudaStream_t st);
+enum TaskBuild { TB_WIDE = 0, TB_288 = 1 };
+size_t task_kernel_smem_bytes(int build, int slots, int hx);
+cudaError_t configure_task_kernels(int build, size_t smem, int threads, int* blocks_per_sm);
+cudaError_t launch_task_kernel(const TaskArgs& a, int mode, int grid, int threads, int build, size_t smem, cudaStream_t st);
 
 cudaError_t launch_scale(float* data, size_t n, float d, cudaStream_t st);
 cudaError_t launch_set_rule(TaskCtl* ctl, const float f[4], cudaStream_t st);
diff --git a/rustsolver_b200/csrc/plan.cpp b/rustsolver_b200/csrc/plan.cpp
--- a/rustsolver_b200/csrc/plan.cpp
+++ b/rustsolver_b200/csrc/plan.cpp
@@ -1452,6 +1452,38 @@
         if (x.dep >= 0) x.dep = int32_t(t[x.dep].first);
 }
 
+void task_round_threads(const Plan& P, bool uniform, int* all, int out[3]) {
+    const size_t maxHP = std::max((P.H[0] + 3) & ~3u, (P.H[1] + 3) & ~3u);
+    *all = int(((maxHP / 4) + 31) / 32 * 32);
+    for (uint32_t k = 0; k < 3; ++k) {
+        out[k] = *all;
+        if (k < P.n_rounds && !P.board_mask[k].empty() && !uniform) {
+            const int left = 52 - __builtin_popcountll(P.board_mask[k][0]);
+            const size_t live_max = std::min<size_t>(maxHP, size_t(left) * size_t(left - 1) / 2);
+            out[k] = std::min(*all, int((((live_max + 3) / 4) + 31) / 32 * 32));
+        }
+    }
+}
+
+void task_runs(const Plan& P, int trav, const MaterializedTasks& m, const int round_threads[3], std::vector<TaskRun>* out) {
+    out->clear();
+    const int hmax = int(std::max((P.H[0] + 3) & ~3u, (P.H[1] + 3) & ~3u));
+    for (const NodeTask& x : m.tasks) {
+        if (x.count == 0) continue;
+        const int thr = round_threads[x.round_k];
+        if (out->empty() || out->back().threads != thr) out->push_back({x.first, x.first + x.count, thr, 0, std::min(hmax, 4 * thr)});
+        TaskRun& r = out->back();
+        r.t1 = x.first + x.count;
+        if (x.kind == TK_DOWN) {
+            int nterm = 0;
+            for (int a = 0; a < x.n_act; ++a) nterm += (x.child[a].kind == CK_FOLD || x.child[a].kind == CK_SHOWDOWN);
+            r.slots = std::max(r.slots, nterm);
+        } else if (x.kind == TK_UP_TRAV && (!P.loc[x.round_k][trav].identity || x.n_act > FAST_BODY_ACTIONS)) {
+            r.slots = std::max(r.slots, 1 + int(x.n_act));
+        }
+    }
+}
+
 bool build_execution_order(const Plan& P, int trav, const MaterializedTasks& m, const uint32_t counts[3], bool force, std::vector<uint32_t>* ord,
                            std::string* err) {
     ord->clear();
diff --git a/rustsolver_b200/csrc/plan.h b/rustsolver_b200/csrc/plan.h
--- a/rustsolver_b200/csrc/plan.h
+++ b/rustsolver_b200/csrc/plan.h
@@ -123,6 +123,15 @@
     uint32_t n_tickets = 0, phase_cut = 0;
 };
 void materialize_tasks(const Plan& P, int trav, const uint32_t counts[3], MaterializedTasks* out);
+
+void task_round_threads(const Plan& P, bool uniform, int* all, int out[3]);
+constexpr int FAST_BODY_ACTIONS = 5;
+struct TaskRun {
+    uint32_t t0, t1;
+    int threads;
+    int slots, hx;
+};
+void task_runs(const Plan& P, int trav, const MaterializedTasks& m, const int round_threads[3], std::vector<TaskRun>* out);
 bool build_execution_order(const Plan& P, int trav, const MaterializedTasks& m, const uint32_t counts[3], bool force, std::vector<uint32_t>* ord,
                            std::string* err);
 std::string check_execution_order(const Plan& P, int trav, const MaterializedTasks& m, const uint32_t counts[3], const std::vector<uint32_t>& ord);
diff --git a/rustsolver_b200/solver.py b/rustsolver_b200/solver.py
--- a/rustsolver_b200/solver.py
+++ b/rustsolver_b200/solver.py
@@ -466,6 +466,14 @@
         sop = np.zeros(hp, dtype=np.uint16)
         check(self._lib.rs_plan_local_tables(self._h, round_idx, player, board_id, _ptr(rec, u32p), _ptr(cl, u16p), _ptr(sop, u16p), dims))
         return rec, cl, sop, nl
+
+    def task_runs(self, traverser: int) -> list:
+        n = C.c_uint32(0)
+        check(self._lib.rs_plan_task_runs(self._h, traverser, None, 0, C.byref(n)))
+        out = np.zeros(6 * n.value, dtype=np.uint32)
+        check(self._lib.rs_plan_task_runs(self._h, traverser, _ptr(out, u32p), out.size, C.byref(n)))
+        keys = ("t0", "t1", "threads", "slots", "hx", "smem")
+        return [dict(zip(keys, (int(x) for x in row))) for row in out.reshape(-1, 6)]
 
     def street_info(self, traverser: int) -> dict:
         out = (C.c_uint32 * 8)()
```

Result: faster. 22.02, median of 6 (+1.3%).
